# NJUVISION/PCGCv2

Measured on AMD Instinct MI355X. Metric: encode+decode Mpoints/sec at fixed bpp (r3 ckpt), vox10 frame, higher is better.
Workload: dtype f32

## Files before the change

### include/pcgc_hip.h

```cpp
#ifndef PCGC_HIP_H
#define PCGC_HIP_H

#include <stddef.h>
#include <stdint.h>

#ifdef __cplusplus
extern "C" {
#endif

const char* pcgc_last_error(void);
int pcgc_version(void);

int64_t pcgc_hash_capacity(int64_t n);
int pcgc_hash_clear(uint64_t* keys , int32_t* vals , int64_t cap, void* stream);
int pcgc_hash_insert(const int32_t* coords , int64_t n, int32_t stride, uint64_t* keys, int32_t* vals,
                     int64_t cap, void* stream);
int pcgc_hash_insert_policy(const int32_t* coords, int64_t n, int32_t stride, uint64_t* keys, int32_t* vals, int64_t cap,
                            int keep_last, void* stream);
int pcgc_hash_first_mask(const int32_t* coords, int64_t n, int32_t stride, const uint64_t* keys, const int32_t* vals,
                         int64_t cap, uint8_t* keep , int32_t* first_row , void* stream);

int pcgc_coords_check_order(const int32_t* coords , int64_t n, int32_t* out2 , void* stream);

int pcgc_coords_quantize(const int32_t* coords, int64_t n, int32_t stride_out, int32_t* out , void* stream);
int pcgc_coords_children(const int32_t* coords, int64_t n, int32_t stride_in, int32_t* out , void* stream);
int pcgc_coords_scale(const int32_t* coords, int64_t n, float factor, int32_t* out , void* stream);

size_t pcgc_scan_workspace_bytes(int64_t n);
int pcgc_mask_scan(const uint8_t* mask , int64_t n, int32_t* prefix , int32_t* total ,
                   void* workspace , size_t workspace_bytes, void* stream);
int pcgc_mask_scan_zeroed(const uint8_t* mask, int64_t n, int32_t* prefix, int32_t* total, void* workspace, size_t workspace_bytes,
                          void* stream);
int pcgc_compact_coords(const int32_t* coords, const uint8_t* mask, const int32_t* prefix, int64_t n,
                        int32_t* out , void* stream);
int pcgc_compact_feats(const float* in, int C, int in_ld, const uint8_t* mask, const int32_t* prefix, int64_t n,
                       float* out , void* stream);

int pcgc_kmap_k3(const int32_t* coords, int64_t n, int32_t stride, const uint64_t* keys, const int32_t* vals,
                 int64_t cap, int32_t* nbr , void* stream);

int pcgc_kmap_k3_children(const int32_t* parent_nbr, int64_t n_parent, int32_t* nbr , void* stream);
int pcgc_kmap_k3_prune(const int32_t* cand_nbr , int64_t n_cand, const uint8_t* mask, const int32_t* prefix,
                       const int32_t* orig , int64_t n_out, int32_t* nbr , void* stream);
int pcgc_kmap_k3_prune_parent(const int32_t* parent_nbr , int64_t n_parent, const uint8_t* mask,
                              const int32_t* prefix, const int32_t* orig, int64_t n_out, int32_t* nbr , void* stream);
int pcgc_kmap_k3_from_coarse(const int32_t* fine , int64_t n_fine, int32_t stride_fine,
                             const int32_t* parent_of , const int32_t* coarse_nbr ,
                             const int32_t* down , int64_t n_coarse, int32_t* nbr ,
                             void* stream);
int pcgc_down_maps(const int32_t* fine, const int32_t* first_row, const int32_t* prefix, int64_t n_fine, int32_t stride_fine,
                   int64_t n_coarse, int32_t* parent_of , int32_t* down , void* stream);
int pcgc_down_prepare(const int32_t* fine , int64_t n, int32_t stride_fine, int32_t* q ,
                      uint64_t* keys, int32_t* vals, int64_t cap, uint8_t* keep , int32_t* first_row ,
                      int32_t* prefix , int32_t* total , void* scan_ws, size_t scan_ws_bytes, void* stream);
int pcgc_down_finish(const int32_t* fine, const int32_t* q, const uint8_t* keep, const int32_t* first_row, const int32_t* prefix,
                     int64_t n, int32_t stride_fine, int64_t n_coarse, int32_t* coarse ,
                     int32_t* parent_of , int32_t* down , void* stream);
int pcgc_down_level(const int32_t* fine , int64_t n, int32_t stride_fine, int32_t* q, uint64_t* keys, int32_t* vals,
                    int64_t cap, uint8_t* keep, int32_t* first_row, int32_t* prefix, int32_t* total, void* scan_ws,
                    size_t scan_ws_bytes, int32_t* coarse , int32_t* parent_of ,
                    int32_t* down , int64_t* n_coarse_out , void* stream);
size_t pcgc_pyramid_scratch_bytes(int64_t n, int levels);
int pcgc_pyramid(const int32_t* fine , int64_t n, int32_t stride, int levels, void* scratch, size_t scratch_bytes,
                 int32_t* const* coarse, int32_t* const* parent_of, int32_t* const* down, int64_t* counts , void* stream);
int pcgc_compact_index(const uint8_t* mask, const int32_t* prefix, int64_t n, int32_t* orig , void* stream);

int pcgc_conv_gather(const int32_t* nbr, int K, int64_t n_out, const float* in, int64_t n_in , int Cin,
                     int in_ld, int in_coff, const float* W, const float* bias, const float* residual, int res_ld,
                     int res_coff, int relu, float* out, int Cout, int out_ld, int out_coff, void* stream);
int pcgc_last_conv_impl(void);
int pcgc_conv_gather_unit(const int32_t* nbr , int K, int64_t n_out, const float* W, const float* bias, int relu,
                          float* out, int Cout, int out_ld, void* stream);
int pcgc_conv_unit_from_coarse(const int32_t* fine , int64_t n_fine, int32_t stride_fine, const int32_t* parent_of,
                               const int32_t* coarse_nbr , const int32_t* down , int64_t n_coarse,
                               const float* W , const float* bias, int relu, float* out, int Cout, int out_ld, void* stream);
int pcgc_set_conv_impl(int impl);
int pcgc_set_up2_impl(int mfma);
int pcgc_irn_block(const int32_t* nbr , int64_t n, const float* x , int C, int x_ld,
                   const float* const* params, float* t_scratch, float* out, int out_ld, void* stream);
int pcgc_irn_pass(const int32_t* nbr, int64_t n, const float* x, int C, int x_ld, const float* const* params,
                  float* t_scratch, float* out, int out_ld, int pass, void* stream);
int pcgc_conv_up2(int64_t n_in, const float* in, int Cin, int in_ld, const float* W , const float* bias,
                  int relu, float* out , int Cout, void* stream);
int pcgc_conv_up2_gather(int64_t n_in, const float* in, int Cin, int in_ld, const int32_t* rows, const float* W ,
                         const float* bias, int relu, float* out , int Cout, void* stream);

int pcgc_conv_child(const int32_t* parent_nbr , int64_t n_parent, const float* in ,
                    int Cin, int in_ld, const float* table , int64_t table_bytes,
                    const float* bias, const float* residual, int res_ld, int relu, float* out, int Cout, int out_ld, void* stream);
int pcgc_irn_child_pass(const int32_t* parent_nbr, int64_t n_parent, int C, int pass, const float* in, int in_ld,
                        const float* table, int64_t table_bytes, const float* b0, const float* b1, const float* b2,
                        const float* x, int x_ld, float* out, int out_ld, void* stream);
int pcgc_irn_child_q4(const int32_t* parent_nbr, int64_t n_parent, int C, int pass, const float* in, int in_ld,
                      const float* table, int64_t table_bytes, const float* b0, const float* b1, const float* b2,
                      const float* x, int x_ld, float* out, int out_ld, void* stream);
int pcgc_cls_child_q4(const int32_t* parent_nbr, int64_t n_parent, const float* in, int Cin, int in_ld, const float* table,
                      int64_t table_bytes, const float* bias, float* out, void* stream);
int pcgc_irn_rows_pass(const int32_t* nbr, int64_t n, int C, int pass, const float* in, int in_ld, const float* table,
                       int64_t table_bytes, const float* b0, const float* b1, const float* b2, const float* x, int x_ld, float* out,
                       int out_ld, void* stream);
int pcgc_irn_rows_q4_pass(const int32_t* nbr, int64_t n, int C, int pass, const float* in, int in_ld, const float* table,
                          int64_t table_bytes, const float* b0, const float* b1, const float* b2, const float* x, int x_ld, float* out,
                          int out_ld, void* stream);
int pcgc_set_rows_q4_variant(int v);
int pcgc_conv_rows(const int32_t* nbr, int64_t n, const float* in, int Cin, int in_ld, const float* table, int64_t table_bytes,
                   const float* bias, const float* residual, int res_ld, int relu, float* out, int Cout, int out_ld, void* stream);
int pcgc_conv_down_rows(const int32_t* down, int64_t n_coarse, const float* in, int64_t n_in, int Cin, int in_ld, const float* table,
                        int64_t table_bytes, const float* bias, int relu, float* out, int Cout, int out_ld, void* stream);

int pcgc_conv_packed64(const int32_t* nbr, int64_t n, const float* in, int in_ld, const float* table, int64_t table_bytes,
                       const float* bias, int relu, float* out, int out_ld, void* stream);
int pcgc_set_packed_tuning(int rows, int waves);

int pcgc_set_convention(int what, int value);

size_t pcgc_topk_workspace_bytes(int64_t n);
int pcgc_topk_mask(const float* logits , int ld, int64_t n, int64_t k, uint8_t* mask ,
                   void* workspace, size_t workspace_bytes, void* stream);
int pcgc_topk_mask_segments(const float* logits, int ld, int nseg, const int64_t* seg_rows, const int64_t* seg_k, uint8_t* mask,
                            void* workspace, size_t workspace_bytes, void* stream);
size_t pcgc_topk_select_workspace_bytes(int64_t n);
int pcgc_topk_select(const float* logits , int ld, int nseg, const int64_t* seg_rows, const int64_t* seg_k,
                     const int32_t* coords, const int32_t* parent_coords, int32_t parent_stride,
                     uint8_t* bits, int32_t* wprefix, int32_t* orig, int32_t* out_coords, void* workspace, size_t workspace_bytes, void* stream);
int pcgc_kmap_k3_prune_sel(const int32_t* cand_nbr , int64_t n_cand, const uint8_t* bits, const int32_t* wprefix,
                           const int32_t* orig , int64_t n_out, int32_t* nbr , void* stream);
int pcgc_kmap_k3_prune_parent_sel(const int32_t* parent_nbr , int64_t n_parent, const uint8_t* bits, const int32_t* wprefix,
                                  const int32_t* orig, int64_t n_out, int32_t* nbr , void* stream);
int pcgc_gather_rows_f32_ld(const float* in, int C, int in_ld, const int32_t* orig, int64_t n_out, float* out , void* stream);
int pcgc_batch_counts(const int32_t* coords , int64_t n, int32_t* counts , void* stream);

size_t pcgc_sort_workspace_bytes(int64_t n);
int pcgc_sort_zyx(const int32_t* coords, int64_t n, int32_t* perm , void* workspace, size_t workspace_bytes,
                  void* stream);
int pcgc_sort_bzyx(const int32_t* coords, int64_t n, int32_t* perm , void* workspace, size_t workspace_bytes, void* stream);
int pcgc_gather_rows_i32x4(const int32_t* in, const int32_t* perm, int64_t n, int32_t* out, void* stream);
int pcgc_gather_rows_f32(const float* in, int C, const int32_t* perm, int64_t n, float* out, void* stream);

int pcgc_relu(const float* in, int64_t count, float* out, void* stream);
int pcgc_add(const float* a, const float* b, int64_t count, float* out, void* stream);

int pcgc_round_minmax(const float* feats, int64_t count, float* minmax , void* stream);
int pcgc_symbolize(const float* feats, int64_t count, float min_v, int16_t* sym , void* stream);
int pcgc_desymbolize(const int16_t* sym, int64_t count, float min_v, float* feats, void* stream);
int pcgc_quantize_symbols(const float* feats, int64_t count, float* minmax , int16_t* sym , void* stream);
int pcgc_quantize_symbols_segments(const float* feats, int C, int nseg, const int64_t* seg_rows, float* minmax, int16_t* sym, void* stream);
int pcgc_cdf_table(const float* params , int C, float min_v, float max_v, uint16_t* cdf_u16 ,
                   float* cdf_f32 , void* stream);


size_t pcgc_loss_workspace_bytes(int64_t elements);
int pcgc_hash_contains(const int32_t* coords , int64_t n, const uint64_t* keys, const int32_t* vals, int64_t cap,
                       const uint8_t* or_mask , uint8_t* mask , void* stream);
int pcgc_eb_likelihood(const float* feats, int ld, int64_t n, int C, const float* params , float bound, float* likelihood,
                       double* bits, void* workspace, size_t workspace_bytes, void* stream);
int pcgc_neg_log2_sum(const float* x, int ld, int64_t n, int C, double* bits , void* workspace, size_t workspace_bytes, void* stream);
int pcgc_bce_logits(const float* logits, int64_t ld, int64_t n, const uint8_t* truth , const uint8_t* pred ,
                    double* bce, int64_t* counts, void* workspace, size_t workspace_bytes, void* stream);

size_t pcgc_occ_workspace_bytes(int64_t n);
int pcgc_occ_symbols(const float* logits, int64_t ld, int64_t n, const uint8_t* truth , uint16_t* packed ,
                     int64_t* sums , void* workspace, size_t workspace_bytes, void* stream);
int pcgc_occ_tables(uint16_t* p1, int32_t* cost);

size_t pcgc_conv_wgrad_workspace_bytes(int K, int64_t n_rows, int Cin, int Cout);
int64_t pcgc_conv_wgrad_rows_per_group(int K, int64_t n_rows, int Cin, int Cout);
int pcgc_conv_wgrad(const int32_t* nbr, int K, int64_t n_out, const float* x, int64_t n_in, int Cin, int x_ld, const float* gy, int Cout,
                    int gy_ld, float* gW, float* gb, void* workspace, size_t workspace_bytes, void* stream);
int pcgc_conv_up2_wgrad(int64_t n_in, const float* x, int64_t x_rows, int Cin, int x_ld, const int32_t* rows, const float* gy, int Cout,
                        int gy_ld, float* gW, float* gb, void* workspace, size_t workspace_bytes, void* stream);
int pcgc_kmap_invert(const int32_t* nbr, int K, int64_t n_out, int64_t n_in, int32_t* inv , void* stream);
int pcgc_relu_bwd(const float* g, int g_ld, const float* y, int y_ld, int64_t n, int C, float* out, int out_ld, void* stream);
int pcgc_scatter_rows(const float* gy, int C, int gy_ld, const int32_t* orig, int64_t n_rows, float* gx, int64_t n_out, int gx_ld, void* stream);
int pcgc_bce_logits_bwd(const float* logits, int64_t ld, int64_t n, const uint8_t* truth, double scale, float* g , void* stream);
size_t pcgc_eb_bwd_workspace_bytes(int64_t n, int C);
int pcgc_eb_likelihood_bwd(const float* feats, int ld, int64_t n, int C, const float* params , float bound, double scale,
                           float* gy, float* gparams, void* workspace, size_t workspace_bytes, void* stream);

int64_t pcgc_rc_encode(const uint16_t* cdf , int C, int Lp, const int16_t* sym , int64_t n,
                       uint8_t* out , int64_t cap);
int pcgc_rc_decode(const uint16_t* cdf, int C, int Lp, const uint8_t* in, int64_t nbytes, int16_t* sym, int64_t n);
#define PCGC_RC_CKPT_WORDS 6
int64_t pcgc_rc_encode_indexed(const uint16_t* cdf, int C, int Lp, const int16_t* sym, int64_t n, uint8_t* out, int64_t cap, int n_ckpt,
                               uint32_t* ckpt );
int pcgc_rc_decode_indexed(const uint16_t* cdf, int C, int Lp, const uint8_t* in, int64_t nbytes, int16_t* sym, int64_t n, int n_ckpt,
                           const uint32_t* ckpt);
int64_t pcgc_rc_encode_ctx(const uint16_t* cdf , int R, int Lp, const uint16_t* ctx , const int16_t* sym ,
                           int64_t n, uint8_t* out , int64_t cap);
int pcgc_rc_decode_ctx(const uint16_t* cdf, int R, int Lp, const uint16_t* ctx , const uint8_t* in, int64_t nbytes,
                       int16_t* sym , int64_t n);
int pcgc_set_rc_threads(int threads);
int pcgc_set_rc_lanes(int mode);
int pcgc_set_rc_impl(int impl);

int64_t pcgc_oct_encode(const int32_t* xyz , int64_t n, uint8_t* out, int64_t cap);
int64_t pcgc_oct_decode_count(const uint8_t* in, int64_t nbytes);
int pcgc_oct_decode(const uint8_t* in, int64_t nbytes, int32_t* xyz , int64_t n);
int pcgc_set_oct_tiled(int on);
int pcgc_set_oct_model(int model);
int pcgc_oct_warm(void);

int pcgc_d1_nn(const int32_t* a , int64_t na, const uint64_t* b_keys, const int32_t* b_vals, int64_t b_cap,
               const int32_t* offsets , int n_offsets, double* sum , uint64_t* max_d2 ,
               int32_t* unresolved , void* stream);
int pcgc_d1_cell_masks(const int32_t* b , int64_t nb, const uint64_t* cell_keys, const int32_t* cell_vals, int64_t cell_cap,
                       uint64_t* masks , int64_t n_cells, void* stream);
int pcgc_d1_nn_cells(const int32_t* a , int64_t na, const uint64_t* cell_keys, const int32_t* cell_vals, int64_t cell_cap,
                     const uint64_t* masks, const int32_t* offsets , int n_offsets, int32_t reach2, double* sum, uint64_t* max_d2,
                     int32_t* unresolved, void* stream);

int pcgc_d2_runs(const int32_t* qs , int64_t nq, int32_t* runlen , void* stream);
int pcgc_d2_count(const int32_t* p , int64_t n, const int32_t* sel, const uint64_t* cell_keys, const int32_t* cell_vals,
                  int64_t cell_cap, const uint64_t* masks, const uint64_t* keys, const int32_t* vals, int64_t cap, const int32_t* runlen,
                  const int32_t* offsets , int n_offsets, int32_t reach2, int64_t* best , int32_t* cnt ,
                  int32_t* unresolved , int32_t* n_unresolved , void* stream);
int pcgc_d2_fill(const int32_t* p, int64_t n, const int32_t* sel, const uint64_t* cell_keys, const int32_t* cell_vals, int64_t cell_cap,
                 const uint64_t* masks, const uint64_t* keys, const int32_t* vals, int64_t cap, const int32_t* runlen, const int32_t* perm,
                 const int32_t* offsets, int n_offsets, int32_t reach2, const int64_t* best, const int64_t* seg , int32_t* rows, void* stream);
int pcgc_d2_exhaustive(const int32_t* p, int64_t n, const int32_t* sel, const int32_t* qs, int64_t nq, const int32_t* perm, int fill,
                       int64_t* best, int32_t* cnt, const int64_t* seg, int32_t* rows, int32_t* n_empty , void* stream);
size_t pcgc_d2_scan_workspace_bytes(int64_t n);
int pcgc_d2_scan(const int32_t* cnt , int64_t n, int64_t* seg , void* workspace, size_t workspace_bytes, void* stream);
int pcgc_d2_segment_lowest(const int64_t* seg, int64_t n, int32_t* rows, int32_t cap, int32_t* kept, void* stream);
int pcgc_d2_recv_count(const int64_t* seg, const int32_t* kept, int64_t na, const int32_t* rows, int64_t nb, int32_t* rcnt, void* stream);
int pcgc_d2_recv_fill(const int64_t* seg, const int32_t* kept, int64_t na, const int32_t* rows, int64_t nb, const int64_t* rseg, int32_t* cursor,
                      int32_t* recv, void* stream);
int pcgc_d2_normals(const int64_t* rseg, const int32_t* recv, int64_t nb, const double* na, const int64_t* seg_ba, const int32_t* kept_ba,
                    const int32_t* rows_ba, double* nb_out, void* stream);
int pcgc_d2_c2p(const int32_t* p, int64_t n, const int32_t* q, const double* nq, const int64_t* seg, const int32_t* kept, const int32_t* rows,
                double* c2p, void* stream);
size_t pcgc_d2_reduce_workspace_bytes(void);
int pcgc_d2_reduce(const int64_t* c2c, const double* c2p, int64_t n, int64_t* c2c_sum_max, double* c2p_sum, void* workspace, size_t workspace_bytes,
                   void* stream);

size_t pcgc_attr_transfer_workspace_bytes(int64_t ns, int64_t nt, int channels);
int pcgc_attr_transfer(const int64_t* seg_st, const int32_t* kept_st, const int32_t* rows_st, int64_t ns, const int64_t* seg_ts,
                       const int32_t* kept_ts, const int32_t* rows_ts, int64_t nt, const uint8_t* attr_s, int channels, uint8_t* attr_t,
                       void* workspace, size_t workspace_bytes, void* stream);
int pcgc_colour_dist(const uint8_t* cp, int64_t n, const uint8_t* cq, int64_t nq, const int64_t* seg, const int32_t* kept, const int32_t* rows,
                     int64_t* yuv2, int32_t* rgb2, void* stream);
size_t pcgc_colour_reduce_workspace_bytes(void);
int pcgc_colour_reduce(const int64_t* yuv2, const int32_t* rgb2, int64_t n, int64_t* out, void* workspace, size_t workspace_bytes, void* stream);

int64_t pcgc_normals_ball_masks(int32_t r2, uint64_t* table );
size_t pcgc_normals_workspace_bytes(int64_t n);
int pcgc_normals_estimate(const int32_t* coords , int64_t n, const int32_t* qs , const int32_t* perm,
                          const uint64_t* cell_keys, const int32_t* cell_vals, int64_t cell_cap, const uint64_t* masks, const uint64_t* keys,
                          const int32_t* vals, int64_t cap, const int32_t* runlen, const uint64_t* ball , int32_t r2, int orient,
                          const double* viewpoint , int64_t* moments , double* normals ,
                          double* lam , int32_t* count , uint8_t* valid , void* workspace,
                          size_t workspace_bytes, void* stream);
int pcgc_set_normals_mapping(int mode);

int64_t pcgc_ply_read_ascii_geo(const char* path, int32_t* xyz , int64_t cap);
int pcgc_ply_write_ascii_geo(const char* path, const int32_t* xyz , int64_t n);
int pcgc_ply_write_ascii_geo_rgb(const char* path, const int32_t* xyz , const uint8_t* rgb , int64_t n);

typedef int (*pcgc_table_fn)(const float* params, int C, float min_v, float max_v, uint16_t* table_u16, float* cdf_f32);
int pcgc_items_encode(int n_items, const char* const* stems, const int16_t* sym, const int32_t* xyz, const int64_t* rows, const float* ranges,
                      int C, const int32_t* counts, const float* eb_params, pcgc_table_fn table_fn, int index_segments, int write_coords,
                      int threads);
int pcgc_items_probe(int n_items, const char* const* stems, int64_t* rows, int32_t* channels, float* ranges, int32_t* counts,
                     int32_t* native_coords);
int pcgc_items_decode(int n_items, const char* const* stems, const int64_t* rows, int C, const float* ranges, const int32_t* native_coords,
                      const float* eb_params, pcgc_table_fn table_fn, int use_sidecar, int16_t* sym, int32_t* xyz, int coord_layout,
                      int coord_scale, int threads);

int pcgc_level_prepare_children(const int32_t* coords, int64_t n, int32_t stride, uint64_t* keys, int32_t* vals, int64_t cap, int32_t* nbr,
                                int32_t* children, int32_t* nbr_children, void* stream);

int pcgc_frame_decode(const char* stem, int C, const float* eb_params, pcgc_table_fn table_fn, int use_sidecar, int coord_scale,
                      int64_t cap_rows, int16_t* sym, int32_t* level, int64_t* info, float* range, int threads);
int pcgc_frame_decode_begin(const char* stem, int C, const float* eb_params, pcgc_table_fn table_fn, int use_sidecar, int coord_scale,
                            int64_t cap_rows, int16_t* sym, int32_t* level, int64_t* info, float* range, int threads);
int pcgc_frame_decode_end(void);
int pcgc_frame_worker_test(int delay_us);

int pcgc_table_cache(int mode);

uint32_t pcgc_crc32(uint32_t crc, const uint8_t* buf, int64_t len);

int pcgc_mesh_read(const char* path, double* verts , int64_t vcap, int32_t* faces , int64_t fcap,
                   int64_t* counts );
size_t pcgc_mesh_cdf_workspace_bytes(int64_t T);
int pcgc_mesh_area_cdf(const double* verts , int64_t V, const int32_t* faces , int64_t T,
                       double* cdf , int32_t* bad_faces , void* workspace, size_t workspace_bytes, void* stream);
int pcgc_mesh_sample(const double* verts, int64_t V, const int32_t* faces, const double* cdf, int64_t T, uint64_t seed, uint64_t first,
                     int64_t n, int32_t* tri , double* points , void* stream);
size_t pcgc_mesh_voxelize_workspace_bytes(int32_t resolution);
int pcgc_mesh_voxelize(const double* verts, int64_t V, const int32_t* faces, const double* cdf, int64_t T, uint64_t seed, int64_t n,
                       const double* R , int32_t resolution, int32_t* out , int64_t cap,
                       int32_t* count , void* workspace , size_t workspace_bytes, void* stream);

#define PCGC_COLLATE_MAX_ITEMS 16
typedef struct pcgc_collate_item {
    int64_t offset;
    int32_t first_row, rows, width, symmetry, extent, reserved;
} pcgc_collate_item;
int pcgc_collate_rows(const uint8_t* arena , const pcgc_collate_item* items , int n_items,
                      int32_t* coords_out , float* feats_out , void* stream);

#ifdef __cplusplus
}
#endif
#endif
```

### pcgcv2_amd/_build.py

```python
import os
import subprocess
import sys
from concurrent.futures import ThreadPoolExecutor

HERE = os.path.dirname(os.path.abspath(__file__))
CSRC = os.path.join(HERE, 'csrc')
VARIANT = os.environ.get('PCGC_BUILD_VARIANT', '')
OBJ = os.path.join(CSRC, '_obj' + ('_' + VARIANT if VARIANT else ''))
LIB = os.path.join(HERE, 'libpcgc_hip' + ('_' + VARIANT if VARIANT else '') + '.so')
SOURCES = ['coords.hip', 'select.hip', 'conv.hip', 'child_conv.hip', 'child_conv32.hip', 'child_cls_w.hip', 'child_irn.hip', 'child_irn_a16.hip', 'child_irn_b16.hip',
           'child_irn_a32.hip', 'child_irn_b32.hip', 'child_q4.hip', 'rows_irn.hip', 'rows_q4.hip', 'conv_packed.hip', 'entropy.hip', 'loss.hip', 'occupancy.hip', 'grad.hip', 'metric.hip', 'colour.hip', 'normals.hip', 'mesh.hip', 'collate.hip', 'hostcodec.cpp', 'ply.cpp', 'mesh_io.cpp']
HEADERS = [os.path.join(CSRC, 'pcgc_common.h'), os.path.join(CSRC, 'mfma_util.h'), os.path.join(CSRC, 'child_kernels.h'), os.path.join(CSRC, 'child_q4.h'), os.path.join(CSRC, 'q4x.h'), os.path.join(CSRC, 'q4x_sched.h'), os.path.join(CSRC, 'rows_q4_policy.h'), os.path.join(CSRC, 'eb_logits.h'), os.path.join(CSRC, 'occupancy_tables.h'), os.path.join(HERE, '..', 'include', 'pcgc_hip.h')]
FLAGS = ['--offload-arch=gfx950', '-O3', '-std=c++17', '-ffp-contract=off', '-fPIC', '-Wall', '-Wno-unused-result'] + \
        os.environ.get('PCGC_EXTRA_HIPCC_FLAGS', '').split()


def _hipcc():
    for c in (os.environ.get('HIPCC'), '/opt/rocm/bin/hipcc', 'hipcc'):
        if c and (os.path.isabs(c) and os.path.exists(c) or not os.path.isabs(c)):
            return c
    return 'hipcc'


def _stale(target, deps):
    if not os.path.exists(target):
        return True
    t = os.path.getmtime(target)
    return any(os.path.getmtime(d) > t for d in deps)


def build(force=False, verbose=False):
    os.makedirs(OBJ, exist_ok=True)
    if VARIANT:
        import shutil
        base = os.path.join(CSRC, '_obj')
        for src in SOURCES:
            o = src.rsplit('.', 1)[0] + '.o'
            if 'child_kernels.h' not in open(os.path.join(CSRC, src)).read() and os.path.exists(os.path.join(base, o)) \
                    and not os.path.exists(os.path.join(OBJ, o)):
                shutil.copy2(os.path.join(base, o), os.path.join(OBJ, o))
    hipcc = _hipcc()
    jobs = []
    only = [t for t in os.environ.get('PCGC_BUILD_ONLY', '').split(',') if t]
    for src in SOURCES:
        s = os.path.join(CSRC, src)
        o = os.path.join(OBJ, src.rsplit('.', 1)[0] + '.o')
        if only and os.path.exists(o):
            if src.rsplit('.', 1)[0] in only:
                jobs.append((o, [hipcc] + FLAGS + (['-x', 'hip'] if src.endswith('.hip') else []) + ['-c', s, '-o', o]))
            continue
        if force or _stale(o, [s] + HEADERS):
            lang = ['-x', 'hip'] if src.endswith('.hip') else []
            jobs.append((o, [hipcc] + FLAGS + lang + ['-c', s, '-o', o]))

    def run(job):
        o, cmd = job
        if verbose:
            print(' '.join(cmd), file=sys.stderr)
        r = subprocess.run(cmd, capture_output=True, text=True)
        if r.returncode != 0:
            raise RuntimeError('hipcc failed:\n' + ' '.join(cmd) + '\n' + r.stderr[-4000:])
        return o

    with ThreadPoolExecutor(max_workers=max(2, min(8, os.cpu_count() or 4))) as ex:
        list(ex.map(run, jobs))
    objs = [os.path.join(OBJ, s.rsplit('.', 1)[0] + '.o') for s in SOURCES]
    if force or jobs or _stale(LIB, objs):
        cmd = [hipcc, '--offload-arch=gfx950', '-shared', '-fPIC', '-o', LIB] + objs + ['-lz']
        r = subprocess.run(cmd, capture_output=True, text=True)
        if r.returncode != 0:
            raise RuntimeError('link failed:\n' + r.stderr[-4000:])
    if not VARIANT:
        build_reftable(force=force)
    return LIB


REFTABLE_LIB = os.path.join(HERE, 'libpcgc_reftable.so')


def build_reftable(force=False):
    src = os.path.join(CSRC, 'reftable.cpp')
    if not (force or _stale(REFTABLE_LIB, [src])):
        return REFTABLE_LIB
    import torch
    tdir = os.path.dirname(torch.__file__)
    cmd = ['g++', '-O2', '-std=c++17', '-fPIC', '-shared', f'-D_GLIBCXX_USE_CXX11_ABI={int(torch._C._GLIBCXX_USE_CXX11_ABI)}',
           '-I' + os.path.join(tdir, 'include'), '-I' + os.path.join(tdir, 'include', 'torch', 'csrc', 'api', 'include'), src,
           '-o', REFTABLE_LIB, '-L' + os.path.join(tdir, 'lib'), '-ltorch_cpu', '-lc10', '-Wl,-rpath,' + os.path.join(tdir, 'lib')]
    r = subprocess.run(cmd, capture_output=True, text=True)
    if r.returncode != 0:
        raise RuntimeError('g++ failed:\n' + ' '.join(cmd) + '\n' + r.stderr[-4000:])
    return REFTABLE_LIB


if __name__ == '__main__':
    print(build(force='--force' in sys.argv, verbose=True))
```

### pcgcv2_amd/_lib.py

```python
import ctypes as C
import os

_HERE = os.path.dirname(os.path.abspath(__file__))
LIB_PATH = os.environ.get('PCGC_LIB') or os.path.join(_HERE, 'libpcgc_hip.so')

vp, i64, i32, f32, sz = C.c_void_p, C.c_int64, C.c_int32, C.c_float, C.c_size_t
ci = C.c_int

SIGNATURES = {
    'pcgc_last_error': (C.c_char_p, []),
    'pcgc_version': (ci, []),
    'pcgc_hash_capacity': (i64, [i64]),
    'pcgc_hash_clear': (ci, [vp, vp, i64, vp]),
    'pcgc_hash_insert': (ci, [vp, i64, i32, vp, vp, i64, vp]),
    'pcgc_hash_insert_policy': (ci, [vp, i64, i32, vp, vp, i64, ci, vp]),
    'pcgc_set_convention': (ci, [ci, ci]),
    'pcgc_hash_first_mask': (ci, [vp, i64, i32, vp, vp, i64, vp, vp, vp]),
    'pcgc_coords_check_order': (ci, [vp, i64, vp, vp]),
    'pcgc_coords_quantize': (ci, [vp, i64, i32, vp, vp]),
    'pcgc_coords_children': (ci, [vp, i64, i32, vp, vp]),
    'pcgc_coords_scale': (ci, [vp, i64, f32, vp, vp]),
    'pcgc_scan_workspace_bytes': (sz, [i64]),
    'pcgc_mask_scan': (ci, [vp, i64, vp, vp, vp, sz, vp]),
    'pcgc_mask_scan_zeroed': (ci, [vp, i64, vp, vp, vp, sz, vp]),
    'pcgc_compact_coords': (ci, [vp, vp, vp, i64, vp, vp]),
    'pcgc_compact_feats': (ci, [vp, ci, ci, vp, vp, i64, vp, vp]),
    'pcgc_kmap_k3': (ci, [vp, i64, i32, vp, vp, i64, vp, vp]),
    'pcgc_kmap_k3_children': (ci, [vp, i64, vp, vp]),
    'pcgc_kmap_k3_prune': (ci, [vp, i64, vp, vp, vp, i64, vp, vp]),
    'pcgc_kmap_k3_prune_parent': (ci, [vp, i64, vp, vp, vp, i64, vp, vp]),
    'pcgc_kmap_k3_from_coarse': (ci, [vp, i64, i32, vp, vp, vp, i64, vp, vp]),
    'pcgc_down_maps': (ci, [vp, vp, vp, i64, i32, i64, vp, vp, vp]),
    'pcgc_down_prepare': (ci, [vp, i64, i32, vp, vp, vp, i64, vp, vp, vp, vp, vp, sz, vp]),
    'pcgc_down_finish': (ci, [vp, vp, vp, vp, vp, i64, i32, i64, vp, vp, vp, vp]),
    'pcgc_down_level': (ci, [vp, i64, i32, vp, vp, vp, i64, vp, vp, vp, vp, vp, sz, vp, vp, vp, vp, vp]),
    'pcgc_pyramid_scratch_bytes': (sz, [i64, ci]),
    'pcgc_pyramid': (ci, [vp, i64, i32, ci, vp, sz, vp, vp, vp, vp, vp]),
    'pcgc_compact_index': (ci, [vp, vp, i64, vp, vp]),
    'pcgc_conv_gather': (ci, [vp, ci, i64, vp, i64, ci, ci, ci, vp, vp, vp, ci, ci, ci, vp, ci, ci, ci, vp]),
    'pcgc_conv_gather_unit': (ci, [vp, ci, i64, vp, vp, ci, vp, ci, ci, vp]),
    'pcgc_conv_unit_from_coarse': (ci, [vp, i64, i32, vp, vp, vp, i64, vp, vp, ci, vp, ci, ci, vp]),
    'pcgc_set_conv_impl': (ci, [ci]),
    'pcgc_last_conv_impl': (ci, []),
    'pcgc_set_up2_impl': (ci, [ci]),
    'pcgc_irn_block': (ci, [vp, i64, vp, ci, ci, vp, vp, vp, ci, vp]),
    'pcgc_irn_pass': (ci, [vp, i64, vp, ci, ci, vp, vp, vp, ci, ci, vp]),
    'pcgc_conv_child': (ci, [vp, i64, vp, ci, ci, vp, i64, vp, vp, ci, ci, vp, ci, ci, vp]),
    'pcgc_irn_child_pass': (ci, [vp, i64, ci, ci, vp, ci, vp, i64, vp, vp, vp, vp, ci, vp, ci, vp]),
    'pcgc_irn_child_q4': (ci, [vp, i64, ci, ci, vp, ci, vp, i64, vp, vp, vp, vp, ci, vp, ci, vp]),
    'pcgc_cls_child_q4': (ci, [vp, i64, vp, ci, ci, vp, i64, vp, vp, vp]),
    'pcgc_conv_down_rows': (ci, [vp, i64, vp, i64, ci, ci, vp, i64, vp, ci, vp, ci, ci, vp]),
    'pcgc_conv_rows': (ci, [vp, i64, vp, ci, ci, vp, i64, vp, vp, ci, ci, vp, ci, ci, vp]),
    'pcgc_irn_rows_pass': (ci, [vp, i64, ci, ci, vp, ci, vp, i64, vp, vp, vp, vp, ci, vp, ci, vp]),
    'pcgc_irn_rows_q4_pass': (ci, [vp, i64, ci, ci, vp, ci, vp, i64, vp, vp, vp, vp, ci, vp, ci, vp]),
    'pcgc_set_rows_q4_variant': (ci, [ci]),
    'pcgc_conv_packed64': (ci, [vp, i64, vp, ci, vp, i64, vp, ci, vp, ci, vp]),
    'pcgc_set_packed_tuning': (ci, [ci, ci]),
    'pcgc_conv_up2': (ci, [i64, vp, ci, ci, vp, vp, ci, vp, ci, vp]),
    'pcgc_conv_up2_gather': (ci, [i64, vp, ci, ci, vp, vp, vp, ci, vp, ci, vp]),
    'pcgc_topk_workspace_bytes': (sz, [i64]),
    'pcgc_topk_mask': (ci, [vp, ci, i64, i64, vp, vp, sz, vp]),
    'pcgc_topk_mask_segments': (ci, [vp, ci, ci, vp, vp, vp, vp, sz, vp]),
    'pcgc_topk_select_workspace_bytes': (sz, [i64]),
    'pcgc_topk_select': (ci, [vp, ci, ci, vp, vp, vp, vp, i32, vp, vp, vp, vp, vp, sz, vp]),
    'pcgc_kmap_k3_prune_sel': (ci, [vp, i64, vp, vp, vp, i64, vp, vp]),
    'pcgc_kmap_k3_prune_parent_sel': (ci, [vp, i64, vp, vp, vp, i64, vp, vp]),
    'pcgc_gather_rows_f32_ld': (ci, [vp, ci, ci, vp, i64, vp, vp]),
    'pcgc_batch_counts': (ci, [vp, i64, vp, vp]),
    'pcgc_sort_bzyx': (ci, [vp, i64, vp, vp, sz, vp]),
    'pcgc_quantize_symbols_segments': (ci, [vp, ci, ci, vp, vp, vp, vp]),
    'pcgc_sort_workspace_bytes': (sz, [i64]),
    'pcgc_sort_zyx': (ci, [vp, i64, vp, vp, sz, vp]),
    'pcgc_gather_rows_i32x4': (ci, [vp, vp, i64, vp, vp]),
    'pcgc_gather_rows_f32': (ci, [vp, ci, vp, i64, vp, vp]),
    'pcgc_relu': (ci, [vp, i64, vp, vp]),
    'pcgc_add': (ci, [vp, vp, i64, vp, vp]),
    'pcgc_round_minmax': (ci, [vp, i64, vp, vp]),
    'pcgc_symbolize': (ci, [vp, i64, f32, vp, vp]),
    'pcgc_desymbolize': (ci, [vp, i64, f32, vp, vp]),
    'pcgc_quantize_symbols': (ci, [vp, i64, vp, vp, vp]),
    'pcgc_cdf_table': (ci, [vp, ci, f32, f32, vp, vp, vp]),
    'pcgc_loss_workspace_bytes': (sz, [i64]),
    'pcgc_hash_contains': (ci, [vp, i64, vp, vp, i64, vp, vp, vp]),
    'pcgc_eb_likelihood': (ci, [vp, ci, i64, ci, vp, f32, vp, vp, vp, sz, vp]),
    'pcgc_neg_log2_sum': (ci, [vp, ci, i64, ci, vp, vp, sz, vp]),
    'pcgc_bce_logits': (ci, [vp, i64, i64, vp, vp, vp, vp, vp, sz, vp]),
    'pcgc_occ_workspace_bytes': (sz, [i64]),
    'pcgc_occ_symbols': (ci, [vp, i64, i64, vp, vp, vp, vp, sz, vp]),
    'pcgc_occ_tables': (ci, [vp, vp]),
    'pcgc_conv_wgrad_workspace_bytes': (sz, [ci, i64, ci, ci]),
    'pcgc_conv_wgrad_rows_per_group': (i64, [ci, i64, ci, ci]),
    'pcgc_conv_wgrad': (ci, [vp, ci, i64, vp, i64, ci, ci, vp, ci, ci, vp, vp, vp, sz, vp]),
    'pcgc_conv_up2_wgrad': (ci, [i64, vp, i64, ci, ci, vp, vp, ci, ci, vp, vp, vp, sz, vp]),
    'pcgc_kmap_invert': (ci, [vp, ci, i64, i64, vp, vp]),
    'pcgc_relu_bwd': (ci, [vp, ci, vp, ci, i64, ci, vp, ci, vp]),
    'pcgc_scatter_rows': (ci, [vp, ci, ci, vp, i64, vp, i64, ci, vp]),
    'pcgc_bce_logits_bwd': (ci, [vp, i64, i64, vp, C.c_double, vp, vp]),
    'pcgc_eb_bwd_workspace_bytes': (sz, [i64, ci]),
    'pcgc_eb_likelihood_bwd': (ci, [vp, ci, i64, ci, vp, f32, C.c_double, vp, vp, vp, sz, vp]),
    'pcgc_d1_cell_masks': (ci, [vp, i64, vp, vp, i64, vp, i64, vp]),
    'pcgc_d1_nn_cells': (ci, [vp, i64, vp, vp, i64, vp, vp, ci, i32, vp, vp, vp, vp]),
    'pcgc_d1_nn': (ci, [vp, i64, vp, vp, i64, vp, ci, vp, vp, vp, vp]),
    'pcgc_d2_runs': (ci, [vp, i64, vp, vp]),
    'pcgc_d2_count': (ci, [vp, i64, vp, vp, vp, i64, vp, vp, vp, i64, vp, vp, ci, i32, vp, vp, vp, vp, vp]),
    'pcgc_d2_fill': (ci, [vp, i64, vp, vp, vp, i64, vp, vp, vp, i64, vp, vp, vp, ci, i32, vp, vp, vp, vp]),
    'pcgc_d2_exhaustive': (ci, [vp, i64, vp, vp, i64, vp, ci, vp, vp, vp, vp, vp, vp]),
    'pcgc_d2_scan_workspace_bytes': (sz, [i64]),
    'pcgc_d2_scan': (ci, [vp, i64, vp, vp, sz, vp]),
    'pcgc_d2_segment_lowest': (ci, [vp, i64, vp, i32, vp, vp]),
    'pcgc_d2_recv_count': (ci, [vp, vp, i64, vp, i64, vp, vp]),
    'pcgc_d2_recv_fill': (ci, [vp, vp, i64, vp, i64, vp, vp, vp, vp]),
    'pcgc_d2_normals': (ci, [vp, vp, i64, vp, vp, vp, vp, vp, vp]),
    'pcgc_d2_c2p': (ci, [vp, i64, vp, vp, vp, vp, vp, vp, vp]),
    'pcgc_d2_reduce_workspace_bytes': (sz, []),
    'pcgc_d2_reduce': (ci, [vp, vp, i64, vp, vp, vp, sz, vp]),
    'pcgc_attr_transfer_workspace_bytes': (sz, [i64, i64, ci]),
    'pcgc_attr_transfer': (ci, [vp, vp, vp, i64, vp, vp, vp, i64, vp, ci, vp, vp, sz, vp]),
    'pcgc_colour_dist': (ci, [vp, i64, vp, i64, vp, vp, vp, vp, vp, vp]),
    'pcgc_colour_reduce_workspace_bytes': (sz, []),
    'pcgc_colour_reduce': (ci, [vp, vp, i64, vp, vp, sz, vp]),
    'pcgc_normals_ball_masks': (i64, [i32, vp]),
    'pcgc_normals_workspace_bytes': (sz, [i64]),
    'pcgc_normals_estimate': (ci, [vp, i64, vp, vp, vp, vp, i64, vp, vp, vp, i64, vp, vp, i32, ci, vp, vp, vp, vp, vp, vp, vp, sz, vp]),
    'pcgc_set_normals_mapping': (ci, [ci]),
    'pcgc_rc_encode': (i64, [vp, ci, ci, vp, i64, vp, i64]),
    'pcgc_rc_decode': (ci, [vp, ci, ci, vp, i64, vp, i64]),
    'pcgc_set_rc_impl': (ci, [ci]),
    'pcgc_rc_encode_indexed': (i64, [vp, ci, ci, vp, i64, vp, i64, ci, vp]),
    'pcgc_rc_decode_indexed': (ci, [vp, ci, ci, vp, i64, vp, i64, ci, vp]),
    'pcgc_rc_encode_ctx': (i64, [vp, ci, ci, vp, vp, i64, vp, i64]),
    'pcgc_rc_decode_ctx': (ci, [vp, ci, ci, vp, vp, i64, vp, i64]),
    'pcgc_set_rc_threads': (ci, [ci]),
    'pcgc_set_rc_lanes': (ci, [ci]),
    'pcgc_set_oct_tiled': (ci, [ci]),
    'pcgc_set_oct_model': (ci, [ci]),
    'pcgc_oct_warm': (ci, []),
    'pcgc_oct_encode': (i64, [vp, i64, vp, i64]),
    'pcgc_oct_decode_count': (i64, [vp, i64]),
    'pcgc_oct_decode': (ci, [vp, i64, vp, i64]),
    'pcgc_items_encode': (ci, [ci, vp, vp, vp, vp, vp, ci, vp, vp, vp, ci, ci, ci]),
    'pcgc_items_probe': (ci, [ci, vp, vp, vp, vp, vp, vp]),
    'pcgc_items_decode': (ci, [ci, vp, vp, ci, vp, vp, vp, vp, ci, vp, vp, ci, ci, ci]),
    'pcgc_level_prepare_children': (ci, [vp, i64, i32, vp, vp, i64, vp, vp, vp, vp]),
    'pcgc_frame_decode': (ci, [C.c_char_p, ci, vp, vp, ci, ci, i64, vp, vp, vp, vp, ci]),
    'pcgc_frame_decode_begin': (ci, [C.c_char_p, ci, vp, vp, ci, ci, i64, vp, vp, vp, vp, ci]),
    'pcgc_frame_decode_end': (ci, []),
    'pcgc_frame_worker_test': (ci, [ci]),
    'pcgc_table_cache': (ci, [ci]),
    'pcgc_crc32': (C.c_uint32, [C.c_uint32, vp, i64]),
    'pcgc_ply_read_ascii_geo': (i64, [C.c_char_p, vp, i64]),
    'pcgc_ply_write_ascii_geo': (ci, [C.c_char_p, vp, i64]),
    'pcgc_ply_write_ascii_geo_rgb': (ci, [C.c_char_p, vp, vp, i64]),
    'pcgc_mesh_read': (ci, [C.c_char_p, vp, i64, vp, i64, vp]),
    'pcgc_mesh_cdf_workspace_bytes': (sz, [i64]),
    'pcgc_mesh_area_cdf': (ci, [vp, i64, vp, i64, vp, vp, vp, sz, vp]),
    'pcgc_mesh_sample': (ci, [vp, i64, vp, vp, i64, C.c_uint64, C.c_uint64, i64, vp, vp, vp]),
    'pcgc_mesh_voxelize_workspace_bytes': (sz, [i32]),
    'pcgc_mesh_voxelize': (ci, [vp, i64, vp, vp, i64, C.c_uint64, i64, vp, i32, vp, i64, vp, vp, sz, vp]),
    'pcgc_collate_rows': (ci, [vp, vp, ci, vp, vp, vp]),
}


class CollateItem(C.Structure):
    _fields_ = [('offset', i64), ('first_row', i32), ('rows', i32), ('width', i32), ('symmetry', i32), ('extent', i32), ('reserved', i32)]


class PcgcError(RuntimeError):
    pass


_lib = None


def lib():
    global _lib
    if _lib is None:
        if not os.path.exists(LIB_PATH):
            raise PcgcError(f'{LIB_PATH} not found: run `python -c "import __graft_entry__ as g; g.build()"` '
                            '(hipcc --offload-arch=gfx950). The HIP library is mandatory; there is no fallback path.')
        l = C.CDLL(LIB_PATH)
        for name, (res, args) in SIGNATURES.items():
            fn = getattr(l, name)
            fn.restype, fn.argtypes = res, args
        _lib = l
    return _lib


REFTABLE_PATH = os.path.join(_HERE, 'libpcgc_reftable.so')
_reftable = None


def reftable_lib():
    global _reftable
    if _reftable is None:
        if not os.path.exists(REFTABLE_PATH):
            raise PcgcError(f'{REFTABLE_PATH} not found: run `python -c "import __graft_entry__ as g; g.build()"`')
        import torch
        l = C.CDLL(REFTABLE_PATH)
        l.pcgc_reference_table.restype = ci
        l.pcgc_reference_table.argtypes = [vp, ci, f32, f32, vp, vp]
        l.pcgc_reference_table_clear.restype = ci
        l.pcgc_reference_table_clear.argtypes = []
        _reftable = l
    return _reftable


def check(rc, what=''):
    if rc != 0:
        raise PcgcError(f'{what or "pcgc call"} failed ({rc}): {lib().pcgc_last_error().decode()}')
```

### pcgcv2_amd/csrc/child_kernels.h

```cpp
#pragma once
#include "pcgc_common.h"
#include "mfma_util.h"
#include <type_traits>

#ifdef PCGC_CHILD_TIMING
static __device__ unsigned long long g_child_dbg[8];
#define CHILD_T(var) const unsigned long long var = __builtin_amdgcn_s_memtime()
#define CHILD_TADD(slot, a, b) do { child_dbg[slot] += (b) - (a); } while (0)
#define CHILD_DBG_DECL unsigned long long child_dbg[8] = {0, 0, 0, 0, 0, 0, 0, 0};
#define CHILD_DBG_PARAM , unsigned long long (&child_dbg)[8]
#define CHILD_DBG_ARG , child_dbg
#define CHILD_TFLUSH do { if ((threadIdx.x & 63) == 0) { for (int q_ = 0; q_ < 8; ++q_) if (child_dbg[q_]) atomicAdd(&g_child_dbg[q_], child_dbg[q_]); } } while (0)
#define CHILD_TIMING_READER(NAME)                                                                                      \
    extern "C" int NAME(unsigned long long* out8, int reset) {                                                         \
        (void)hipDeviceSynchronize();                                                                                  \
        if (out8) (void)hipMemcpyFromSymbol(out8, HIP_SYMBOL(g_child_dbg), 8 * sizeof(unsigned long long));           \
        if (reset) { unsigned long long z[8] = {0}; (void)hipMemcpyToSymbol(HIP_SYMBOL(g_child_dbg), z, sizeof(z)); }  \
        return 0;                                                                                                      \
    }
#else
#define CHILD_T(var)
#define CHILD_TADD(slot, a, b)
#define CHILD_DBG_DECL
#define CHILD_DBG_PARAM
#define CHILD_DBG_ARG
#define CHILD_TFLUSH
#define CHILD_TIMING_READER(NAME)
#endif

struct ChildEpi {
    const float* bias;
    const float* res;
    int res_ld;
    int relu;
    float* out;
    int out_ld;
    int nt;
};
struct IrnEpi {
    const float* b0;
    const float* b1;
    const float* b2;
    const float* x;
    int x_ld;
    float* out;
    int out_ld;
};
namespace {


constexpr int halo_p1(int c) { return c == 0 ? 0 : (c == 3 ? 2 : 1); }
constexpr int halo_bit(int c) { return (c == 0 || c == 2) ? 1 : 0; }
constexpr int cell_kp(int c) { return halo_p1(c >> 4) * 9 + halo_p1((c >> 2) & 3) * 3 + halo_p1(c & 3); }
constexpr int cell_child(int c) { return halo_bit(c & 3) + 2 * halo_bit((c >> 2) & 3) + 4 * halo_bit(c >> 4); }
constexpr bool axis_reach(int c, int jb) { return c - jb >= 0 && c - jb <= 2; }
constexpr unsigned cell_reach(int c) {
    unsigned m = 0;
    for (int j = 0; j < 8; ++j)
        if (axis_reach(c & 3, j & 1) && axis_reach((c >> 2) & 3, (j >> 1) & 1) && axis_reach(c >> 4, j >> 2)) m |= 1u << j;
    return m;
}
constexpr int cell_k(int c, int j) {
    return ((c >> 4) - (j >> 2)) * 9 + (((c >> 2) & 3) - ((j >> 1) & 1)) * 3 + ((c & 3) - (j & 1));
}
constexpr int cz_of(int c) { return c >> 4; }
constexpr int cy_of(int c) { return (c >> 2) & 3; }
constexpr int cx_of(int c) { return c & 3; }
constexpr bool in02(int v) { return v >= 0 && v <= 2; }

struct HaloGeometry {
    static constexpr int NCELLS = 64, ROW_MUL = 8, NMAP = 27;
    static constexpr int kp(int c) { return cell_kp(c); }
    static constexpr int child(int c) { return cell_child(c); }
    static constexpr int byte_off(int) { return 0; }
};

template <int NB_, int NT, int HZ = -1>
struct PlainConv : HaloGeometry {
    static constexpr int NB = NB_, ROWCHUNKS = 4, T = 8 * NT, KS = 4;
    static constexpr int Z_HALF = HZ;
    static constexpr bool HALF = false;
    static constexpr int kfirst(int) { return 0; }
    static constexpr bool active(int c, int t) { return (HZ < 0 || (((t / NT) >> 2) & 1) == HZ) && ((cell_reach(c) >> (t / NT)) & 1); }
    static constexpr int frag(int c, int t) { return cell_k(c, t / NT) * NT + t % NT; }
    static constexpr bool uses_block(int, int) { return true; }
    static constexpr int frag_off(int c, int t, int cb) { return (frag(c, t) * NB + cb) * 64 * KS * 4; }
};
template <int NB_>
struct ClsHead : HaloGeometry {
    static constexpr int NB = NB_, ROWCHUNKS = 4, T = 1, KS = 4;
    static constexpr bool HALF = true;
    static constexpr int ROWB = NB * 64 + 16;
    static constexpr int TABLE_BYTES = (125 * ROWB + 1023) / 1024 * 1024;
    static constexpr int kfirst(int) { return 0; }
    static constexpr bool active(int, int) { return true; }
    static constexpr bool uses_block(int, int) { return true; }
    static constexpr int frag_off(int c, int, int cb) { return (cz_of(c) * 25 + cy_of(c) * 5 + cx_of(c)) * ROWB + cb * 64; }
    __device__ static inline int lane_table_off(int mi, int mq) {
        const int j = mi & 7;
        return (31 - (25 * (j >> 2) + 5 * ((j >> 1) & 1) + (j & 1))) * ROWB + mq * 16;
    }
};
template <int C, int HZ = -1>
struct PassA : HaloGeometry {
    static_assert(C == 16 || C == 32, "children-level passes: C = 16, 32 (C = 64 runs on the rows kernels through the level's own map)");
    static constexpr int Q = C / 4, NB = C / 16, ROWCHUNKS = 4, CPT = 16 / Q , TH = 8 / CPT, T = 2 * TH, KS = 4;
    static_assert(HZ < 0 || CPT <= 2, "half units: tiles of one or two children (a z-half tile holds both halves' columns)");
    static constexpr int Z_HALF = HZ;
    static constexpr bool HALF = false;
    static constexpr int kfirst(int) { return 0; }
    static constexpr int tz(int t) { return CPT == 4 ? (t % TH) : (t % TH) >> 1; }
    static constexpr int ty(int t) { return (t % TH) & 1; }
    static constexpr bool active(int c, int t) {
        const int kz = cz_of(c) - tz(t);
        if (HZ >= 0 && tz(t) != HZ) return false;
        if (CPT == 4) {
            if (t < TH) return in02(kz);
            return kz == 1 && (cy_of(c) == 1 || cy_of(c) == 2) && (cx_of(c) == 1 || cx_of(c) == 2);
        }
        const int ky = cy_of(c) - ty(t);
        if (t < TH) return in02(kz) && in02(ky);
        return kz == 1 && ky == 1 && (cx_of(c) == 1 || cx_of(c) == 2);
    }
    static constexpr int N0 = CPT == 4 ? 48 : (CPT == 2 ? 36 : 27);
    static constexpr int frag(int c, int t) {
        const int kz = cz_of(c) - tz(t);
        if (CPT == 4) return t < TH ? kz * 16 + (c & 15) : N0 + (cy_of(c) - 1) * 2 + (cx_of(c) - 1);
        const int ky = cy_of(c) - ty(t);
        return t < TH ? (kz * 3 + ky) * 4 + cx_of(c) : N0 + (cx_of(c) - 1);
    }
    static constexpr bool uses_block(int, int) { return true; }
    static constexpr int frag_off(int c, int t, int cb) { return (frag(c, t) * NB + cb) * 64 * KS * 4; }
};
template <int C, int HZ = -1, bool T2_ = false>
struct PassB : HaloGeometry {
    static constexpr bool T2 = T2_;
    static_assert(!T2_ || C == 16, "the split layout exists for C = 16");
    static constexpr int Q = C / 4, NB = 1, ROWCHUNKS = Q / 2 , KS = Q / 4;
    static constexpr int CPT0 = 16 / (2 * Q) , T0 = 8 / CPT0, CPT1 = 16 / Q, T1 = 8 / CPT1, T = T0 + T1;
    static constexpr int Z_HALF = HZ;
    static_assert(HZ < 0 || CPT1 <= 2, "half units: no tile may hold children of both z halves");
    static constexpr bool HALF = false;
    static constexpr int kfirst(int t) { return t < T0 ? 0 : KS; }
    static constexpr int tile_z(int t) { return t < T0 ? ((t * CPT0) >> 2) & 1 : (((t - T0) * CPT1) >> 2) & 1; }
    static constexpr bool active(int c, int t) {
        if (HZ >= 0 && tile_z(t) != HZ) return false;
        if (t < T0) {
            if (CPT0 == 1) return (cell_reach(c) >> t) & 1;
            return in02(cz_of(c) - (t >> 1)) && in02(cy_of(c) - (t & 1));
        }
        const int u = t - T0;
        if (CPT1 == 2) return in02(cz_of(c) - (u >> 1)) && in02(cy_of(c) - (u & 1));
        return in02(cz_of(c) - u);
    }
    static constexpr int N0 = CPT0 == 1 ? 27 : 36;
    static constexpr int N1 = CPT1 == 2 ? 36 : 48;
    static constexpr int FRAG_W12 = N0 + N1;
    static constexpr int frag(int c, int t) {
        if (t < T0) {
            if (CPT0 == 1) return cell_k(c, t);
            return ((cz_of(c) - (t >> 1)) * 3 + (cy_of(c) - (t & 1))) * 4 + cx_of(c);
        }
        const int u = t - T0;
        if (CPT1 == 2) return N0 + ((cz_of(c) - (u >> 1)) * 3 + (cy_of(c) - (u & 1))) * 4 + cx_of(c);
        return N0 + (cz_of(c) - u) * 16 + (c & 15);
    }
    static constexpr bool uses_block(int, int) { return true; }
    static constexpr int frag_off(int c, int t, int cb) { return (frag(c, t) * NB + cb) * 64 * KS * 4; }
};

template <class V, class = void> struct child_t2_layout : std::false_type {};
template <class V> struct child_t2_layout<V, std::enable_if_t<V::T2>> : std::true_type {};

template <int I, int N, typename F>
__device__ __forceinline__ void static_for(F&& f) {
    if constexpr (I < N) {
        f(std::integral_constant<int, I>{});
        static_for<I + 1, N>(f);
    }
}

template <int KS> struct BFrag;
template <> struct BFrag<4> {
    f32x4 v;
    template <int OFF> __device__ __forceinline__ void load(unsigned base) { asm volatile("ds_read_b128 %0, %1 offset:%2" : "=v"(v) : "v"(base), "n"(OFF) : "memory"); }
    __device__ __forceinline__ void tie() { asm volatile("" : "+v"(v)); }
    __device__ __forceinline__ float get(int i) const { return v[i]; }
};
typedef float f32x2 __attribute__((ext_vector_type(2)));
template <> struct BFrag<2> {
    f32x2 v;
    template <int OFF> __device__ __forceinline__ void load(unsigned base) { asm volatile("ds_read_b64 %0, %1 offset:%2" : "=v"(v) : "v"(base), "n"(OFF) : "memory"); }
    __device__ __forceinline__ void tie() { asm volatile("" : "+v"(v)); }
    __device__ __forceinline__ float get(int i) const { return v[i]; }
};
template <> struct BFrag<1> {
    float v;
    template <int OFF> __device__ __forceinline__ void load(unsigned base) { asm volatile("ds_read_b32 %0, %1 offset:%2" : "=v"(v) : "v"(base), "n"(OFF) : "memory"); }
    __device__ __forceinline__ void tie() { asm volatile("" : "+v"(v)); }
    __device__ __forceinline__ float get(int) const { return v; }
};
template <int OFF>
__device__ __forceinline__ float lds_ld32_off(unsigned base) {
    float v;
    asm volatile("ds_read_b32 %0, %1 offset:%2" : "=v"(v) : "v"(base), "n"(OFF) : "memory");
    return v;
}
template <int OFF>
__device__ __forceinline__ f32x4 lds_ld128_off(unsigned base) {
    f32x4 v;
    asm volatile("ds_read_b128 %0, %1 offset:%2" : "=v"(v) : "v"(base), "n"(OFF) : "memory");
    return v;
}

template <class V> constexpr int frag_floats() { return (V::HALF ? 32 : 64) * V::KS; }

template <int NW, bool PERSIST = true>
__device__ __forceinline__ int64_t child_tile(int i, int wave, int64_t ntiles) {
    if constexpr (!PERSIST) {
        const int64_t tile = (int64_t)xcd_tile(blockIdx.x, gridDim.x) * NW + wave;
        return (i == 0 && tile < ntiles) ? tile : -1;
    }
    const int64_t S = (ntiles + 7) >> 3;
    const int64_t l = (blockIdx.x >> 3) + (int64_t)(gridDim.x >> 3) * (wave + NW * i);
    const int64_t tile = (blockIdx.x & 7) * S + l;
    return (l < S && tile < ntiles) ? tile : -1;
}

template <int NW>
__device__ __forceinline__ void child_stage_table(const float* __restrict__ table, int table_bytes, unsigned char* lds_raw) {
    float4* tab = (float4*)lds_raw;
    for (int i = threadIdx.x; i < table_bytes / 16; i += NW * 64) tab[i] = ((const float4*)table)[i];
    __syncthreads();
}

struct ChildCells { int n; int c[64]; };
template <class V> constexpr ChildCells child_cells() {
    ChildCells L{};
    for (int c = 0; c < V::NCELLS; ++c) {
        bool used = false;
        for (int t = 0; t < V::T; ++t) used = used || V::active(c, t);
        if (used) L.c[L.n++] = c;
    }
    return L;
}

template <class V, int D, int MT>
__device__ __forceinline__ void child_tile_mainloop_mt(const int32_t* __restrict__ pnbr, int64_t n_p, int64_t p0,
                                                       const __amdgpu_buffer_rsrc_t& rs_in, int in_ld, const unsigned char* lds_raw,
                                                       float4* ring, f32x4 (&acc)[MT][V::T] CHILD_DBG_PARAM) {
    constexpr int NB = V::NB, T = V::T, KS = V::KS;
    static_assert(MT == 1 || MT == 2, "one or two M tiles per wave");
    static_assert((D & (D - 1)) == 0, "ring depth must be a power of two");
    static_assert((D - 1) * NB * MT < 64, "vmcnt is 6 bits");
    CHILD_T(t_tile0);
    const int lane = threadIdx.x & 63;
    const int mi = lane & 15, mq = lane >> 4;
    const int dma_r = lane >> 2;
    bool row_ok[MT];
#pragma unroll
    for (int m = 0; m < MT; ++m) row_ok[m] = p0 + 16 * m + dma_r < n_p;
    constexpr unsigned ABSENT = 0xF0000000u;
    unsigned rowb[MT][V::NMAP];
#pragma unroll
    for (int m = 0; m < MT; ++m)
#pragma unroll
        for (int kp = 0; kp < V::NMAP; ++kp) rowb[m][kp] = (unsigned)pnbr[(int64_t)kp * n_p + (row_ok[m] ? p0 + 16 * m + dma_r : 0)];
    const int f_a = (0x78 >> (2 * (mi >> 2))) & 3;
    const int dma_chunk = (lane & 3) ^ ((0x78 >> (2 * ((dma_r >> 2) & 3))) & 3);
    const bool chunk_ok = dma_chunk < V::ROWCHUNKS;
    const unsigned row_bytes = (unsigned)in_ld * 4u;
    asm volatile("s_waitcnt vmcnt(0)" ::: "memory");
#pragma unroll
    for (int m = 0; m < MT; ++m)
#pragma unroll
        for (int kp = 0; kp < V::NMAP; ++kp)
            rowb[m][kp] = (row_ok[m] && (int)rowb[m][kp] >= 0) ? rowb[m][kp] * ((unsigned)V::ROW_MUL * row_bytes) : ABSENT;
    constexpr bool T2 = child_t2_layout<V>::value;
    const unsigned lane_off = chunk_ok ? (unsigned)dma_chunk * (T2 ? 64u : 16u) : ABSENT;
    CHILD_T(t_loop0);

    constexpr ChildCells CL = child_cells<V>();
    constexpr int NC = CL.n;
    auto issue = [&](auto ii) {
        constexpr int i = decltype(ii)::value, c = CL.c[i];
        float4* dst = ring + (i & (D - 1)) * (MT * NB * 64);
#pragma unroll
        for (int m = 0; m < MT; ++m) {
            unsigned voff = rowb[m][V::kp(c)] + (T2 ? (unsigned)((V::child(c) >> 2) * 128 + (V::child(c) & 3) * 16) : (unsigned)V::child(c) * row_bytes) + lane_off +
                            (unsigned)V::byte_off(c);
            if constexpr (V::ROWCHUNKS < 4) voff = chunk_ok ? voff : 0xFFFFFFF0u;
#pragma unroll
            for (int cb = 0; cb < NB; ++cb)
                __builtin_amdgcn_raw_ptr_buffer_load_lds(rs_in, (lds_void_ptr)(dst + (m * NB + cb) * 64), 16, (int)(voff + cb * 64), 0, 0, 0);
        }
        asm volatile("" ::: "memory");
    };

#pragma unroll
    for (int m = 0; m < MT; ++m)
#pragma unroll
        for (int t = 0; t < T; ++t) acc[m][t] = (f32x4){0.f, 0.f, 0.f, 0.f};
    unsigned tab_lane;
    if constexpr (V::HALF) tab_lane = (unsigned)(uintptr_t)(lds_void_ptr)(lds_raw + V::lane_table_off(mi, mq));
    else tab_lane = (unsigned)(uintptr_t)(lds_void_ptr)((const float*)lds_raw + lane * KS);
    unsigned a_addr[4];
#pragma unroll
    for (int jj = 0; jj < 4; ++jj) a_addr[jj] = (unsigned)(uintptr_t)(lds_void_ptr)((const float*)ring + (mi * 4 + (jj ^ f_a)) * 4 + mq);
    constexpr unsigned ksteps_used = [] { unsigned m = 0; for (int t = 0; t < T; ++t) for (int j = 0; j < KS; ++j) m |= 1u << (V::kfirst(t) + j); return m; }();

    static_assert(NB * T <= 32, "all B fragments of a cell are held in registers at once");
    static_for<0, (D < NC ? D : NC)>(issue);
    static_for<0, NC>([&](auto ii) {
        constexpr int i = decltype(ii)::value, c = CL.c[i];
        constexpr int younger = (NC - 1 - i) < (D - 1) ? (NC - 1 - i) : (D - 1);
        wait_vmcnt<younger * NB * MT>();
        float a[MT][NB][4];
        BFrag<KS> b[NB][T];
        static_for<0, NB>([&](auto icb) {
            constexpr int cb = decltype(icb)::value;
            static_for<0, MT>([&](auto im) {
                constexpr int m = decltype(im)::value;
                static_for<0, 4>([&](auto ij) {
                    constexpr int jj = decltype(ij)::value;
                    if constexpr ((ksteps_used >> jj) & 1)
                        a[m][cb][jj] = lds_ld32_off<(((i & (D - 1)) * MT + m) * NB + cb) * 1024>(a_addr[jj]);
                });
            });
            static_for<0, T>([&](auto it) {
                constexpr int t = decltype(it)::value;
                if constexpr (V::active(c, t) && V::uses_block(t, cb)) {
                    constexpr int off = V::frag_off(c, t, cb);
                    if constexpr (off < 65536) b[cb][t].template load<off>(tab_lane);
                    else b[cb][t].template load<off - 65536>(tab_lane + 65536);
                }
            });
        });
        asm volatile("s_waitcnt lgkmcnt(0)" ::: "memory");
        static_for<0, NB>([&](auto icb) {
            constexpr int cb = decltype(icb)::value;
            static_for<0, MT>([&](auto im) {
                static_for<0, 4>([&](auto ij) {
                    constexpr int jj = decltype(ij)::value;
                    if constexpr ((ksteps_used >> jj) & 1) lds_tie(a[decltype(im)::value][cb][jj]);
                });
            });
            static_for<0, T>([&](auto it) {
                constexpr int t = decltype(it)::value;
                if constexpr (V::active(c, t) && V::uses_block(t, cb)) b[cb][t].tie();
            });
        });
        if constexpr (i + D < NC) issue(std::integral_constant<int, i + D>{});
        static_for<0, NB>([&](auto icb) {
            constexpr int cb = decltype(icb)::value;
            static_for<0, 4>([&](auto ij) {
                constexpr int jj = decltype(ij)::value;
                static_for<0, T>([&](auto it) {
                    constexpr int t = decltype(it)::value;
                    if constexpr (V::active(c, t) && V::uses_block(t, cb) && jj >= V::kfirst(t) && jj < V::kfirst(t) + KS) {
                        static_for<0, MT>([&](auto im) {
                            constexpr int m = decltype(im)::value;
                            acc[m][t] = __builtin_amdgcn_mfma_f32_16x16x4f32(a[m][cb][jj], b[cb][t].get(jj - V::kfirst(t)), acc[m][t], 0, 0, 0);
                        });
                    }
                });
            });
        });
    });
#ifdef PCGC_CHILD_TIMING
    asm volatile("s_nop 0" : "+v"(acc[0][0]));
    CHILD_T(t_loop1);
    CHILD_TADD(0, t_tile0, t_loop0);
    CHILD_TADD(1, t_loop0, t_loop1);
    CHILD_TADD(3, 0ull, 1ull);
#endif
}

template <class V, int D>
__device__ __forceinline__ void child_tile_mainloop(const int32_t* __restrict__ pnbr, int64_t n_p, int64_t p0,
                                                    const __amdgpu_buffer_rsrc_t& rs_in, int in_ld, const unsigned char* lds_raw,
                                                    float4* ring, f32x4 (&acc)[V::T] CHILD_DBG_PARAM) {
    child_tile_mainloop_mt<V, D, 1>(pnbr, n_p, p0, rs_in, in_ld, lds_raw, ring, reinterpret_cast<f32x4 (&)[1][V::T]>(acc) CHILD_DBG_ARG);
}

__device__ __forceinline__ void wave_lds_sync() {
    __builtin_amdgcn_fence(__ATOMIC_RELEASE, "wavefront");
    __builtin_amdgcn_wave_barrier();
    __builtin_amdgcn_fence(__ATOMIC_ACQUIRE, "wavefront");
}

template <int W, int ROWS>
struct ChildResidual { float4 x[(ROWS * (W / 4) + 63) / 64]; };
template <int W, int ROWS>
__device__ __forceinline__ void child_flush_prefetch(ChildResidual<W, ROWS>& rr, int64_t row0, int64_t rows_total, const float* __restrict__ res,
                                                     int res_ld, int lane, int half = -1) {
    constexpr int C4 = W / 4, N = (ROWS * C4 + 63) / 64;
    if (!res) return;
#pragma unroll
    for (int it = 0; it < N; ++it) {
        const int i = lane + 64 * it, lr = i / C4, c4 = i % C4;
        const int64_t row = row0 + lr;
        const bool ok = i < ROWS * C4 && row < rows_total && !(half >= 0 && ((lr >> 2) & 1) != half);
        rr.x[it] = ok ? *(const float4*)(res + row * res_ld + 4 * c4) : make_float4(0.f, 0.f, 0.f, 0.f);
    }
}
template <int W, int ROWS>
__device__ __forceinline__ void child_flush(const float* scratch, const ChildResidual<W, ROWS>& rr, bool has_res, int64_t row0, int64_t rows_total,
                                            float* __restrict__ out, int out_ld, int relu, int lane, int half = -1) {
    constexpr int C4 = W / 4, N = (ROWS * C4 + 63) / 64;
    ChildResidual<W, ROWS> xr = rr;
    if (has_res) {
#pragma unroll
        for (int it = 0; it < N; ++it) asm volatile("" : "+v"(xr.x[it].x), "+v"(xr.x[it].y), "+v"(xr.x[it].z), "+v"(xr.x[it].w));
    }
#pragma unroll
    for (int it = 0; it < N; ++it) {
        const int i = lane + 64 * it, lr = i / C4, c4 = i % C4;
        const int64_t row = row0 + lr;
        if (i >= ROWS * C4 || row >= rows_total || (half >= 0 && ((lr >> 2) & 1) != half)) continue;
        float4 v = ((const float4*)scratch)[i];
        if (has_res) {
            const float4 x = xr.x[it];
            v.x = v.x + x.x; v.y = v.y + x.y; v.z = v.z + x.z; v.w = v.w + x.w;
        }
        if (relu) { v.x = fmaxf(v.x, 0.0f); v.y = fmaxf(v.y, 0.0f); v.z = fmaxf(v.z, 0.0f); v.w = fmaxf(v.w, 0.0f); }
        *(float4*)(out + row * out_ld + 4 * c4) = v;
    }
}
template <int W, int ROWS>
__device__ __forceinline__ void child_flush(const float* scratch, int64_t row0, int64_t rows_total, float* __restrict__ out, int out_ld,
                                            int relu, int lane, int half = -1) {
    constexpr int C4 = W / 4, N = (ROWS * C4 + 63) / 64;
#pragma unroll
    for (int it = 0; it < N; ++it) {
        const int i = lane + 64 * it, lr = i / C4, c4 = i % C4;
        const int64_t row = row0 + lr;
        if (i >= ROWS * C4 || row >= rows_total || (half >= 0 && ((lr >> 2) & 1) != half)) continue;
        float4 v = ((const float4*)scratch)[i];
        if (relu) { v.x = fmaxf(v.x, 0.0f); v.y = fmaxf(v.y, 0.0f); v.z = fmaxf(v.z, 0.0f); v.w = fmaxf(v.w, 0.0f); }
        *(float4*)(out + row * out_ld + 4 * c4) = v;
    }
}
template <int W>
__device__ __forceinline__ void child_flush(const float* scratch, int rows, int64_t row0, int64_t rows_total, float* __restrict__ out,
                                            int out_ld, const float* __restrict__ res, int res_ld, int relu, int lane, int half = -1) {
    constexpr int C4 = W / 4;
    for (int i = lane; i < rows * C4; i += 64) {
        const int lr = i / C4, c4 = i % C4;
        const int64_t row = row0 + lr;
        if (row >= rows_total || (half >= 0 && ((lr >> 2) & 1) != half)) continue;
        float4 v = ((const float4*)scratch)[i];
        if (res) {
            const float4 x = *(const float4*)(res + row * res_ld + 4 * c4);
            v.x = v.x + x.x; v.y = v.y + x.y; v.z = v.z + x.z; v.w = v.w + x.w;
        }
        if (relu) { v.x = fmaxf(v.x, 0.0f); v.y = fmaxf(v.y, 0.0f); v.z = fmaxf(v.z, 0.0f); v.w = fmaxf(v.w, 0.0f); }
        *(float4*)(out + row * out_ld + 4 * c4) = v;
    }
}

#define CHILD_IN_ROWS(V, n_p) (V::ROW_MUL * (n_p))
#define CHILD_KERNEL_PROLOGUE(V, NW, D, RING_FLOAT4)                                                                          \
    CHILD_DBG_DECL                                                                                                            \
    extern __shared__ __attribute__((aligned(16))) unsigned char lds_raw[];                                                   \
    const int lane = threadIdx.x & 63, mi = lane & 15, mq = lane >> 4;                                                        \
    const int wave = __builtin_amdgcn_readfirstlane(threadIdx.x >> 6);                                                        \
    float4* ring = (float4*)(lds_raw + table_bytes) + wave * (RING_FLOAT4);                                                   \
    child_stage_table<NW>(table, table_bytes, lds_raw);                                                                        \
    const __amdgpu_buffer_rsrc_t rs_in = __builtin_amdgcn_make_buffer_rsrc((void*)in, 0, (int)(CHILD_IN_ROWS(V, n_p) * in_ld * 4), 0x00020000); \
    const int64_t ntiles = (n_p + 15) >> 4;

template <class T_> struct child_type_tag { using type = T_; };
template <int NB, int NT, int NW, int D, bool SPLIT = false, int MT = 1, bool RES = false>
__global__ void __launch_bounds__(NW * 64)
k_child_conv(const int32_t* __restrict__ pnbr, int64_t n_p, const float* __restrict__ in, int in_ld,
             const float* __restrict__ table, int table_bytes, ChildEpi ep) {
    using V = PlainConv<NB, NT>;
    CHILD_KERNEL_PROLOGUE(V, NW, D, D * NB * 64 * MT)
    float bvs[NT];
#pragma unroll
    for (int n = 0; n < NT; ++n) bvs[n] = ep.bias ? ep.bias[16 * n + mi] : 0.0f;
    auto unit = [&](auto tag, const int64_t pu) {
        using VV = typename decltype(tag)::type;
        constexpr int HZ = VV::Z_HALF;
        f32x4 acc[MT][VV::T];
        child_tile_mainloop_mt<VV, D, MT>(pnbr, n_p, pu, rs_in, in_ld, lds_raw, ring, acc CHILD_DBG_ARG);
        constexpr int W = 16 * NT, CH = (64 * W * 4 <= D * NB * 1024 * MT) ? 64 : 32, PPC = CH / 8, MQC = PPC / 4;
        float* scratch = (float*)ring;
#pragma unroll
        for (int m = 0; m < MT; ++m) {
            const int64_t p0 = pu + 16 * m;
            if (m > 0 && p0 >= n_p) break;
#pragma unroll
            for (int h = 0; h < 128 / CH; ++h) {
                ChildResidual<W, RES ? CH : 1> rr;
                if constexpr (RES) child_flush_prefetch<W, CH>(rr, 8 * p0 + h * CH, 8 * n_p, ep.res, ep.res_ld, lane, HZ);
                if (mq / MQC == h) {
#pragma unroll
                    for (int t = 0; t < VV::T; ++t) {
                        const int j = t / NT, n = t % NT;
                        if (HZ >= 0 && ((j >> 2) & 1) != HZ) continue;
#pragma unroll
                        for (int r = 0; r < 4; ++r) {
                            float v = acc[m][t][r];
                            if (ep.bias) v = v + bvs[n];
                            scratch[(8 * (4 * (mq % MQC) + r) + j) * W + 16 * n + mi] = v;
                        }
                    }
                }
                wave_lds_sync();
                if constexpr (RES) child_flush<W, CH>(scratch, rr, true, 8 * p0 + h * CH, 8 * n_p, ep.out, ep.out_ld, ep.relu, lane, HZ);
                else child_flush<W, CH>(scratch, 8 * p0 + h * CH, 8 * n_p, ep.out, ep.out_ld, ep.relu, lane, HZ);
                wave_lds_sync();
            }
        }
    };
    const int64_t nunits = (SPLIT ? 2 : 1) * ((n_p + 16 * MT - 1) / (16 * MT));
    for (int i = 0;; ++i) {
        const int64_t u = child_tile<NW>(i, wave, nunits);
        if (u < 0) break;
        CHILD_T(t_it0);
        if constexpr (SPLIT) {
            if (u & 1) unit(child_type_tag<PlainConv<NB, NT, 1>>{}, (u >> 1) * (16 * MT));
            else unit(child_type_tag<PlainConv<NB, NT, 0>>{}, (u >> 1) * (16 * MT));
        } else {
            unit(child_type_tag<V>{}, u * (16 * MT));
        }
#ifdef PCGC_CHILD_TIMING
        { CHILD_T(t_dr0); asm volatile("s_waitcnt vmcnt(0)" ::: "memory"); CHILD_T(t_it1); CHILD_TADD(5, t_dr0, t_it1); CHILD_TADD(4, t_it0, t_it1); }
#endif
    }
    CHILD_TFLUSH;
}

template <int NB, int NW, int D, int MT = 1>
__global__ void __launch_bounds__(NW * 64)
k_child_cls(const int32_t* __restrict__ pnbr, int64_t n_p, const float* __restrict__ in, int in_ld,
            const float* __restrict__ table, int table_bytes, ChildEpi ep) {
    using V = ClsHead<NB>;
    CHILD_KERNEL_PROLOGUE(V, NW, D, D * NB * 64 * MT)
    const float bv = ep.bias ? ep.bias[0] : 0.0f;
    const int64_t nunits = (n_p + 16 * MT - 1) / (16 * MT);
    for (int i = 0;; ++i) {
        const int64_t tile = child_tile<NW>(i, wave, nunits);
        if (tile < 0) break;
        const int64_t pu = tile * (16 * MT);
        CHILD_T(t_it0);
        f32x4 acc[MT][1];
        child_tile_mainloop_mt<V, D, MT>(pnbr, n_p, pu, rs_in, in_ld, lds_raw, ring, acc CHILD_DBG_ARG);
        if (mi < 8) {
#pragma unroll
            for (int m = 0; m < MT; ++m) {
#pragma unroll
                for (int r = 0; r < 4; ++r) {
                    const int64_t p = pu + 16 * m + 4 * mq + r;
                    if (p >= n_p) continue;
                    float v = acc[m][0][r];
                    if (ep.bias) v = v + bv;
                    ep.out[(8 * p + mi) * ep.out_ld] = v;
                }
            }
        }
#ifdef PCGC_CHILD_TIMING
        { CHILD_T(t_dr0); asm volatile("s_waitcnt vmcnt(0)" ::: "memory"); CHILD_T(t_it1); CHILD_TADD(5, t_dr0, t_it1); CHILD_TADD(4, t_it0, t_it1); }
#endif
    }
    CHILD_TFLUSH;
}



template <int C, int NW, int D, bool SPLIT = false, int MT = 1>
__global__ void __launch_bounds__(NW * 64)
k_child_irn_a(const int32_t* __restrict__ pnbr, int64_t n_p, const float* __restrict__ in, int in_ld,
              const float* __restrict__ table, int table_bytes, IrnEpi ep) {
    using V = PassA<C>;
    constexpr int Q = V::Q, CPT = V::CPT, TH = V::TH;
    static_assert(!SPLIT || CPT <= 2, "half units: tiles of one or two children");
    CHILD_KERNEL_PROLOGUE(V, NW, D, D * V::NB * 64 * MT)
    const int co = mi % Q, sub = mi / Q;
    const float b00 = ep.b0[co], b10 = ep.b1[co];
    auto unit = [&](auto tag, const int64_t pu) {
        using VV = typename decltype(tag)::type;
        constexpr int HZ = VV::Z_HALF;
        f32x4 acc[MT][VV::T];
        child_tile_mainloop_mt<VV, D, MT>(pnbr, n_p, pu, rs_in, in_ld, lds_raw, ring, acc CHILD_DBG_ARG);
        constexpr int W = 2 * Q, CH = (64 * W * 4 <= D * V::NB * 1024 * MT) ? 64 : 32, MQC = CH / 32;
        float* scratch = (float*)ring;
#pragma unroll
        for (int m = 0; m < MT; ++m) {
            const int64_t p0 = pu + 16 * m;
            if (m > 0 && p0 >= n_p) break;
#pragma unroll
            for (int h = 0; h < 128 / CH; ++h) {
                if (mq / MQC == h) {
#pragma unroll
                    for (int t = 0; t < TH; ++t) {
                        if (HZ >= 0 && (((t * CPT) >> 2) & 1) != HZ) continue;
                        const int j = t * CPT + sub;
#pragma unroll
                        for (int r = 0; r < 4; ++r) {
                            float* y = scratch + (8 * (4 * (mq % MQC) + r) + j) * W;
                            y[co] = fmaxf(acc[m][t][r] + b00, 0.0f);
                            y[Q + co] = fmaxf(acc[m][TH + t][r] + b10, 0.0f);
                        }
                    }
                }
                wave_lds_sync();
                child_flush<W, CH>(scratch, 8 * p0 + h * CH, 8 * n_p, ep.out, W, 0, lane, HZ);
                wave_lds_sync();
            }
        }
    };
    const int64_t nunits = (SPLIT ? 2 : 1) * ((n_p + 16 * MT - 1) / (16 * MT));
    for (int i = 0;; ++i) {
        const int64_t u = child_tile<NW>(i, wave, nunits);
        if (u < 0) break;
        CHILD_T(t_it0);
        if constexpr (SPLIT) {
            if (u & 1) unit(child_type_tag<PassA<C, 1>>{}, (u >> 1) * (16 * MT));
            else unit(child_type_tag<PassA<C, 0>>{}, (u >> 1) * (16 * MT));
        } else {
            unit(child_type_tag<V>{}, u * (16 * MT));
        }
#ifdef PCGC_CHILD_TIMING
        { CHILD_T(t_dr0); asm volatile("s_waitcnt vmcnt(0)" ::: "memory"); CHILD_T(t_it1); CHILD_TADD(5, t_dr0, t_it1); CHILD_TADD(4, t_it0, t_it1); }
#endif
    }
    CHILD_TFLUSH;
}

template <int C, int NW, int D, bool SPLIT = false, int MT = 1, bool T2 = false>
__global__ void __launch_bounds__(NW * 64)
k_child_irn_b(const int32_t* __restrict__ pnbr, int64_t n_p, const float* __restrict__ in , int in_ld,
              const float* __restrict__ table, int table_bytes, IrnEpi ep) {
    using V = PassB<C, -1, T2>;
    constexpr int Q = V::Q, H = 2 * Q, KQ = Q / 4, T0 = V::T0, T1 = V::T1, CPT0 = V::CPT0, CPT1 = V::CPT1;
    constexpr int CH = ((128 * Q + 64 * C) * 4 <= D * 1024 * MT) ? 64 : 32, MQC = CH / 32;
    constexpr int NEEDF4 = (128 * Q + CH * C) / 4;
    constexpr int RINGF4 = (D * 64 * MT > NEEDF4) ? D * 64 * MT : NEEDF4;
    CHILD_KERNEL_PROLOGUE(V, NW, D, RINGF4)
    float* us = (float*)ring;
    float* stage = us + 128 * Q;
    float w12[KQ];
#pragma unroll
    for (int jj = 0; jj < KQ; ++jj) w12[jj] = ((const float*)lds_raw)[V::FRAG_W12 * frag_floats<V>() + lane * KQ + jj];
    const int c1 = mi % Q, sub1 = mi / Q, c0 = mi % H, sub0 = mi / H;
    const float b11 = ep.b1[c1], b01 = ep.b0[c0], b12 = mi < H ? ep.b2[mi] : 0.0f;
    auto unit = [&](auto tag, const int64_t pu) {
        using VV = typename decltype(tag)::type;
        constexpr int HZ = VV::Z_HALF;
        f32x4 acc[MT][VV::T];
        child_tile_mainloop_mt<VV, D, MT>(pnbr, n_p, pu, rs_in, in_ld, lds_raw, ring, acc CHILD_DBG_ARG);
#pragma unroll
        for (int m = 0; m < MT; ++m) {
        const int64_t p0 = pu + 16 * m;
        if (m > 0 && p0 >= n_p) break;
        ChildResidual<C, CH> rr;
        child_flush_prefetch<C, CH>(rr, 8 * p0, 8 * n_p, ep.x, ep.x_ld, lane, HZ);
        {
#pragma unroll
            for (int u = 0; u < T1; ++u) {
                if (HZ >= 0 && VV::tile_z(T0 + u) != HZ) continue;
#pragma unroll
                for (int r = 0; r < 4; ++r) us[(8 * (4 * mq + r) + u * CPT1 + sub1) * Q + c1] = fmaxf(acc[m][T0 + u][r] + b11, 0.0f);
            }
        }
        wave_lds_sync();
        {
#pragma unroll
            for (int h = 0; h < 128 / CH; ++h) {
                if (h > 0) child_flush_prefetch<C, CH>(rr, 8 * p0 + h * CH, 8 * n_p, ep.x, ep.x_ld, lane, HZ);
                if (mq / MQC == h) {
#pragma unroll
                    for (int t = 0; t < T0; ++t) {
                        if (HZ >= 0 && VV::tile_z(t) != HZ) continue;
                        const int j = t * CPT0 + sub0;
#pragma unroll
                        for (int r = 0; r < 4; ++r) stage[(8 * (4 * (mq % MQC) + r) + j) * C + c0] = acc[m][t][r] + b01;
                    }
                }
                float au[CH / 16][KQ];
#pragma unroll
                for (int gg = 0; gg < CH / 16; ++gg)
#pragma unroll
                    for (int jj = 0; jj < KQ; ++jj) au[gg][jj] = us[(16 * (h * (CH / 16) + gg) + mi) * Q + 4 * jj + mq];
                f32x4 d[CH / 16];
#pragma unroll
                for (int gg = 0; gg < CH / 16; ++gg) {
                    d[gg] = (f32x4){0.f, 0.f, 0.f, 0.f};
#pragma unroll
                    for (int jj = 0; jj < KQ; ++jj) d[gg] = __builtin_amdgcn_mfma_f32_16x16x4f32(au[gg][jj], w12[jj], d[gg], 0, 0, 0);
                }
                if (mi < H) {
#pragma unroll
                    for (int gg = 0; gg < CH / 16; ++gg)
#pragma unroll
                        for (int r = 0; r < 4; ++r) stage[(16 * gg + 4 * mq + r) * C + H + mi] = d[gg][r] + b12;
                }
                wave_lds_sync();
                child_flush<C, CH>(stage, rr, ep.x != nullptr, 8 * p0 + h * CH, 8 * n_p, ep.out, ep.out_ld, 0, lane, HZ);
                wave_lds_sync();
            }
        }
        }
    };
    const int64_t nunits = (SPLIT ? 2 : 1) * ((n_p + 16 * MT - 1) / (16 * MT));
    for (int i = 0;; ++i) {
        const int64_t u = child_tile<NW>(i, wave, nunits);
        if (u < 0) break;
        CHILD_T(t_it0);
        if constexpr (SPLIT) {
            if (u & 1) unit(child_type_tag<PassB<C, 1, T2>>{}, (u >> 1) * (16 * MT));
            else unit(child_type_tag<PassB<C, 0, T2>>{}, (u >> 1) * (16 * MT));
        } else {
            unit(child_type_tag<V>{}, u * (16 * MT));
        }
#ifdef PCGC_CHILD_TIMING
        { CHILD_T(t_dr0); asm volatile("s_waitcnt vmcnt(0)" ::: "memory"); CHILD_T(t_it1); CHILD_TADD(5, t_dr0, t_it1); CHILD_TADD(4, t_it0, t_it1); }
#endif
    }
    CHILD_TFLUSH;
}

struct ChildLdsGrant { size_t bytes[16] = {0}; };
template <typename K>
int child_lds_limit(K kern, size_t lds, ChildLdsGrant& granted) {
    if (lds > 160 * 1024) { pcgc_set_error("child kernel: %zu bytes of LDS needed", lds); return -2; }
    int dev = 0;
    (void)hipGetDevice(&dev);
    size_t& g = granted.bytes[dev & 15];
    if (lds > 48 * 1024 && lds > g) {
        hipError_t e = hipFuncSetAttribute((const void*)kern, hipFuncAttributeMaxDynamicSharedMemorySize, (int)lds);
        if (e != hipSuccess) { pcgc_set_error("child kernel: cannot raise the LDS limit to %zu: %s", lds, hipGetErrorString(e)); return -1; }
        g = lds;
    }
    return 0;
}
static unsigned child_grid_units(int64_t n_units, int nw, size_t lds, int max_waves_per_cu = 16) {
    static int cus = 0;
    if (!cus) { hipDeviceProp_t p; int dev = 0; (void)hipGetDevice(&dev); cus = (hipGetDeviceProperties(&p, dev) == hipSuccess && p.multiProcessorCount > 0) ? p.multiProcessorCount : 256; }
    int per_cu = (int)((160 * 1024) / (lds ? lds : 1));
    if (per_cu > max_waves_per_cu / nw) per_cu = max_waves_per_cu / nw;
    if (per_cu < 1) per_cu = 1;
    int64_t want = (n_units + nw - 1) / nw;
    int64_t g = (int64_t)cus * per_cu;
    if (g > want) g = want;
    g = (g + 7) / 8 * 8;
    return (unsigned)g;
}
static unsigned child_grid(int64_t n_p, int nw, size_t lds, int units_per_tile = 1) {
    return child_grid_units(((n_p + 15) / 16) * units_per_tile, nw, lds);
}
#define CHILD_LAUNCH_EX(KERN, NW, RINGBYTES, EP, MT_, UPT)                                                                     \
    do {                                                                                                                       \
        const size_t lds = (size_t)table_bytes + (size_t)(NW) * (RINGBYTES);                                                   \
        auto kern = KERN;                                                                                                      \
        static ChildLdsGrant granted;                                                                                          \
        if (int rc = child_lds_limit(kern, lds, granted)) return rc;                                                           \
        const int64_t units = ((n_p + 16 * (MT_) - 1) / (16 * (MT_))) * (UPT);                                                 \
        hipLaunchKernelGGL(kern, dim3(child_grid_units(units, NW, lds)), dim3((NW) * 64), lds, s, pnbr, n_p, in, in_ld, table, table_bytes, EP); \
        return 0;                                                                                                              \
    } while (0)
#define CHILD_LAUNCH(KERN, NW, RINGBYTES, EP) CHILD_LAUNCH_EX(KERN, NW, RINGBYTES, EP, 1, 1)
#define CHILD_LAUNCH_SPLIT(KERN, NW, RINGBYTES, EP) CHILD_LAUNCH_EX(KERN, NW, RINGBYTES, EP, 1, 2)

template <int NB, int NT, int NW, int D, int MT = 1>
int launch_child_conv(const int32_t* pnbr, int64_t n_p, const float* in, int in_ld, const float* table, int table_bytes,
                      const ChildEpi& ep, hipStream_t s) {
    CHILD_LAUNCH_EX((k_child_conv<NB, NT, NW, D, false, MT, false>), NW, D * NB * 1024 * MT, ep, MT, 1);
}
template <int NB, int NT, int NW, int D>
int launch_child_conv_split(const int32_t* pnbr, int64_t n_p, const float* in, int in_ld, const float* table, int table_bytes,
                            const ChildEpi& ep, hipStream_t s) {
    CHILD_LAUNCH_EX((k_child_conv<NB, NT, NW, D, true, 1, false>), NW, D * NB * 1024, ep, 1, 2);
}
template <int NB, int NW, int D, int MT = 1, int WPC = 16>
int launch_child_cls(const int32_t* pnbr, int64_t n_p, const float* in, int in_ld, const float* table, int table_bytes,
                     const ChildEpi& ep, hipStream_t s) {
    const size_t lds = (size_t)table_bytes + (size_t)NW * (D * NB * 1024 * MT);
    auto kern = k_child_cls<NB, NW, D, MT>;
    static ChildLdsGrant granted;
    if (int rc = child_lds_limit(kern, lds, granted)) return rc;
    const int64_t units = (n_p + 16 * MT - 1) / (16 * MT);
    hipLaunchKernelGGL(kern, dim3(child_grid_units(units, NW, lds, WPC)), dim3(NW * 64), lds, s, pnbr, n_p, in, in_ld, table, table_bytes, ep);
    return 0;
}
template <int C, int NW, int D, int MT = 1>
int launch_child_irn_a(const int32_t* pnbr, int64_t n_p, const float* in, int in_ld, const float* table, int table_bytes,
                       const IrnEpi& ep, hipStream_t s) {
    CHILD_LAUNCH_EX((k_child_irn_a<C, NW, D, false, MT>), NW, D * (C / 16) * 1024 * MT, ep, MT, 1);
}
template <int C, int NW, int D>
int launch_child_irn_a_split(const int32_t* pnbr, int64_t n_p, const float* in, int in_ld, const float* table, int table_bytes,
                             const IrnEpi& ep, hipStream_t s) {
    CHILD_LAUNCH_SPLIT((k_child_irn_a<C, NW, D, true>), NW, D * (C / 16) * 1024, ep);
}
template <int C, int NW, int D, int MT = 1, bool T2 = false>
int launch_child_irn_b(const int32_t* pnbr, int64_t n_p, const float* in, int in_ld, const float* table, int table_bytes,
                       const IrnEpi& ep, hipStream_t s) {
    constexpr int Q = C / 4, CH = ((128 * Q + 64 * C) * 4 <= D * 1024 * MT) ? 64 : 32;
    constexpr int need = (128 * Q + CH * C) * 4;
    constexpr int ringb = (D * 1024 * MT > need) ? D * 1024 * MT : need;
    CHILD_LAUNCH_EX((k_child_irn_b<C, NW, D, false, MT, T2>), NW, ringb, ep, MT, 1);
}
template <int C, int NW, int D>
int launch_child_irn_b_split(const int32_t* pnbr, int64_t n_p, const float* in, int in_ld, const float* table, int table_bytes,
                             const IrnEpi& ep, hipStream_t s) {
    constexpr int Q = C / 4, CH = ((128 * Q + 64 * C) * 4 <= D * 1024) ? 64 : 32;
    constexpr int need = (128 * Q + CH * C) * 4;
    constexpr int ringb = (D * 1024 > need) ? D * 1024 : need;
    CHILD_LAUNCH_SPLIT((k_child_irn_b<C, NW, D, true>), NW, ringb, ep);
}

}

#define CHILD_COMMON_CHECKS(ROWS_LD)                                                                                           \
    PCGC_REQUIRE(parent_nbr && in && table, "null argument");                                                                  \
    PCGC_REQUIRE(((ROWS_LD) & 3) == 0 && (((uintptr_t)in | (uintptr_t)table) & 15) == 0, "unaligned input");                 \
    PCGC_REQUIRE(8 * n_parent * (int64_t)(ROWS_LD) * 4 < (int64_t)0xF0000000, "tensor too large for 32-bit buffer offsets"); \
    PCGC_REQUIRE(table_bytes % 16 == 0, "table size");                                                                         \
    if (n_parent == 0) return 0;
```

### pcgcv2_amd/csrc/child_q4.h

```cpp
#pragma once
#include "child_kernels.h"

namespace {

struct Q4Group {
    int cell, child, kind;
    int k;
    bool first, last;
    bool fin;
};
struct Q4Sched {
    int n;
    Q4Group g[232];
    int vm_wait[232];
    int pend[232];
};
constexpr int Q4_PASS_A = 0, Q4_CLS = 1;
template <int KIND, int MT, int D = 2>
constexpr Q4Sched q4_sched() {
    Q4Sched S{};
    for (int c = 0; c < 64; ++c) {
        const int n0 = S.n;
        if (KIND == Q4_CLS) {
            for (int h = 0; h < 2; ++h)
                if (in02(cz_of(c) - h)) { S.g[S.n] = Q4Group{c, h, 0, S.n, false, false, false}; S.n++; }
        } else {
            for (int j = 0; j < 8; ++j) {
                if (!((cell_reach(c) >> j) & 1)) continue;
                const int k = cell_k(c, j);
                S.g[S.n++] = Q4Group{c, j, 0, k, false, false, k == 26};
                if (k == 13) S.g[S.n++] = Q4Group{c, j, 1, 27, false, false, false};
            }
        }
        S.g[n0].first = true;
        S.g[S.n - 1].last = true;
    }
    int ops = 0, pending = 0;
    int gather_end[64 + 16] = {};
    for (int c = 0; c < D; ++c) { ops += 4 * MT; gather_end[c] = ops; }
    for (int n = 0; n < S.n; ++n) {
        const Q4Group& G = S.g[n];
        if (G.last && G.cell + 1 < 64) S.vm_wait[n] = ops - gather_end[G.cell + 1];
        if (G.first && G.cell + D < 64) { ops += 4 * MT; gather_end[G.cell + D] = ops; }
        S.pend[n] = pending;
        ops += pending;
        pending = (KIND == Q4_PASS_A && ((G.kind == 1) || G.fin) && (G.child & 3) == 3) ? 4 * MT : 0;
    }
    return S;
}

typedef unsigned u32x4 __attribute__((ext_vector_type(4)));
__device__ __forceinline__ void q4_store(const f32x4& v, const __amdgpu_buffer_rsrc_t& rs, unsigned voff) {
    u32x4 u = {__float_as_uint(v[0]), __float_as_uint(v[1]), __float_as_uint(v[2]), __float_as_uint(v[3])};
#ifndef Q4_STORE_AUX
#define Q4_STORE_AUX 0
#endif
    __builtin_amdgcn_raw_buffer_store_b128(u, rs, (int)voff, 0, Q4_STORE_AUX);
}

template <int KIND, int NW, int MT, int D = 2>
__global__ void __launch_bounds__(NW * 64)
k_child_q4(const int32_t* __restrict__ pnbr, int64_t n_p, const float* __restrict__ in, int in_ld,
           const float* __restrict__ table, int table_bytes, IrnEpi ep) {
    constexpr int TP = 64 * MT, SLOT_F4 = MT * 256;
    constexpr Q4Sched S = q4_sched<KIND, MT, D>();
    constexpr int NACC = KIND == Q4_CLS ? 2 : 8, OUT_ROW_BYTES = KIND == Q4_CLS ? 4 : 32;
    extern __shared__ __attribute__((aligned(16))) unsigned char lds_raw[];
    const int lane = threadIdx.x & 63;
    const int wave = __builtin_amdgcn_readfirstlane(threadIdx.x >> 6);
    float4* ring = (float4*)(lds_raw + table_bytes) + wave * (D * SLOT_F4);
    child_stage_table<NW>(table, table_bytes, lds_raw);
    const __amdgpu_buffer_rsrc_t rs_in = __builtin_amdgcn_make_buffer_rsrc((void*)in, 0, (int)(8 * n_p * in_ld * 4), 0x00020000);
    const __amdgpu_buffer_rsrc_t rs_out = __builtin_amdgcn_make_buffer_rsrc((void*)ep.out, 0, (int)(8 * n_p * OUT_ROW_BYTES), 0x00020000);
    const int co = lane & 3;
    float b00[4], b10[4];
#pragma unroll
    for (int r = 0; r < 4; ++r) { b00[r] = KIND == Q4_CLS ? (ep.b0 ? ep.b0[0] : 0.0f) : ep.b0[r]; b10[r] = KIND == Q4_CLS ? 0.0f : ep.b1[r]; }
    const unsigned tab_lane = (unsigned)(uintptr_t)(lds_void_ptr)((const float*)lds_raw + co * 16);
    const unsigned a_row = (unsigned)(uintptr_t)(lds_void_ptr)((const float*)ring + lane * 16 + (((lane >> 2) & 3) << 2));
    const unsigned row_bytes = (unsigned)in_ld * 4u;
    const unsigned lane_off = (unsigned)(((lane & 3) ^ ((lane >> 4) & 3)) * 16);
    constexpr unsigned ABSENT = 0xF0000000u;
    const int64_t ntiles = (n_p + TP - 1) / TP;

    for (int it = 0;; ++it) {
#ifdef Q4_EXP_TILE_ORDER
        int64_t tile;
        {
            const int64_t S = (ntiles + 7) >> 3;
            const int64_t l = ((int64_t)(blockIdx.x >> 3) + (int64_t)(gridDim.x >> 3) * it) * NW + wave;
            tile = (blockIdx.x & 7) * S + l;
            if (!(l < S && tile < ntiles)) tile = -1;
        }
#else
        const int64_t tile = child_tile<NW>(it, wave, ntiles);
#endif
        if (tile < 0) break;
        const int64_t p_base = tile * TP;
        unsigned rowb[MT][27];
        bool ok[MT];
#pragma unroll
        for (int m = 0; m < MT; ++m) {
            const int64_t rho = p_base + 64 * m + 16 * (lane & 3) + (lane >> 2);
            ok[m] = rho < n_p;
#pragma unroll
            for (int kp = 0; kp < 27; ++kp) rowb[m][kp] = (unsigned)pnbr[(int64_t)kp * n_p + (ok[m] ? rho : 0)];
        }
        asm volatile("s_waitcnt vmcnt(0)" ::: "memory");
#pragma unroll
        for (int m = 0; m < MT; ++m)
#pragma unroll
            for (int kp = 0; kp < 27; ++kp)
#ifdef Q4_KO_GATHER
                rowb[m][kp] = ((int)rowb[m][kp] == 0x7FFFFFF1) ? rowb[m][kp] * (8u * row_bytes) : ABSENT;
#else
                rowb[m][kp] = (ok[m] && (int)rowb[m][kp] >= 0) ? rowb[m][kp] * (8u * row_bytes) : ABSENT;
#endif
        auto ovq = [&](int m) { return (unsigned)((p_base + 64 * m + (lane & ~3)) * 256 + (lane & 3) * 16); };
#ifdef Q4_KO_STORE
        f32x4 sink = (f32x4){0.f, 0.f, 0.f, 0.f};
#endif

        f32x4 acc0[MT][NACC], c1[MT][KIND == Q4_CLS ? 1 : 4];
#pragma unroll
        for (int m = 0; m < MT; ++m)
#pragma unroll
            for (int j = 0; j < NACC; ++j) acc0[m][j] = (f32x4){0.f, 0.f, 0.f, 0.f};
        f32x4 a[MT][4], b[2][4];

        auto gather = [&](auto ic) {
            constexpr int c = decltype(ic)::value, kp = cell_kp(c), ch = cell_child(c), slot = c % D;
            const unsigned cell_off = (unsigned)ch * row_bytes + lane_off;
#pragma unroll
            for (int m = 0; m < MT; ++m) {
                const int rb = (int)rowb[m][kp];
                const unsigned v0 = (unsigned)__builtin_amdgcn_update_dpp(0, rb, 0x00, 0xF, 0xF, true) + cell_off;
                const unsigned v1 = (unsigned)__builtin_amdgcn_update_dpp(0, rb, 0x55, 0xF, 0xF, true) + cell_off;
                const unsigned v2 = (unsigned)__builtin_amdgcn_update_dpp(0, rb, 0xAA, 0xF, 0xF, true) + cell_off;
                const unsigned v3 = (unsigned)__builtin_amdgcn_update_dpp(0, rb, 0xFF, 0xF, 0xF, true) + cell_off;
                float4* dst = ring + slot * SLOT_F4 + m * 256;
                __builtin_amdgcn_raw_ptr_buffer_load_lds(rs_in, (lds_void_ptr)(dst), 16, (int)v0, 0, 0, 0);
                __builtin_amdgcn_raw_ptr_buffer_load_lds(rs_in, (lds_void_ptr)(dst + 64), 16, (int)v1, 0, 0, 0);
                __builtin_amdgcn_raw_ptr_buffer_load_lds(rs_in, (lds_void_ptr)(dst + 128), 16, (int)v2, 0, 0, 0);
                __builtin_amdgcn_raw_ptr_buffer_load_lds(rs_in, (lds_void_ptr)(dst + 192), 16, (int)v3, 0, 0, 0);
            }
            asm volatile("" ::: "memory");
        };
        auto load_a = [&](auto ic, auto ie) {
            constexpr int c = decltype(ic)::value, e = decltype(ie)::value, slot = c % D;
            static_for<0, MT>([&](auto im) {
                constexpr int m = decltype(im)::value;
                a[m][e] = lds_ld128_off<(slot * MT + m) * 4096>(a_row ^ (unsigned)(e << 4));
            });
        };
        auto load_b = [&](auto in_, auto ibuf) {
            constexpr int n = decltype(in_)::value, buf = decltype(ibuf)::value;
            static_for<0, 4>([&](auto ie) {
                constexpr int e = decltype(ie)::value;
                b[buf][e] = lds_ld128_off<S.g[n].k * 256 + e * 16>(tab_lane);
            });
        };
        auto epi = [&](auto in_) {
            constexpr int n = decltype(in_)::value;
            constexpr Q4Group G = S.g[n];
            constexpr int sidx = G.child & 3, h = G.child >> 2;
            if constexpr (G.kind == 1) {
                static_for<0, MT>([&](auto im) {
                    constexpr int m = decltype(im)::value;
#pragma unroll
                    for (int r = 0; r < 4; ++r) c1[m][sidx][r] = fmaxf(c1[m][sidx][r] + b10[r], 0.0f);
                });
            }
            if constexpr ((G.kind == 1 || G.fin) && sidx == 3) {
                float onehot[4];
#pragma unroll
                for (int k = 0; k < 4; ++k) onehot[k] = (co == k) ? 1.0f : 0.0f;
                static_for<0, MT>([&](auto im) {
                    constexpr int m = decltype(im)::value;
                    f32x4 V[4], W[4];
#pragma unroll
                    for (int k = 0; k < 4; ++k) {
                        if constexpr (G.kind == 1) V[k] = c1[m][k];
                        else {
#pragma unroll
                            for (int r = 0; r < 4; ++r) V[k][r] = fmaxf(acc0[m][4 * h + k][r] + b00[r], 0.0f);
                        }
                    }
#pragma unroll
                    for (int r = 0; r < 4; ++r) W[r] = (f32x4){0.f, 0.f, 0.f, 0.f};
#pragma unroll
                    for (int k = 0; k < 4; ++k)
#pragma unroll
                        for (int r = 0; r < 4; ++r) W[r] = __builtin_amdgcn_mfma_f32_4x4x1f32(V[k][r], onehot[k], W[r], 0, 0, 0);
#pragma unroll
                    for (int t = 0; t < 4; ++t) {
                        const f32x4 v = {W[0][t], W[1][t], W[2][t], W[3][t]};
#ifdef Q4_KO_STORE
                        sink = sink + v;
#else
                        q4_store(v, rs_out, ovq(m) + (unsigned)(t * 256 + h * 128 + (G.kind == 1 ? 64 : 0)));
#endif
                    }
                });
            }
        };

        using I0 = std::integral_constant<int, 0>;
        static_for<0, D>(gather);
        wait_vmcnt<4 * MT * (D - 1)>();
        load_b(I0{}, I0{});
        static_for<0, 4>([&](auto ie) { load_a(I0{}, ie); });

        static_for<0, S.n>([&](auto in_) {
            constexpr int n = decltype(in_)::value, cur = n & 1;
            constexpr Q4Group G = S.g[n];
            constexpr bool has_next = n + 1 < S.n, next_cell = G.cell + 1 < 64;
            if constexpr (G.first) wait_lgkmcnt<3 * MT>(); else wait_lgkmcnt<0>();
            static_for<0, 4>([&](auto ie) { lds_tie(b[cur][decltype(ie)::value]); });
            if constexpr (G.first) static_for<0, MT>([&](auto im) { lds_tie(a[decltype(im)::value][0]); });
            if constexpr (has_next) load_b(std::integral_constant<int, has_next ? n + 1 : n>{}, std::integral_constant<int, cur ^ 1>{});
            if constexpr (G.last && next_cell) wait_vmcnt<S.vm_wait[n]>();
            if constexpr (G.kind == 1) static_for<0, MT>([&](auto im) { c1[decltype(im)::value][G.child & 3] = (f32x4){0.f, 0.f, 0.f, 0.f}; });
            static_for<0, 4>([&](auto ie) {
                constexpr int e = decltype(ie)::value;
                if constexpr (G.first && e > 0) {
                    __builtin_amdgcn_sched_barrier(0);
                    wait_lgkmcnt<(3 - e) * MT + (has_next ? 4 : 0) + ((G.last && next_cell) ? e * MT : 0)>();
                    static_for<0, MT>([&](auto im) { lds_tie(a[decltype(im)::value][e]); });
                }
                static_for<0, 4>([&](auto iu) {
                    constexpr int u = decltype(iu)::value;
                    static_for<0, MT>([&](auto im) {
                        constexpr int m = decltype(im)::value;
#ifdef Q4_KO_MFMA
                        if constexpr (u == 0) { if constexpr (G.kind == 1) c1[m][G.child & 3][0] += a[m][e][0] * b[cur][e][0]; else acc0[m][G.child][0] += a[m][e][0] * b[cur][e][0]; }
#else
                        if constexpr (G.kind == 1) c1[m][G.child & 3] = __builtin_amdgcn_mfma_f32_4x4x1f32(b[cur][e][u], a[m][e][u], c1[m][G.child & 3], 0, 0, 0);
                        else acc0[m][G.child] = __builtin_amdgcn_mfma_f32_4x4x1f32(b[cur][e][u], a[m][e][u], acc0[m][G.child], 0, 0, 0);
#endif
                    });
                });
                if constexpr (G.last && next_cell) {
                    __builtin_amdgcn_sched_barrier(0);
                    load_a(std::integral_constant<int, next_cell ? G.cell + 1 : G.cell>{}, ie);
                }
            });
            __builtin_amdgcn_sched_barrier(0);
            if constexpr (G.first && G.cell + D < 64) gather(std::integral_constant<int, (G.cell + D < 64) ? G.cell + D : 0>{});
            if constexpr (KIND == Q4_PASS_A && n > 0) epi(std::integral_constant<int, (n > 0 ? n - 1 : 0)>{});
        });
        if constexpr (KIND == Q4_PASS_A) {
            epi(std::integral_constant<int, S.n - 1>{});
        } else {
            static_for<0, MT>([&](auto im) {
                constexpr int m = decltype(im)::value;
                const unsigned ov = (unsigned)((p_base + 64 * m + lane) * 32);
#pragma unroll
                for (int h = 0; h < 2; ++h) {
                    f32x4 v = acc0[m][h];
                    if (ep.b0) {
#pragma unroll
                        for (int r = 0; r < 4; ++r) v[r] = v[r] + b00[r];
                    }
#ifdef Q4_KO_STORE
                    sink = sink + v;
#else
                    q4_store(v, rs_out, ov + (unsigned)(h * 16));
#endif
                }
            });
        }
#ifdef Q4_KO_STORE
        q4_store(sink, rs_out, ovq(0));
#endif
    }
}

template <int KIND, int NW, int MT, int D = 2>
int launch_child_q4(const int32_t* pnbr, int64_t n_p, const float* in, int in_ld, const float* table, int table_bytes,
                    const IrnEpi& ep, hipStream_t s) {
    const size_t lds = (size_t)table_bytes + (size_t)NW * (D * MT * 4096);
    auto kern = k_child_q4<KIND, NW, MT, D>;
    static ChildLdsGrant granted;
    if (int rc = child_lds_limit(kern, lds, granted)) return rc;
    const int64_t units = (n_p + 64 * MT - 1) / (64 * MT);
    hipLaunchKernelGGL(kern, dim3(child_grid_units(units, NW, lds)), dim3(NW * 64), lds, s, pnbr, n_p, in, in_ld, table, table_bytes, ep);
    return 0;
}

}
```

### pcgcv2_amd/csrc/rows_irn.hip

```cpp
#include "child_kernels.h"

namespace {

struct RowsGeometry {
    static constexpr int NCELLS = 27, ROW_MUL = 1, NMAP = 27;
    static constexpr int kp(int c) { return c; }
    static constexpr int child(int) { return 0; }
    static constexpr int byte_off(int) { return 0; }
};
struct RowsPassA64H {
    static constexpr int NCELLS = 54, ROW_MUL = 1, NMAP = 27;
    static constexpr int kp(int c) { return c >> 1; }
    static constexpr int child(int) { return 0; }
    static constexpr int byte_off(int c) { return (c & 1) * 128; }
    static constexpr int NB = 2, ROWCHUNKS = 4, T = 2, KS = 4, Z_HALF = -1;
    static constexpr bool HALF = false;
    static constexpr int kfirst(int) { return 0; }
    static constexpr bool active(int c, int t) { return t == 0 || (c >> 1) == 13; }
    static constexpr int frag(int c, int t) { return t == 0 ? (c >> 1) : 27; }
    static constexpr bool uses_block(int, int) { return true; }
    static constexpr int frag_off(int c, int t, int cb) { return (frag(c, t) * 4 + 2 * (c & 1) + cb) * 1024; }
};
struct RowsPassB64 : RowsGeometry {
    static constexpr int NB = 2, ROWCHUNKS = 4, T = 3, KS = 4, Z_HALF = -1, FRAG_W12 = 81;
    static constexpr bool HALF = false;
    static constexpr int kfirst(int) { return 0; }
    static constexpr bool active(int, int) { return true; }
    static constexpr int frag(int c, int t) { return t < 2 ? 2 * c + t : 54 + c; }
    static constexpr bool uses_block(int t, int cb) { return t < 2 ? cb == 0 : cb == 1; }
    static constexpr int frag_off(int c, int t, int) { return frag(c, t) * 1024; }
};

template <int NW, int D, class V = RowsPassA64H>
__global__ void __launch_bounds__(NW * 64)
k_rows_irn_a64(const int32_t* __restrict__ pnbr, int64_t n_p , const float* __restrict__ in, int in_ld,
               const float* __restrict__ table, int table_bytes, IrnEpi ep) {
    CHILD_KERNEL_PROLOGUE(V, NW, D, D * V::NB * 64)
    const float b00 = ep.b0[mi], b10 = ep.b1[mi];
    float* scratch = (float*)ring;
    for (int i = 0;; ++i) {
        const int64_t tile = child_tile<NW>(i, wave, ntiles);
        if (tile < 0) break;
        const int64_t row0 = tile * 16;
        CHILD_T(t_it0);
        f32x4 acc[V::T];
        child_tile_mainloop<V, D>(pnbr, n_p, row0, rs_in, in_ld, lds_raw, ring, acc CHILD_DBG_ARG);
#pragma unroll
        for (int r = 0; r < 4; ++r) {
            scratch[(4 * mq + r) * 32 + mi] = fmaxf(acc[0][r] + b00, 0.0f);
            scratch[(4 * mq + r) * 32 + 16 + mi] = fmaxf(acc[1][r] + b10, 0.0f);
        }
        wave_lds_sync();
        child_flush<32, 16>(scratch, row0, n_p, ep.out, 32, 0, lane);
        wave_lds_sync();
#ifdef PCGC_CHILD_TIMING
        { CHILD_T(t_dr0); asm volatile("s_waitcnt vmcnt(0)" ::: "memory"); CHILD_T(t_it1); CHILD_TADD(5, t_dr0, t_it1); CHILD_TADD(4, t_it0, t_it1); }
#endif
    }
    CHILD_TFLUSH;
}

template <int NW, int D>
__global__ void __launch_bounds__(NW * 64)
k_rows_irn_b64(const int32_t* __restrict__ pnbr, int64_t n_p, const float* __restrict__ in , int in_ld,
               const float* __restrict__ table, int table_bytes, IrnEpi ep) {
    using V = RowsPassB64;
    constexpr int NEEDF4 = (16 * 16 + 16 * 64) / 4;
    constexpr int RINGF4 = (D * V::NB * 64 > NEEDF4) ? D * V::NB * 64 : NEEDF4;
    CHILD_KERNEL_PROLOGUE(V, NW, D, RINGF4)
    float* us = (float*)ring;
    float* stage = us + 16 * 16;
    f32x4 w12[2];
#pragma unroll
    for (int n2 = 0; n2 < 2; ++n2) w12[n2] = *((const f32x4*)(lds_raw + (V::FRAG_W12 + n2) * 1024) + lane);
    const float b01a = ep.b0[mi], b01b = ep.b0[16 + mi], b11 = ep.b1[mi], b12a = ep.b2[mi], b12b = ep.b2[16 + mi];
    for (int i = 0;; ++i) {
        const int64_t tile = child_tile<NW>(i, wave, ntiles);
        if (tile < 0) break;
        const int64_t row0 = tile * 16;
        CHILD_T(t_it0);
        f32x4 acc[V::T];
        child_tile_mainloop<V, D>(pnbr, n_p, row0, rs_in, in_ld, lds_raw, ring, acc CHILD_DBG_ARG);
        ChildResidual<64, 16> rr;
        child_flush_prefetch<64, 16>(rr, row0, n_p, ep.x, ep.x_ld, lane);
#pragma unroll
        for (int r = 0; r < 4; ++r) {
            us[(4 * mq + r) * 16 + mi] = fmaxf(acc[2][r] + b11, 0.0f);
            stage[(4 * mq + r) * 64 + mi] = acc[0][r] + b01a;
            stage[(4 * mq + r) * 64 + 16 + mi] = acc[1][r] + b01b;
        }
        wave_lds_sync();
#pragma unroll
        for (int n2 = 0; n2 < 2; ++n2) {
            f32x4 d = (f32x4){0.f, 0.f, 0.f, 0.f};
#pragma unroll
            for (int jj = 0; jj < 4; ++jj) d = __builtin_amdgcn_mfma_f32_16x16x4f32(us[mi * 16 + 4 * jj + mq], w12[n2][jj], d, 0, 0, 0);
#pragma unroll
            for (int r = 0; r < 4; ++r) stage[(4 * mq + r) * 64 + 32 + 16 * n2 + mi] = d[r] + (n2 ? b12b : b12a);
        }
        wave_lds_sync();
        child_flush<64, 16>(stage, rr, ep.x != nullptr, row0, n_p, ep.out, ep.out_ld, 0, lane);
        wave_lds_sync();
#ifdef PCGC_CHILD_TIMING
        { CHILD_T(t_dr0); asm volatile("s_waitcnt vmcnt(0)" ::: "memory"); CHILD_T(t_it1); CHILD_TADD(5, t_dr0, t_it1); CHILD_TADD(4, t_it0, t_it1); }
#endif
    }
    CHILD_TFLUSH;
}

struct RowsPassA32 : RowsGeometry {
    static constexpr int NB = 2, ROWCHUNKS = 4, T = 1, KS = 4, Z_HALF = -1;
    static constexpr bool HALF = false;
    static constexpr int kfirst(int) { return 0; }
    static constexpr bool active(int, int) { return true; }
    static constexpr int frag(int c, int) { return c; }
    static constexpr bool uses_block(int, int) { return true; }
    static constexpr int frag_off(int c, int t, int cb) { return (frag(c, t) * NB + cb) * 1024; }
};
struct RowsPassB32 : RowsGeometry {
    static constexpr int NB = 1, ROWCHUNKS = 4, T = 2, KS = 2, Z_HALF = -1, FRAG_W12 = 54;
    static constexpr bool HALF = false;
    static constexpr int kfirst(int t) { return t == 0 ? 0 : 2; }
    static constexpr bool active(int, int) { return true; }
    static constexpr int frag(int c, int t) { return t == 0 ? c : 27 + c; }
    static constexpr bool uses_block(int, int) { return true; }
    static constexpr int frag_off(int c, int t, int) { return frag(c, t) * 512; }
};
template <int NW, int D>
__global__ void __launch_bounds__(NW * 64)
k_rows_irn_a32(const int32_t* __restrict__ pnbr, int64_t n_p, const float* __restrict__ in, int in_ld,
               const float* __restrict__ table, int table_bytes, IrnEpi ep) {
    using V = RowsPassA32;
    CHILD_KERNEL_PROLOGUE(V, NW, D, D * V::NB * 64)
    const float bcol = mi < 8 ? ep.b0[mi] : ep.b1[mi - 8];
    float* scratch = (float*)ring;
    for (int i = 0;; ++i) {
        const int64_t tile = child_tile<NW>(i, wave, ntiles);
        if (tile < 0) break;
        const int64_t row0 = tile * 16;
        CHILD_T(t_it0);
        f32x4 acc[V::T];
        child_tile_mainloop<V, D>(pnbr, n_p, row0, rs_in, in_ld, lds_raw, ring, acc CHILD_DBG_ARG);
#pragma unroll
        for (int r = 0; r < 4; ++r) scratch[(4 * mq + r) * 16 + mi] = fmaxf(acc[0][r] + bcol, 0.0f);
        wave_lds_sync();
        child_flush<16, 16>(scratch, row0, n_p, ep.out, 16, 0, lane);
        wave_lds_sync();
#ifdef PCGC_CHILD_TIMING
        { CHILD_T(t_dr0); asm volatile("s_waitcnt vmcnt(0)" ::: "memory"); CHILD_T(t_it1); CHILD_TADD(5, t_dr0, t_it1); CHILD_TADD(4, t_it0, t_it1); }
#endif
    }
    CHILD_TFLUSH;
}
template <int NW, int D>
__global__ void __launch_bounds__(NW * 64)
k_rows_irn_b32(const int32_t* __restrict__ pnbr, int64_t n_p, const float* __restrict__ in , int in_ld,
               const float* __restrict__ table, int table_bytes, IrnEpi ep) {
    using V = RowsPassB32;
    constexpr int NEEDF4 = (16 * 8 + 16 * 32) / 4;
    constexpr int RINGF4 = (D * V::NB * 64 > NEEDF4) ? D * V::NB * 64 : NEEDF4;
    CHILD_KERNEL_PROLOGUE(V, NW, D, RINGF4)
    float* us = (float*)ring;
    float* stage = us + 16 * 8;
    float w12[2];
#pragma unroll
    for (int jj = 0; jj < 2; ++jj) w12[jj] = ((const float*)(lds_raw + V::FRAG_W12 * 512))[lane * 2 + jj];
    const float b01 = ep.b0[mi], b11 = mi < 8 ? ep.b1[mi] : 0.0f, b12 = ep.b2[mi];
    for (int i = 0;; ++i) {
        const int64_t tile = child_tile<NW>(i, wave, ntiles);
        if (tile < 0) break;
        const int64_t row0 = tile * 16;
        CHILD_T(t_it0);
        f32x4 acc[V::T];
        child_tile_mainloop<V, D>(pnbr, n_p, row0, rs_in, in_ld, lds_raw, ring, acc CHILD_DBG_ARG);
        ChildResidual<32, 16> rr;
        child_flush_prefetch<32, 16>(rr, row0, n_p, ep.x, ep.x_ld, lane);
#pragma unroll
        for (int r = 0; r < 4; ++r) {
            if (mi < 8) us[(4 * mq + r) * 8 + mi] = fmaxf(acc[1][r] + b11, 0.0f);
            stage[(4 * mq + r) * 32 + mi] = acc[0][r] + b01;
        }
        wave_lds_sync();
        f32x4 d = (f32x4){0.f, 0.f, 0.f, 0.f};
#pragma unroll
        for (int jj = 0; jj < 2; ++jj) d = __builtin_amdgcn_mfma_f32_16x16x4f32(us[mi * 8 + 4 * jj + mq], w12[jj], d, 0, 0, 0);
#pragma unroll
        for (int r = 0; r < 4; ++r) stage[(4 * mq + r) * 32 + 16 + mi] = d[r] + b12;
        wave_lds_sync();
        child_flush<32, 16>(stage, rr, ep.x != nullptr, row0, n_p, ep.out, ep.out_ld, 0, lane);
        wave_lds_sync();
#ifdef PCGC_CHILD_TIMING
        { CHILD_T(t_dr0); asm volatile("s_waitcnt vmcnt(0)" ::: "memory"); CHILD_T(t_it1); CHILD_TADD(5, t_dr0, t_it1); CHILD_TADD(4, t_it0, t_it1); }
#endif
    }
    CHILD_TFLUSH;
}

template <int NB_, int NT>
struct RowsConv : RowsGeometry {
    static constexpr int NB = NB_, ROWCHUNKS = 4, T = NT, KS = 4, Z_HALF = -1;
    static constexpr bool HALF = false;
    static constexpr int kfirst(int) { return 0; }
    static constexpr bool active(int, int) { return true; }
    static constexpr int frag(int c, int t) { return c * NT + t; }
    static constexpr bool uses_block(int, int) { return true; }
    static constexpr int frag_off(int c, int t, int cb) { return (frag(c, t) * NB + cb) * 1024; }
};
template <int NB, int NT, int NW, int D>
__global__ void __launch_bounds__(NW * 64)
k_rows_conv(const int32_t* __restrict__ pnbr, int64_t n_p, const float* __restrict__ in, int in_ld,
            const float* __restrict__ table, int table_bytes, ChildEpi ep) {
    using V = RowsConv<NB, NT>;
    constexpr int W = 16 * NT;
    constexpr int NEEDF4 = 16 * W / 4;
    constexpr int RINGF4 = (D * NB * 64 > NEEDF4) ? D * NB * 64 : NEEDF4;
    CHILD_KERNEL_PROLOGUE(V, NW, D, RINGF4)
    float* scratch = (float*)ring;
    float bv[NT];
#pragma unroll
    for (int t = 0; t < NT; ++t) bv[t] = ep.bias ? ep.bias[16 * t + mi] : 0.0f;
    for (int i = 0;; ++i) {
        const int64_t tile = child_tile<NW>(i, wave, ntiles);
        if (tile < 0) break;
        const int64_t row0 = tile * 16;
        CHILD_T(t_it0);
        f32x4 acc[V::T];
        child_tile_mainloop<V, D>(pnbr, n_p, row0, rs_in, in_ld, lds_raw, ring, acc CHILD_DBG_ARG);
        ChildResidual<W, 16> rr;
        child_flush_prefetch<W, 16>(rr, row0, n_p, ep.res, ep.res_ld, lane);
#pragma unroll
        for (int t = 0; t < NT; ++t) {
#pragma unroll
            for (int r = 0; r < 4; ++r) {
                float v = acc[t][r];
                if (ep.bias) v = v + bv[t];
                scratch[(4 * mq + r) * W + 16 * t + mi] = v;
            }
        }
        wave_lds_sync();
        child_flush<W, 16>(scratch, rr, ep.res != nullptr, row0, n_p, ep.out, ep.out_ld, ep.relu, lane);
        wave_lds_sync();
#ifdef PCGC_CHILD_TIMING
        { CHILD_T(t_dr0); asm volatile("s_waitcnt vmcnt(0)" ::: "memory"); CHILD_T(t_it1); CHILD_TADD(5, t_dr0, t_it1); CHILD_TADD(4, t_it0, t_it1); }
#endif
    }
    CHILD_TFLUSH;
}

struct DownGeometry {
    static constexpr int NCELLS = 8, ROW_MUL = 1, NMAP = 8;
    static constexpr int kp(int c) { return c; }
    static constexpr int child(int) { return 0; }
    static constexpr int byte_off(int) { return 0; }
};
template <int NB_, int NT>
struct RowsDown : DownGeometry {
    static constexpr int NB = NB_, ROWCHUNKS = 4, T = NT, KS = 4, Z_HALF = -1;
    static constexpr bool HALF = false;
    static constexpr int kfirst(int) { return 0; }
    static constexpr bool active(int, int) { return true; }
    static constexpr int frag(int c, int t) { return c * NT + t; }
    static constexpr bool uses_block(int, int) { return true; }
    static constexpr int frag_off(int c, int t, int cb) { return (frag(c, t) * NB + cb) * 1024; }
};
template <int NB, int NT, int NW, int D>
__global__ void __launch_bounds__(NW * 64)
k_rows_down(const int32_t* __restrict__ pnbr , int64_t n_p , const float* __restrict__ in, int in_ld,
            const float* __restrict__ table, int table_bytes, ChildEpi ep, int64_t n_in ) {
    using V = RowsDown<NB, NT>;
    constexpr int W = 16 * NT;
    constexpr int NEEDF4 = 16 * W / 4;
    constexpr int RINGF4 = (D * NB * 64 > NEEDF4) ? D * NB * 64 : NEEDF4;
    CHILD_KERNEL_PROLOGUE(V, NW, D, RINGF4)
    (void)rs_in;
    const __amdgpu_buffer_rsrc_t rs_fine = __builtin_amdgcn_make_buffer_rsrc((void*)in, 0, (int)(n_in * in_ld * 4), 0x00020000);
    float* scratch = (float*)ring;
    float bv[NT];
#pragma unroll
    for (int t = 0; t < NT; ++t) bv[t] = ep.bias ? ep.bias[16 * t + mi] : 0.0f;
    for (int i = 0;; ++i) {
        const int64_t tile = child_tile<NW>(i, wave, ntiles);
        if (tile < 0) break;
        const int64_t row0 = tile * 16;
        CHILD_T(t_it0);
        f32x4 acc[V::T];
        child_tile_mainloop<V, D>(pnbr, n_p, row0, rs_fine, in_ld, lds_raw, ring, acc CHILD_DBG_ARG);
        ChildResidual<W, 16> rr;
        child_flush_prefetch<W, 16>(rr, row0, n_p, ep.res, ep.res_ld, lane);
#pragma unroll
        for (int t = 0; t < NT; ++t) {
#pragma unroll
            for (int r = 0; r < 4; ++r) {
                float v = acc[t][r];
                if (ep.bias) v = v + bv[t];
                scratch[(4 * mq + r) * W + 16 * t + mi] = v;
            }
        }
        wave_lds_sync();
        child_flush<W, 16>(scratch, rr, ep.res != nullptr, row0, n_p, ep.out, ep.out_ld, ep.relu, lane);
        wave_lds_sync();
#ifdef PCGC_CHILD_TIMING
        { CHILD_T(t_dr0); asm volatile("s_waitcnt vmcnt(0)" ::: "memory"); CHILD_T(t_it1); CHILD_TADD(5, t_dr0, t_it1); CHILD_TADD(4, t_it0, t_it1); }
#endif
    }
    CHILD_TFLUSH;
}

template <typename K, typename EPI>
int launch_rows(K kern, int nw, size_t lds, const int32_t* nbr, int64_t n, const float* in, int in_ld, const float* table, int table_bytes,
                const EPI& ep, hipStream_t s, ChildLdsGrant& granted) {
    if (int rc = child_lds_limit(kern, lds, granted)) return rc;
    hipLaunchKernelGGL(kern, dim3(child_grid(n, nw, lds)), dim3(nw * 64), lds, s, nbr, n, in, in_ld, table, table_bytes, ep);
    return 0;
}

}

constexpr int64_t ROWS32_DEEP_MAX = 32768;

extern "C" int pcgc_irn_rows_pass(const int32_t* nbr, int64_t n, int C, int pass, const float* in, int in_ld, const float* table,
                                  int64_t table_bytes, const float* b0, const float* b1, const float* b2, const float* x, int x_ld, float* out,
                                  int out_ld, void* stream) {
    PCGC_REQUIRE(nbr && in && table, "null argument");
    PCGC_REQUIRE((in_ld & 3) == 0 && (((uintptr_t)in | (uintptr_t)table) & 15) == 0, "unaligned input");
    PCGC_REQUIRE(n * (int64_t)in_ld * 4 < (int64_t)0xF0000000, "tensor too large for 32-bit buffer offsets");
    PCGC_REQUIRE(C == 64 || C == 32, "channels must be 32 or 64");
    PCGC_REQUIRE(pass == 1 || pass == 2, "pass must be 1 (A) or 2 (B)");
    PCGC_REQUIRE(out && b0 && b1 && (pass == 1 || (b2 && x)), "null argument");
    PCGC_REQUIRE((out_ld & 3) == 0 && (((uintptr_t)out) & 15) == 0 && (pass == 1 || ((x_ld & 3) == 0 && (((uintptr_t)x) & 15) == 0)),
                 "rows must be 16-byte aligned");
    PCGC_REQUIRE(pass == 2 || out_ld == C / 2, "pass A writes a dense [rows, C/2] tensor");
    PCGC_REQUIRE(pass == 1 ? in_ld >= C : in_ld >= C / 2, "input rows narrower than the pass reads");
    PCGC_REQUIRE(table_bytes == (C == 64 ? (pass == 1 ? 28 * 4 * 1024 : 83 * 1024) : (pass == 1 ? 27 * 2 * 1024 : 55 * 512)), "table size");
    if (n == 0) return 0;
    hipStream_t s = S(stream);
    IrnEpi ep{b0, b1, b2, x, x_ld, out, out_ld};
    int rc;
    static ChildLdsGrant granted[8];
#define ROWS_GO(SLOT, KERN, NW_, RINGBYTES) launch_rows(KERN, NW_, (size_t)table_bytes + (size_t)(NW_) * (RINGBYTES), nbr, n, in, in_ld, table, (int)table_bytes, ep, s, granted[SLOT])
    if (C == 32 && n <= ROWS32_DEEP_MAX) {
        rc = pass == 1 ? ROWS_GO(4, (k_rows_irn_a32<8, 4>), 8, 4 * 2048) : ROWS_GO(5, (k_rows_irn_b32<8, 8>), 8, 8 * 1024);
    } else if (C == 32) {
        rc = pass == 1 ? ROWS_GO(0, (k_rows_irn_a32<16, 2>), 16, 2 * 2048) : ROWS_GO(1, (k_rows_irn_b32<16, 4>), 16, 4 * 1024);
    } else if (pass == 1) {
        rc = ROWS_GO(2, (k_rows_irn_a64<12, 2, RowsPassA64H>), 12, 2 * 2048);
    } else {
        rc = ROWS_GO(3, (k_rows_irn_b64<12, 2>), 12, 5120);
    }
#undef ROWS_GO
    if (rc) return rc;
    PCGC_CHECK_LAUNCH("irn_rows_pass");
    return 0;
}

extern "C" int pcgc_conv_rows(const int32_t* nbr, int64_t n, const float* in, int Cin, int in_ld, const float* table, int64_t table_bytes,
                              const float* bias, const float* residual, int res_ld, int relu, float* out, int Cout, int out_ld, void* stream) {
    PCGC_REQUIRE(nbr && in && table && out, "null argument");
    PCGC_REQUIRE((in_ld & 3) == 0 && (((uintptr_t)in | (uintptr_t)table) & 15) == 0, "unaligned input");
    PCGC_REQUIRE((out_ld & 3) == 0 && (((uintptr_t)out) & 15) == 0, "output rows must be 16-byte aligned");
    PCGC_REQUIRE(residual == nullptr || ((res_ld & 3) == 0 && (((uintptr_t)residual) & 15) == 0), "residual rows must be 16-byte aligned");
    PCGC_REQUIRE(n * (int64_t)in_ld * 4 < (int64_t)0xF0000000, "tensor too large for 32-bit buffer offsets");
    PCGC_REQUIRE(Cin == 32 && Cout == 32, "conv_rows: 32 -> 32");
    PCGC_REQUIRE(in_ld >= Cin && out_ld >= Cout, "rows narrower than the layer");
    PCGC_REQUIRE(table_bytes == (int64_t)27 * Cin * Cout * 4, "table size");
    if (n == 0) return 0;
    hipStream_t s = S(stream);
    ChildEpi ep{bias, residual, res_ld, relu, out, out_ld, Cout / 16};
    static ChildLdsGrant granted[4];
    int rc;
#define ROWS_GO(SLOT, KERN, NW_, RINGBYTES) launch_rows(KERN, NW_, (size_t)table_bytes + (size_t)(NW_) * (RINGBYTES), nbr, n, in, in_ld, table, (int)table_bytes, ep, s, granted[SLOT])
    rc = ROWS_GO(3, (k_rows_conv<2, 2, 12, 2>), 12, 2 * 2048);
#undef ROWS_GO
    if (rc) return rc;
    PCGC_CHECK_LAUNCH("conv_rows");
    return 0;
}

extern "C" int pcgc_conv_down_rows(const int32_t* down, int64_t n_coarse, const float* in, int64_t n_in, int Cin, int in_ld, const float* table,
                                   int64_t table_bytes, const float* bias, int relu, float* out, int Cout, int out_ld, void* stream) {
    PCGC_REQUIRE(down && in && table && out, "null argument");
    PCGC_REQUIRE((in_ld & 3) == 0 && (((uintptr_t)in | (uintptr_t)table) & 15) == 0, "unaligned input");
    PCGC_REQUIRE((out_ld & 3) == 0 && (((uintptr_t)out) & 15) == 0, "output rows must be 16-byte aligned");
    PCGC_REQUIRE(n_in * (int64_t)in_ld * 4 < (int64_t)0xF0000000, "tensor too large for 32-bit buffer offsets");
    PCGC_REQUIRE((Cin == 16 && Cout == 32) || (Cin == 32 && Cout == 64) || (Cin == 64 && Cout == 32), "conv_down_rows: 16 -> 32, 32 -> 64 or 64 -> 32");
    PCGC_REQUIRE(in_ld >= Cin && out_ld >= Cout, "rows narrower than the layer");
    PCGC_REQUIRE(table_bytes == (int64_t)8 * Cin * Cout * 4, "table size");
    if (n_coarse == 0) return 0;
    hipStream_t s = S(stream);
    ChildEpi ep{bias, nullptr, 0, relu, out, out_ld, Cout / 16};
    static ChildLdsGrant granted[3];
    int rc;
#define DOWN_GO(SLOT, NB_, NT_, NW_, D_)                                                                                                       \
    do {                                                                                                                                       \
        constexpr int need = 16 * 16 * (NT_) * 4, ringb = ((D_) * (NB_) * 1024 > need) ? (D_) * (NB_) * 1024 : need;                           \
        const size_t lds = (size_t)table_bytes + (size_t)(NW_) * ringb;                                                                        \
        auto kern = k_rows_down<NB_, NT_, NW_, D_>;                                                                                            \
        rc = child_lds_limit(kern, lds, granted[SLOT]);                                                                                        \
        if (!rc) hipLaunchKernelGGL(kern, dim3(child_grid(n_coarse, NW_, lds)), dim3((NW_) * 64), lds, s, down, n_coarse, in, in_ld, table,   \
                                    (int)table_bytes, ep, n_in);                                                                               \
    } while (0)
    if (Cin == 16) DOWN_GO(0, 1, 2, 16, 2);
    else if (Cin == 32) DOWN_GO(1, 2, 4, 12, 2);
    else DOWN_GO(2, 4, 2, 8, 2);
#undef DOWN_GO
    if (rc) return rc;
    PCGC_CHECK_LAUNCH("conv_down_rows");
    return 0;
}
CHILD_TIMING_READER(pcgc_child_timing_rows)
```

### pcgcv2_amd/csrc/rows_q4.hip

```cpp
#include "q4x.h"

namespace {

#include "rows_q4_policy.h"

#define ROWS_Q4_PROLOGUE                                                                                                       \
    extern __shared__ __attribute__((aligned(16))) unsigned char lds_raw[];                                                    \
    const int lane = threadIdx.x & 63;                                                                                         \
    const int wave = __builtin_amdgcn_readfirstlane(threadIdx.x >> 6);                                                         \
    float4* ring = (float4*)(lds_raw + table_bytes) + wave * (D * MT * 256);                                                   \
    unsigned char* stage = (unsigned char*)ring;                                                                               \
    child_stage_table<NW>(table, table_bytes, lds_raw);                                                                        \
    const __amdgpu_buffer_rsrc_t rs_in = __builtin_amdgcn_make_buffer_rsrc((void*)in, 0, (int)(n * in_ld * 4), 0x00020000);   \
    const int64_t ntiles = (n + 64 * MT - 1) / (64 * MT);

template <int NW, int MT, int D, bool PAIRED>
__global__ void __launch_bounds__(NW * 64)
k_rows_q4_a32(const int32_t* __restrict__ nbr, int64_t n, const float* __restrict__ in, int in_ld, const float* __restrict__ table,
              int table_bytes, IrnEpi ep) {
    ROWS_Q4_PROLOGUE
    float bias[4][4];
#pragma unroll
    for (int c = 0; c < 4; ++c)
#pragma unroll
        for (int r = 0; r < 4; ++r) bias[c][r] = c < 2 ? ep.b0[4 * c + r] : ep.b1[4 * (c - 2) + r];
    for (int it = 0;; ++it) {
        const int64_t tile = child_tile<NW>(it, wave, ntiles);
        if (tile < 0) break;
        const int64_t row0 = tile * (64 * MT);
        f32x4 acc[MT][4];
        Q4XTile<RowsQ4A32<PAIRED>, MT, D>::run(nbr, n, row0, rs_in, (unsigned)in_ld * 4u, lds_raw, ring, acc);
#pragma unroll
        for (int m = 0; m < MT; ++m)
#pragma unroll
            for (int c = 0; c < 4; ++c) {
                f32x4 v;
#pragma unroll
                for (int r = 0; r < 4; ++r) v[r] = fmaxf(acc[m][c][r] + bias[c][r], 0.0f);
                *(f32x4*)(stage + m * 4096 + q4x_stage_addr<4>(lane, c)) = v;
            }
        wave_lds_sync();
#pragma unroll
        for (int m = 0; m < MT; ++m)
#pragma unroll
            for (int i = 0; i < 4; ++i) {
                const int q = lane + 64 * i, r = q >> 2, c = q & 3;
                const int64_t row = row0 + 64 * m + r;
                if (row < n) *(f32x4*)(ep.out + row * 16 + 4 * c) = *(const f32x4*)(stage + m * 4096 + q4x_stage_addr<4>(r, c));
            }
        wave_lds_sync();
    }
}

template <int NW, int MT, int D>
__global__ void __launch_bounds__(NW * 64)
k_rows_q4_b32(const int32_t* __restrict__ nbr, int64_t n, const float* __restrict__ in , int in_ld,
              const float* __restrict__ table, int table_bytes, IrnEpi ep) {
    static_assert(D >= 2, "the output staging needs two ring slots");
    ROWS_Q4_PROLOGUE
    float b01[4][4], b11[2][4], b12[4][4];
#pragma unroll
    for (int g = 0; g < 4; ++g)
#pragma unroll
        for (int r = 0; r < 4; ++r) { b01[g][r] = ep.b0[4 * g + r]; b12[g][r] = ep.b2[4 * g + r]; }
#pragma unroll
    for (int g = 0; g < 2; ++g)
#pragma unroll
        for (int r = 0; r < 4; ++r) b11[g][r] = ep.b1[4 * g + r];
    const unsigned tab_lane = (unsigned)(uintptr_t)(lds_void_ptr)((const float*)lds_raw + (lane & 3) * 16);
    for (int it = 0;; ++it) {
        const int64_t tile = child_tile<NW>(it, wave, ntiles);
        if (tile < 0) break;
        const int64_t row0 = tile * (64 * MT);
        f32x4 acc[MT][6];
        Q4XTile<RowsQ4B32, MT, D>::run(nbr, n, row0, rs_in, (unsigned)in_ld * 4u, lds_raw, ring, acc);
        f32x4 xr[MT][8];
#pragma unroll
        for (int m = 0; m < MT; ++m)
#pragma unroll
            for (int i = 0; i < 8; ++i) {
                const int q = lane + 64 * i;
                const int64_t row = row0 + 64 * m + (q >> 3);
                xr[m][i] = row < n ? *(const f32x4*)(ep.x + row * ep.x_ld + 4 * (q & 7)) : (f32x4){0.f, 0.f, 0.f, 0.f};
            }
        f32x4 w12[2][4];
        static_for<0, 2>([&](auto ip) {
            static_for<0, 4>([&](auto ie) {
                constexpr int p = decltype(ip)::value, e = decltype(ie)::value;
                w12[p][e] = lds_ld128_off<(RowsQ4B32::FRAG_W12 + p) * 256 + e * 16>(tab_lane);
            });
        });
        wait_lgkmcnt<0>();
        static_for<0, 2>([&](auto ip) { static_for<0, 4>([&](auto ie) { lds_tie(w12[decltype(ip)::value][decltype(ie)::value]); }); });
        f32x4 o2[MT][4];
#pragma unroll
        for (int m = 0; m < MT; ++m) {
            f32x4 u[2];
#pragma unroll
            for (int g = 0; g < 2; ++g)
#pragma unroll
                for (int r = 0; r < 4; ++r) u[g][r] = fmaxf(acc[m][4 + g][r] + b11[g][r], 0.0f);
#pragma unroll
            for (int g = 0; g < 4; ++g) o2[m][g] = (f32x4){0.f, 0.f, 0.f, 0.f};
#pragma unroll
            for (int p = 0; p < 2; ++p)
#pragma unroll
                for (int e = 0; e < 4; ++e)
#pragma unroll
                    for (int uu = 0; uu < 4; ++uu)
                        o2[m][2 * p + (e >> 1)] = __builtin_amdgcn_mfma_f32_4x4x1f32(w12[p][e][uu], u[e & 1][uu], o2[m][2 * p + (e >> 1)], 0, 0, 0);
        }
#pragma unroll
        for (int m = 0; m < MT; ++m)
#pragma unroll
            for (int c = 0; c < 8; ++c) {
                f32x4 v;
#pragma unroll
                for (int r = 0; r < 4; ++r) v[r] = c < 4 ? acc[m][c][r] + b01[c][r] : o2[m][c - 4][r] + b12[c - 4][r];
                *(f32x4*)(stage + m * 8192 + q4x_stage_addr<8>(lane, c)) = v;
            }
        wave_lds_sync();
#pragma unroll
        for (int m = 0; m < MT; ++m)
#pragma unroll
            for (int i = 0; i < 8; ++i) {
                const int q = lane + 64 * i, r = q >> 3, c = q & 7;
                const int64_t row = row0 + 64 * m + r;
                f32x4 v = *(const f32x4*)(stage + m * 8192 + q4x_stage_addr<8>(r, c));
                v = v + xr[m][i];
                if (row < n) *(f32x4*)(ep.out + row * ep.out_ld + 4 * c) = v;
            }
        wave_lds_sync();
    }
}

template <typename K>
int launch_rows_q4(K kern, int nw, int mt, int d, const int32_t* nbr, int64_t n, const float* in, int in_ld, const float* table, int table_bytes,
                   const IrnEpi& ep, hipStream_t s, ChildLdsGrant& granted) {
    const size_t lds = (size_t)table_bytes + (size_t)nw * d * mt * 4096;
    if (int rc = child_lds_limit(kern, lds, granted)) return rc;
    const int64_t units = (n + 64 * mt - 1) / (64 * mt);
    hipLaunchKernelGGL(kern, dim3(child_grid_units(units, nw, lds)), dim3(nw * 64), lds, s, nbr, n, in, in_ld, table, table_bytes, ep);
    return 0;
}

int g_rows_q4_variant = 0;

}

extern "C" int pcgc_set_rows_q4_variant(int v) {
    if (v < 0 || v > 3) return -1;
    g_rows_q4_variant = v;
    return 0;
}

extern "C" int pcgc_irn_rows_q4_pass(const int32_t* nbr, int64_t n, int C, int pass, const float* in, int in_ld, const float* table,
                                     int64_t table_bytes, const float* b0, const float* b1, const float* b2, const float* x, int x_ld,
                                     float* out, int out_ld, void* stream) {
    PCGC_REQUIRE(nbr && in && table, "null argument");
    PCGC_REQUIRE((in_ld & 3) == 0 && (((uintptr_t)in | (uintptr_t)table) & 15) == 0, "unaligned input");
    PCGC_REQUIRE(n * (int64_t)in_ld * 4 < (int64_t)0xF0000000, "tensor too large for 32-bit buffer offsets");
    PCGC_REQUIRE(C == 32, "the quad-block rows kernels serve C = 32");
    PCGC_REQUIRE(pass == 1 || pass == 2, "pass must be 1 (A) or 2 (B)");
    PCGC_REQUIRE(out && b0 && b1 && (pass == 1 || (b2 && x)), "null argument");
    PCGC_REQUIRE((out_ld & 3) == 0 && (((uintptr_t)out) & 15) == 0 && (pass == 1 || ((x_ld & 3) == 0 && (((uintptr_t)x) & 15) == 0)),
                 "rows must be 16-byte aligned");
    PCGC_REQUIRE(pass == 2 || out_ld == 16, "pass A writes a dense [rows, 16] tensor");
    PCGC_REQUIRE(pass == 1 ? in_ld >= 32 : in_ld == 16, "input rows: x at least 32 wide, t dense [rows, 16]");
    PCGC_REQUIRE(pass == 1 || (out_ld >= 32 && x_ld >= 32), "pass B rows narrower than the layer");
    PCGC_REQUIRE(table_bytes == (pass == 1 ? RowsQ4A32Base::NFRAG : RowsQ4B32::NFRAG) * 256, "table size");
    if (n == 0) return 0;
    hipStream_t s = S(stream);
    IrnEpi ep{b0, b1, b2, x, x_ld, out, out_ld};
    const int v = g_rows_q4_variant ? g_rows_q4_variant : 3;
    static ChildLdsGrant granted[6];
    int rc;
#define Q4_GO(SLOT, KERN, NW_, MT_, D_) launch_rows_q4(KERN, NW_, MT_, D_, nbr, n, in, in_ld, table, (int)table_bytes, ep, s, granted[SLOT])
    if (pass == 1)
        rc = v == 1 ? Q4_GO(0, (k_rows_q4_a32<8, 2, 2, false>), 8, 2, 2) : v == 2 ? Q4_GO(1, (k_rows_q4_a32<8, 1, 4, true>), 8, 1, 4)
           : Q4_GO(2, (k_rows_q4_a32<16, 1, 2, false>), 16, 1, 2);
    else
        rc = v == 1 ? Q4_GO(3, (k_rows_q4_b32<8, 2, 2>), 8, 2, 2) : v == 2 ? Q4_GO(4, (k_rows_q4_b32<8, 1, 4>), 8, 1, 4) : Q4_GO(5, (k_rows_q4_b32<12, 1, 2>), 12, 1, 2);
#undef Q4_GO
    if (rc) return rc;
    PCGC_CHECK_LAUNCH("irn_rows_q4_pass");
    return 0;
}
```

### pcgcv2_amd/ops.py

```python
import os as _os

import numpy as np
import torch

from ._lib import lib, check, PcgcError


def _stream(t=None):
    if t is None:
        return torch.cuda.current_stream().cuda_stream
    return torch.cuda.current_stream(t.device).cuda_stream


def _p(t):
    return None if t is None else t.data_ptr()


def _dev(t, dtype, what):
    if not t.is_cuda:
        raise PcgcError(f'{what}: expected a ROCm device tensor, got {t.device} (no CPU fallback exists)')
    if t.dtype != dtype:
        raise PcgcError(f'{what}: expected {dtype}, got {t.dtype}')
    if not t.is_contiguous():
        raise PcgcError(f'{what}: tensor must be contiguous')
# ... 395 lines not shown
    return out


def coords_children(coords, stride_in):
    out = torch.empty((8 * coords.shape[0], 4), dtype=torch.int32, device=coords.device)
    check(lib().pcgc_coords_children(_p(_i32(coords)), coords.shape[0], int(stride_in), _p(out), _stream(coords)), 'coords_children')
    return out


def coords_scale(coords, factor):
    out = torch.empty_like(coords)
    check(lib().pcgc_coords_scale(_p(_i32(coords)), coords.shape[0], float(np.float32(factor)), _p(out), _stream(coords)),
          'coords_scale')
    return out


def kmap_k3(coords, stride, table):
    n = coords.shape[0]
    nbr = torch.empty((27, n), dtype=torch.int32, device=coords.device)
    check(lib().pcgc_kmap_k3(_p(_i32(coords)), n, int(stride), _p(table.keys), _p(table.vals), table.cap, _p(nbr), _stream(coords)),
          'kmap_k3')
    return nbr


def set_conv_impl(impl):
    check(lib().pcgc_set_conv_impl(int(impl)), 'set_conv_impl')


def conv_gather(nbr, x, W, bias, out=None, residual=None, relu=False, n_out=None):
    _f32(x, 'x'); _f32(W, 'W')
    if W.dim() == 2:
        K, (Cin, Cout) = 1, W.shape
    else:
        K, Cin, Cout = W.shape
    if x.shape[1] != Cin:
        raise PcgcError(f'conv_gather: input has {x.shape[1]} channels, kernel expects {Cin}')
    if nbr is None:
        n_out = x.shape[0]
    else:
        n_out = nbr.shape[1]
        if nbr.shape[0] != K:
            raise PcgcError('conv_gather: kernel map / kernel volume mismatch')
    if out is None:
        out = torch.empty((n_out, Cout), dtype=torch.float32, device=x.device)
    res_p, res_ld = (None, 0) if residual is None else (_p(_f32(residual)), _ld(residual))
    prof = K == 27 and PROFILE.want(('conv', Cin, Cout, n_out))
    if prof:
        mfma = Cin in (16, 32, 64) and Cout in (16, 32, 64) and n_out >= 8192
        e0, e1 = PROFILE.bracket(('conv', Cin, Cout, n_out), f'k3 gather conv Cin={Cin} Cout={Cout} (k_conv_gather_mfma*/dma, per-row gather)', n_out,
                                 lambda P, a=Cin, b=Cout, n=n_out: P * a * 4 + P * 8 + n * b * 4,
                                 lambda P, a=Cin, b=Cout: 2 * P * a * b,
                                 compulsory=x.shape[0] * Cin * 4 + 27 * n_out * 4 + n_out * Cout * 4,
                                 mfma_issued=(2 * 27 * ((n_out + 15) // 16 * 16) * Cin * Cout) if mfma else None)
        e0.record()
    check(lib().pcgc_conv_gather(_p(nbr), K, n_out, _p(x), x.shape[0], Cin, _ld(x), 0, _p(W), _p(bias), res_p, res_ld, 0, int(relu),
                                 _p(out), Cout, _ld(out), 0, _stream(nbr)), 'conv_gather')
    if prof:
        e1.record()
    elif PROFILE.counting and K == 27:
        PROFILE.count(nbr)
    return out




def conv_gather_unit(nbr, W, bias, relu=False):
    _f32(W, 'W')
    K, Cin, Cout = W.shape
    if Cin != 1 or nbr.shape[0] != K:
        raise PcgcError('conv_gather_unit: kernel [K, 1, Cout] and a [K, n] map expected')
    n_out = nbr.shape[1]
    out = torch.empty((n_out, Cout), dtype=torch.float32, device=W.device)
    key = ('conv', 1, Cout, n_out)
    prof = K == 27 and PROFILE.want(key)
    if prof:
        e0, e1 = PROFILE.bracket(key, f'k3 conv 1->{Cout} on the unit input (k_conv_unit: kernel map only, no feature gather)', n_out,
                                 lambda P, b=Cout, n=n_out: P * 4 + P * 8 + n * b * 4, lambda P, b=Cout: 2 * P * b,
                                 compulsory=27 * n_out * 4 + n_out * Cout * 4)
        e0.record()
    check(lib().pcgc_conv_gather_unit(_p(nbr), K, n_out, _p(W), _p(bias), int(relu), _p(out), Cout, Cout, _stream(nbr)), 'conv_gather_unit')
    if prof:
        e1.record()
    elif PROFILE.counting and K == 27:
        PROFILE.count(nbr)
    return out


def conv_unit_from_coarse(fine, stride_fine, parent_of, coarse_nbr, down, W, bias, relu=False):
    _f32(W, 'W')
    K, Cin, Cout = W.shape
    if Cin != 1 or K != 27:
        raise PcgcError('conv_unit_from_coarse: kernel [27, 1, Cout] expected')
    n = fine.shape[0]
    out = torch.empty((n, Cout), dtype=torch.float32, device=W.device)
    key = ('conv', 1, Cout, n)
    prof = PROFILE.want(key)
    if prof:
        e0, e1 = PROFILE.bracket(key, f'k3 conv 1->{Cout} on the unit input (k_conv_unit_coarse: presence from the parent level\'s map, no map of its own)', n,
                                 lambda P, b=Cout, n=n: P * 4 + P * 8 + n * b * 4, lambda P, b=Cout: 2 * P * b,
                                 compulsory=n * 16 + n * 4 + n * Cout * 4)
        e0.record()
    check(lib().pcgc_conv_unit_from_coarse(_p(_i32(fine)), n, int(stride_fine), _p(parent_of), _p(coarse_nbr), _p(down), coarse_nbr.shape[1],
                                           _p(W), _p(bias), int(relu), _p(out), Cout, Cout, _stream(fine)), 'conv_unit_from_coarse')
    if prof:
        e1.record()
    return out


def set_up2_impl(mfma):
    check(lib().pcgc_set_up2_impl(int(mfma)), 'set_up2_impl')




def _irn_pass_formulas(n, C, map_bytes, names):
    Q = C // 4
    return ((1, names[0], lambda P: (P * C * 4 + P * 8 + n * Q * 4) + n * (C + Q) * 4, lambda P: 2 * P * C * Q + 2 * n * C * Q,
             n * C * 4 + map_bytes + n * 2 * Q * 4),
            (2, names[1], lambda P: (P * Q * 4 + P * 8 + n * 2 * Q * 4) + (P * Q * 4 + P * 8 + n * Q * 4) + n * 3 * Q * 4,
             lambda P: 2 * P * Q * 2 * Q + 2 * P * Q * Q + 2 * n * Q * 2 * Q,
             n * 2 * Q * 4 + map_bytes + n * C * 4 + n * C * 4))


def irn_block(nbr, x, params):
    import ctypes
    _f32(x, 'x')
    n, C = x.shape
    t = torch.empty((n, C // 2), dtype=torch.float32, device=x.device)
    out = torch.empty((n, C), dtype=torch.float32, device=x.device)
    arr = (ctypes.c_void_p * 10)(*[p.data_ptr() for p in params])
    if PROFILE.counting:
        PROFILE.count(nbr)
    name_a, name_b = (f'k_irn_a<{C}, 16>', f'k_irn_b<{C}, 16>') if C == 64 else (f'k_irn_a_split<{C}>', f'k_irn_b_split<{C}>')
    if not (PROFILE.want((name_a, n)) or PROFILE.want((name_b, n))):
        check(lib().pcgc_irn_block(_p(nbr), n, _p(x), C, _ld(x), arr, _p(t), _p(out), C, _stream(nbr)), 'irn_block')
        return out
    Q = C // 4
    passes = _irn_pass_formulas(n, C, 27 * n * 4, (name_a, name_b))
    for ps, name, bf, ff, comp in passes:
        prof = PROFILE.want((name, n))
        if prof:
            e0, e1 = PROFILE.bracket((name, n), name + ' (per-row gather, VALU)', n, bf, ff, compulsory=comp)
            e0.record()
        check(lib().pcgc_irn_pass(_p(nbr), n, _p(x), C, _ld(x), arr, _p(t), _p(out), C, ps, _stream(nbr)), 'irn_pass')
        if prof:
            e1.record()
    return out




def irn_block_rows64(nbr, x, params, tables):
    _f32(x, 'x')
    n = x.shape[0]
    ta, tb = tables
    t = torch.empty((n, 32), dtype=torch.float32, device=x.device)
    out = torch.empty((n, 64), dtype=torch.float32, device=x.device)
    P = [p.data_ptr() for p in params]
    s = _stream(x)
    if PROFILE.counting:
        PROFILE.count(nbr)
    tiles = (n + 15) // 16
    forms = _irn_pass_formulas(n, 64, 27 * n * 4, ('k_rows_irn_a64', 'k_rows_irn_b64'))
    per_tile = (27 * 16 + 16, 27 * 12 + 8)
    calls = (lambda: lib().pcgc_irn_rows_pass(_p(nbr), n, 64, 1, _p(x), _ld(x), _p(ta), ta.numel() * 4, P[1], P[5], None, None, 0, _p(t), 32, s),
             lambda: lib().pcgc_irn_rows_pass(_p(nbr), n, 64, 2, _p(t), 32, _p(tb), tb.numel() * 4, P[3], P[7], P[9], _p(x), _ld(x), _p(out), 64, s))
    for (ps, name, bf, ff, comp), call, mf in zip(forms, calls, per_tile):
        prof = PROFILE.want((name, n))
        if prof:
            e0, e1 = PROFILE.bracket((name, n), name + ' (fused InceptionResNet pass on a plain level, LDS-resident table + per-wave row ring, fp32 MFMA)', n, bf, ff,
                                     compulsory=comp, mfma_issued=tiles * mf * 2048)
            e0.record()
        check(call(), 'irn_rows_pass')
        if prof:
            e1.record()
    return out


def _rows_irn32_index():
    C, Q = 32, 8
    shapes = [(27, C, Q), (27, Q, 2 * Q), (C, Q), (27, Q, Q), (Q, 2 * Q)]
    off, Ws = 0, []
    for shp in shapes:
        n = int(np.prod(shp))
        Ws.append(np.arange(off, off + n, dtype=np.int64).reshape(shp))
        off += n
    W00, W01, W10, W11, W12 = Ws
    fa = [_fragment([W00[k][:, co] for co in range(Q)] + [(W10[:, co] if k == 13 else None) for co in range(Q)], 2) for k in range(27)]
    pad = lambda w: np.concatenate([np.full(Q, -1, np.int64), w])
    fb = [_fragment([W01[k][:, co] for co in range(16)], 1, KS=2, k0=0) for k in range(27)]
    fb += [_fragment([pad(W11[k][:, co]) for co in range(Q)] + [None] * Q, 1, KS=2, k0=2) for k in range(27)]
    fb.append(_fragment([W12[:, co] for co in range(16)], 1, KS=2, k0=0))
    return np.concatenate([f.reshape(-1) for f in fa]), np.concatenate([f.reshape(-1) for f in fb])


def rows_irn32_tables(params):
    W00, b00, W01, b01, W10, b10, W11, b11, W12, b12 = params
    ia, ib = _table_index(('rows_irn32', W00.device), _rows_irn32_index)
    flat = torch.cat([w.detach().reshape(-1) for w in (W00, W01, W10, W11, W12)])
    return _gather_table(ia, flat), _gather_table(ib, flat)




def irn_block_rows32(nbr, x, params, tables):
    _f32(x, 'x')
    n = x.shape[0]
    ta, tb = tables
    t = torch.empty((n, 16), dtype=torch.float32, device=x.device)
    out = torch.empty((n, 32), dtype=torch.float32, device=x.device)
    P = [p.data_ptr() for p in params]
    s = _stream(x)
    if PROFILE.counting:
        PROFILE.count(nbr)
    tiles = (n + 15) // 16
    forms = _irn_pass_formulas(n, 32, 27 * n * 4, ('k_rows_irn_a32', 'k_rows_irn_b32'))
    per_tile = (27 * 8, 27 * 4 + 2)
    calls = (lambda: lib().pcgc_irn_rows_pass(_p(nbr), n, 32, 1, _p(x), _ld(x), _p(ta), ta.numel() * 4, P[1], P[5], None, None, 0, _p(t), 16, s),
             lambda: lib().pcgc_irn_rows_pass(_p(nbr), n, 32, 2, _p(t), 16, _p(tb), tb.numel() * 4, P[3], P[7], P[9], _p(x), _ld(x), _p(out), 32, s))
    for (ps, name, bf, ff, comp), call, mf in zip(forms, calls, per_tile):
        prof = PROFILE.want((name, n))
        if prof:
            e0, e1 = PROFILE.bracket((name, n), name + ' (fused InceptionResNet pass on a plain level, LDS-resident table + per-wave row ring, packed-N fp32 MFMA)', n, bf, ff,
                                     compulsory=comp, mfma_issued=tiles * mf * 2048)
            e0.record()
        check(call(), 'irn_rows_pass')
        if prof:
            e1.record()
    return out


def rows32_pass(nbr, x, params, tables, ps, t=None):
    n = x.shape[0]
    ta, tb = tables
    P = [p.data_ptr() for p in params]
    s = _stream(x)
    if ps == 1:
        t = torch.empty((n, 16), dtype=torch.float32, device=x.device)
        check(lib().pcgc_irn_rows_pass(_p(nbr), n, 32, 1, _p(x), _ld(x), _p(ta), ta.numel() * 4, P[1], P[5], None, None, 0, _p(t), 16, s), 'irn_rows_pass')
        return t
    out = torch.empty((n, 32), dtype=torch.float32, device=x.device)
    check(lib().pcgc_irn_rows_pass(_p(nbr), n, 32, 2, _p(t), 16, _p(tb), tb.numel() * 4, P[3], P[7], P[9], _p(x), _ld(x), _p(out), 32, s), 'irn_rows_pass')
    return out


def rows_q4_tables(params):
    W00, b00, W01, b01, W10, b10, W11, b11, W12, b12 = params
    C = W00.shape[1]
    if C != 32:
        raise PcgcError('rows_q4_tables: C = 32')
    a0 = W00.detach().reshape(27, 2, 16, 2, 4).permute(0, 1, 3, 4, 2).reshape(-1)
    a1 = W10.detach().reshape(2, 16, 2, 4).permute(0, 2, 3, 1).reshape(-1)
    x01 = W01.detach().reshape(27, 8, 2, 2, 4).permute(0, 2, 4, 3, 1).reshape(27, 2, 64)
    y11 = W11.detach().reshape(27, 8, 2, 4).permute(0, 3, 2, 1).reshape(27, 1, 64)
    w12 = W12.detach().reshape(8, 2, 2, 4).permute(1, 3, 2, 0).reshape(-1)
    return torch.cat([a0, a1]).contiguous(), torch.cat([torch.cat([x01, y11], 1).reshape(-1), w12]).contiguous()




def rows_q4_pass(nbr, x, params, tables, ps, t=None):
    n = x.shape[0]
    ta, tb = tables
    P = [p.data_ptr() for p in params]
    s = _stream(x)
    if ps == 1:
        t = torch.empty((n, 16), dtype=torch.float32, device=x.device)
        check(lib().pcgc_irn_rows_q4_pass(_p(nbr), n, 32, 1, _p(x), _ld(x), _p(ta), ta.numel() * 4, P[1], P[5], None, None, 0, _p(t), 16, s), 'irn_rows_q4_pass')
        return t
    out = torch.empty((n, 32), dtype=torch.float32, device=x.device)
    check(lib().pcgc_irn_rows_q4_pass(_p(nbr), n, 32, 2, _p(t), 16, _p(tb), tb.numel() * 4, P[3], P[7], P[9], _p(x), _ld(x), _p(out), 32, s), 'irn_rows_q4_pass')
    return out


def irn_block_rows32_q4(nbr, x, params, tables):
    _f32(x, 'x')
    n = x.shape[0]
    ta, tb = tables
    t = torch.empty((n, 16), dtype=torch.float32, device=x.device)
    out = torch.empty((n, 32), dtype=torch.float32, device=x.device)
    P = [p.data_ptr() for p in params]
    s = _stream(x)
    if PROFILE.counting:
        PROFILE.count(nbr)
    tiles = (n + 63) // 64
    forms = _irn_pass_formulas(n, 32, 27 * n * 4, ('k_rows_q4_a32', 'k_rows_q4_b32'))
    per_tile = (112 * 16, 81 * 16 + 32)
    calls = (lambda: lib().pcgc_irn_rows_q4_pass(_p(nbr), n, 32, 1, _p(x), _ld(x), _p(ta), ta.numel() * 4, P[1], P[5], None, None, 0, _p(t), 16, s),
             lambda: lib().pcgc_irn_rows_q4_pass(_p(nbr), n, 32, 2, _p(t), 16, _p(tb), tb.numel() * 4, P[3], P[7], P[9], _p(x), _ld(x), _p(out), 32, s))
    for (ps, name, bf, ff, comp), call, mf in zip(forms, calls, per_tile):
        prof = PROFILE.want((name, n))
        if prof:
            e0, e1 = PROFILE.bracket((name, n), name + ' (fused InceptionResNet pass on a plain level, quad-block 4x4x1 fp32 MFMA, lane = row)', n, bf, ff,
                                     compulsory=comp, mfma_issued=tiles * mf * 512)
            e0.record()
        check(call(), 'irn_rows_q4_pass')
        if prof:
            e1.record()
    return out


def set_rows_q4_variant(v):
    check(lib().pcgc_set_rows_q4_variant(int(v)), 'set_rows_q4_variant')




def _halo_cells():
    P1 = (0, 1, 1, 2)
    B = (1, 0, 1, 0)
    cells = []
    for cz in range(4):
        for cy in range(4):
            for cx in range(4):
                kp = P1[cz] * 9 + P1[cy] * 3 + P1[cx]
                jc = B[cx] + 2 * B[cy] + 4 * B[cz]
                reach = []
                for j in range(8):
                    kx, ky, kz = cx - (j & 1), cy - ((j >> 1) & 1), cz - (j >> 2)
                    if 0 <= kx <= 2 and 0 <= ky <= 2 and 0 <= kz <= 2:
                        reach.append((j, kz * 9 + ky * 3 + kx))
                cells.append((kp, jc, reach))
    assert sum(len(r) for _, _, r in cells) == 216
    return cells


def child_conv_table(W):
    K, Cin, Cout = W.shape
    NB, NT = Cin // 16, Cout // 16
    return W.detach().reshape(K, NB, 4, 4, NT, 16).permute(0, 4, 1, 3, 5, 2).contiguous().reshape(-1)


def _fragment(col_weights, NB, KS=4, k0=0, half=False):
    ncol = 8 if half else 16
    out = np.full((NB, 4, ncol, KS), -1, np.int64)
    for mi, w in enumerate(col_weights):
        if w is None:
            continue
        for cb in range(NB):
            for jj in range(KS):
                for mq in range(4):
                    ch = 16 * cb + 4 * (k0 + jj) + mq
                    if ch < len(w):
                        out[cb, mq, mi, jj] = w[ch]
    return out.reshape(NB, -1)


_TABLE_INDEX = {}


def _table_index(key, make):
    hit = _TABLE_INDEX.get(key)
    if hit is None:
        made = make()
        dev = key[-1]
        up = lambda a: None if a is None else torch.from_numpy(a).to(dev)
        hit = tuple(up(a) for a in made) if isinstance(made, tuple) else up(made)
        if torch.device(dev).type == 'cuda':
            torch.cuda.current_stream(dev).synchronize()
        _TABLE_INDEX[key] = hit
    return hit


def _gather_table(index, flat):
    return torch.where(index >= 0, flat[index.clamp(min=0)], torch.zeros((), dtype=flat.dtype, device=flat.device)).contiguous()


def _cls_index(C):
    nb = C // 16
    rowf = nb * 16 + 4
    idx = np.full(((125 * rowf * 4 + 1023) // 1024 * 256,), -1, np.int64)
    for kz in range(3):
        for ky in range(3):
            for kx in range(3):
                r = 25 * (kz + 1) + 5 * (ky + 1) + (kx + 1)
                k = 9 * kz + 3 * ky + kx
                for cb in range(nb):
                    for mq in range(4):
                        for jj in range(4):
                            idx[r * rowf + cb * 16 + mq * 4 + jj] = k * C + 16 * cb + 4 * jj + mq
    return idx


def child_cls_table(W):
    C = W.shape[1]
    return _gather_table(_table_index(('cls', C, W.device), lambda: _cls_index(C)), W.detach().reshape(-1))


def _q4_cls_index(C):
    W = np.arange(27 * C, dtype=np.int64).reshape(27, C)
    frags = []
    for c, (kp, jc, reach) in enumerate(_halo_cells()):
        cz = c >> 4
        kof = dict(reach)
        for h in range(2):
            if not 0 <= cz - h <= 2:
                continue
            f = np.full((4, C), -1, np.int64)
            for sidx in range(4):
                if 4 * h + sidx in kof:
                    f[sidx] = W[kof[4 * h + sidx]]
            frags.append(f.reshape(-1))
    assert len(frags) == 96
    return np.concatenate(frags)


def child_q4_cls_table(W):
    C = W.shape[1]
    return _gather_table(_table_index(('q4cls', C, W.device), lambda: _q4_cls_index(C)), W.detach().reshape(-1))


def cls_child_q4(parent_nbr, x, table, bias):
    _f32(x, 'x')
    n_p = parent_nbr.shape[1]
    if x.shape[0] != 8 * n_p:
        raise PcgcError('cls_child_q4: feature rows must be 8 x the parent level')
    Cin = x.shape[1]
    n = 8 * n_p
    out = torch.empty((n, 1), dtype=torch.float32, device=x.device)
    key = ('child_conv', Cin, 1, n)
    prof = PROFILE.want(key)
    if prof:
        e0, e1 = PROFILE.bracket(key, f'k_child_q4<1, 8, 2> (k3 {Cin}->1 on a children level, parent-map halo gather + quad-block 4x4x1 fp32 MFMA)', n,
                                 lambda P, a=Cin: P * a * 4 + P * 8 + n * 4, lambda P, a=Cin: 2 * P * a,
                                 compulsory=n * Cin * 4 + 27 * n_p * 4 + n * 4, mfma_issued=((n_p + 63) // 64) * 96 * 16 * 512)
        e0.record()
    check(lib().pcgc_cls_child_q4(_p(parent_nbr), n_p, _p(x), Cin, _ld(x), _p(table), table.numel() * 4, _p(bias), _p(out), _stream(x)), 'cls_child_q4')
    if prof:
        e1.record()
    elif PROFILE.counting:
        PROFILE.count_children(parent_nbr)
    return out


def _irn_index(C):
    Q, NB = C // 4, C // 16
    shapes = [(27, C, Q), (27, Q, 2 * Q), (C, Q), (27, Q, Q), (Q, 2 * Q)]
    off, Ws = 0, []
    for shp in shapes:
        n = int(np.prod(shp))
        Ws.append(np.arange(off, off + n, dtype=np.int64).reshape(shp))
        off += n
    W00, W01, W10, W11, W12 = Ws
    cpt = 16 // Q

    def packed(Wk3, width, kz, ky, cy, cx):
        cols = []
        nchild = 16 // width
        for sub in range(nchild):
            if ky is None:
                jy, jx = sub >> 1, sub & 1
                kyy = cy - jy
            else:
                jx, kyy = sub, ky
            kxx = cx - jx
            ok = 0 <= kyy <= 2 and 0 <= kxx <= 2
            for co in range(width):
                cols.append(Wk3[kz * 9 + kyy * 3 + kxx][:, co] if ok else None)
        return cols

    fa = []
    if cpt == 1:
        for k in range(27):
            fa.append(_fragment([W00[k][:, co] for co in range(16)], NB))
        fa.append(_fragment([W10[:, co] for co in range(16)], NB))
        fb = []
        for k in range(27):
            for n2 in range(2):
                fb.append(_fragment([W01[k][:, 16 * n2 + co] for co in range(16)], 1))
        for k in range(27):
            fb.append(_fragment([W11[k][:, co] for co in range(16)], 1))
        for n2 in range(2):
            fb.append(_fragment([W12[:, 16 * n2 + co] for co in range(16)], 1))
        return np.concatenate([f.reshape(-1) for f in fa]), np.concatenate([f.reshape(-1) for f in fb])
    if cpt == 4:
        for kz in range(3):
            for cy in range(4):
                for cx in range(4):
                    fa.append(_fragment(packed(W00, Q, kz, None, cy, cx), NB))
        for vy in range(2):
            for vx in range(2):
                fa.append(_fragment([W10[:, co] if sub == vy * 2 + vx else None for sub in range(4) for co in range(Q)], NB))
    else:
        for kz in range(3):
            for ky in range(3):
                for cx in range(4):
                    fa.append(_fragment(packed(W00, Q, kz, ky, None, cx), NB))
        for vx in range(2):
            fa.append(_fragment([W10[:, co] if sub == vx else None for sub in range(2) for co in range(Q)], NB))
    table_a = np.concatenate([f.reshape(-1) for f in fa])
    KS = Q // 4
    H = 2 * Q
    fb = []
    pad = lambda w, lo: np.concatenate([np.full(lo, -1, np.int64), w])
    if H == 16:
        for k in range(27):
            fb.append(_fragment([W01[k][:, co] for co in range(16)], 1, KS=KS, k0=0))
    else:
        for kz in range(3):
            for ky in range(3):
                for cx in range(4):
                    fb.append(_fragment(packed(W01, H, kz, ky, None, cx), 1, KS=KS, k0=0))
    W11p = np.stack([np.stack([pad(W11[k][:, co], Q) for co in range(Q)], 1) for k in range(27)])
    if cpt == 2:
        for kz in range(3):
            for ky in range(3):
                for cx in range(4):
                    fb.append(_fragment(packed(W11p, Q, kz, ky, None, cx), 1, KS=KS, k0=KS))
    else:
        for kz in range(3):
            for cy in range(4):
                for cx in range(4):
                    fb.append(_fragment(packed(W11p, Q, kz, None, cy, cx), 1, KS=KS, k0=KS))
    fb.append(_fragment([W12[:, co] if co < H else None for co in range(16)], 1, KS=KS, k0=0))
    table_b = np.concatenate([f.reshape(-1) for f in fb])
    return table_a, table_b


def child_irn_tables(params):
    W00, b00, W01, b01, W10, b10, W11, b11, W12, b12 = params
    C = W00.shape[1]
    ia, ib = _table_index(('irn', C, W00.device), lambda: _irn_index(C))
    flat = torch.cat([w.detach().reshape(-1) for w in (W00, W01, W10, W11, W12)])
    return _gather_table(ia, flat), (None if ib is None else _gather_table(ib, flat))




def child_q4_tables(params):
    W00, W10 = params[0], params[4]
    C = W00.shape[1]
    return torch.cat([W00.detach().reshape(27, C, C // 4).permute(0, 2, 1).reshape(-1),
                      W10.detach().reshape(C, C // 4).t().reshape(-1)]).contiguous()




def irn_block_child(parent_nbr, x, params, tables, q4_table=None):
    _f32(x, 'x')
    n_p = parent_nbr.shape[1]
    n, C = x.shape
    if n != 8 * n_p:
        raise PcgcError('irn_block_child: feature rows must be 8 x the parent level')
    ta, tb = tables
    t = torch.empty((n, C // 2), dtype=torch.float32, device=x.device)
    out = torch.empty((n, C), dtype=torch.float32, device=x.device)
    P = [p.data_ptr() for p in params]
    s = _stream(x)
    if PROFILE.counting:
        PROFILE.count_children(parent_nbr)
    tiles = (n_p + 15) // 16
    per_tile = {16: (416, 248), 32: (1216, 736)}[C]
    names = (f'k_child_irn_a<{C}>', f'k_child_irn_b<{C}>')
    q4 = PATH.CHILD_Q4 and C == 16 and q4_table is not None
    if q4:
        per_tile = ((216 + 8) * 16 // 4 // 4 + 128 // 8 // 4, per_tile[1])
        names = ('k_child_q4<0, 8, 2>', 'k_child_irn_b<16>')
    forms = _irn_pass_formulas(n, C, 27 * n_p * 4, names)
    if q4:
        calls = (lambda: lib().pcgc_irn_child_q4(_p(parent_nbr), n_p, C, 1, _p(x), _ld(x), _p(q4_table), q4_table.numel() * 4, P[1], P[5], None,
                                                 None, 0, _p(t), C // 2, s),
                 lambda: lib().pcgc_irn_child_q4(_p(parent_nbr), n_p, C, 2, _p(t), C // 2, _p(tb), tb.numel() * 4, P[3], P[7], P[9], _p(x), _ld(x),
                                                 _p(out), C, s))
    else:
        calls = (lambda: lib().pcgc_irn_child_pass(_p(parent_nbr), n_p, C, 1, _p(x), _ld(x), _p(ta), ta.numel() * 4, P[1], P[5], None, None, 0,
                                                   _p(t), C // 2, s),
                 lambda: lib().pcgc_irn_child_pass(_p(parent_nbr), n_p, C, 2, _p(t), C // 2, _p(tb), tb.numel() * 4, P[3], P[7], P[9], _p(x), _ld(x),
                                                   _p(out), C, s))
    for (ps, name, bf, ff, comp), call, mf in zip(forms, calls, per_tile):
        prof = PROFILE.want((name, n))
        if prof:
            e0, e1 = PROFILE.bracket((name, n), name + ' (fused InceptionResNet pass on a children level, packed-N fp32 MFMA)', n, bf, ff,
                                     compulsory=comp, mfma_issued=tiles * mf * 2048)
            e0.record()
        check(call(), 'irn_child_pass')
        if prof:
            e1.record()
    return out


def conv_child(parent_nbr, x, table, bias, Cout, out=None, residual=None, relu=False):
    _f32(x, 'x')
    n_p = parent_nbr.shape[1]
    if x.shape[0] != 8 * n_p:
        raise PcgcError('conv_child: feature rows must be 8 x the parent level')
    Cin = x.shape[1]
    if out is None:
        out = torch.empty((8 * n_p, Cout), dtype=torch.float32, device=x.device)
    res_p, res_ld = (None, 0) if residual is None else (_p(_f32(residual)), _ld(residual))
    n = 8 * n_p
    key = ('child_conv', Cin, Cout, n)
    prof = PROFILE.want(key)
    if prof:
        tiles = (n_p + 15) // 16
        per_tile = 64 * (Cin // 16) * 4 if Cout == 1 else 216 * (Cin // 16) * (Cout // 16) * 4
        name = f'k_child_cls<{Cin // 16}>' if Cout == 1 else f'k_child_conv<{Cin // 16}, {Cout // 16}>'
        e0, e1 = PROFILE.bracket(key, name + f' (k3 {Cin}->{Cout} on a children level, parent-map halo gather + fp32 MFMA)', n,
                                 lambda P, a=Cin, b=Cout: P * a * 4 + P * 8 + n * b * 4, lambda P, a=Cin, b=Cout: 2 * P * a * b,
                                 compulsory=n * Cin * 4 + 27 * n_p * 4 + n * Cout * 4 + (0 if residual is None else n * Cout * 4),
                                 mfma_issued=tiles * per_tile * 2048)
        e0.record()
    check(lib().pcgc_conv_child(_p(parent_nbr), n_p, _p(x), Cin, _ld(x), _p(table), table.numel() * 4, _p(bias), res_p, res_ld,
                                int(relu), _p(out), Cout, _ld(out), _stream(x)), 'conv_child')
    if prof:
        e1.record()
    elif PROFILE.counting:
# ... 1085 lines not shown
```

Before: 144.1.

## Route persistent-kernel grid sizing and tile walk through a shared plan

Replaces the ad hoc child_grid_units sizing and inline XCD-striped tile walk with a shared PersistPlan that picks workgroup count, active waves per block and slot count. Each persistent kernel gets a slots argument so waves beyond the plan exit immediately. Per-kernel families hook in saturation thresholds, and host entry points let the plan be forced or inspected. All family saturation values are zero, so the default plan may reproduce the old layout, making this mostly groundwork with some risk of shifting occupancy or tile order.

```diff
diff --git a/include/pcgc_hip.h b/include/pcgc_hip.h
--- a/include/pcgc_hip.h
+++ b/include/pcgc_hip.h
@@ -112,6 +112,12 @@
                        const float* bias, int relu, float* out, int out_ld, void* stream);
 int pcgc_set_packed_tuning(int rows, int waves);
 
+int pcgc_set_persist_plan(int waves, int max_workgroups);
+int pcgc_persist_plan(int64_t n_units, int nw_max, int wg_per_xcd, int wg_per_cu, int family, int n_sat, int force_waves, int max_workgroups,
+                      int* plan4);
+int64_t pcgc_persist_tile(int64_t n_units, const int* plan4, int block, int wave, int i);
+int pcgc_persist_walk(int64_t n_units, const int* plan4, int nw_max, int64_t* tiles);
+
 int pcgc_set_convention(int what, int value);
 
 size_t pcgc_topk_workspace_bytes(int64_t n);
diff --git a/pcgcv2_amd/_build.py b/pcgcv2_amd/_build.py
--- a/pcgcv2_amd/_build.py
+++ b/pcgcv2_amd/_build.py
@@ -9,8 +9,8 @@
 OBJ = os.path.join(CSRC, '_obj' + ('_' + VARIANT if VARIANT else ''))
 LIB = os.path.join(HERE, 'libpcgc_hip' + ('_' + VARIANT if VARIANT else '') + '.so')
 SOURCES = ['coords.hip', 'select.hip', 'conv.hip', 'child_conv.hip', 'child_conv32.hip', 'child_cls_w.hip', 'child_irn.hip', 'child_irn_a16.hip', 'child_irn_b16.hip',
-           'child_irn_a32.hip', 'child_irn_b32.hip', 'child_q4.hip', 'rows_irn.hip', 'rows_q4.hip', 'conv_packed.hip', 'entropy.hip', 'loss.hip', 'occupancy.hip', 'grad.hip', 'metric.hip', 'colour.hip', 'normals.hip', 'mesh.hip', 'collate.hip', 'hostcodec.cpp', 'ply.cpp', 'mesh_io.cpp']
-HEADERS = [os.path.join(CSRC, 'pcgc_common.h'), os.path.join(CSRC, 'mfma_util.h'), os.path.join(CSRC, 'child_kernels.h'), os.path.join(CSRC, 'child_q4.h'), os.path.join(CSRC, 'q4x.h'), os.path.join(CSRC, 'q4x_sched.h'), os.path.join(CSRC, 'rows_q4_policy.h'), os.path.join(CSRC, 'eb_logits.h'), os.path.join(CSRC, 'occupancy_tables.h'), os.path.join(HERE, '..', 'include', 'pcgc_hip.h')]
+           'child_irn_a32.hip', 'child_irn_b32.hip', 'child_q4.hip', 'rows_irn.hip', 'rows_q4.hip', 'conv_packed.hip', 'entropy.hip', 'loss.hip', 'occupancy.hip', 'grad.hip', 'metric.hip', 'colour.hip', 'normals.hip', 'mesh.hip', 'collate.hip', 'persist_plan.cpp', 'hostcodec.cpp', 'ply.cpp', 'mesh_io.cpp']
+HEADERS = [os.path.join(CSRC, 'pcgc_common.h'), os.path.join(CSRC, 'mfma_util.h'), os.path.join(CSRC, 'child_kernels.h'), os.path.join(CSRC, 'persist_plan.h'), os.path.join(CSRC, 'child_q4.h'), os.path.join(CSRC, 'q4x.h'), os.path.join(CSRC, 'q4x_sched.h'), os.path.join(CSRC, 'rows_q4_policy.h'), os.path.join(CSRC, 'eb_logits.h'), os.path.join(CSRC, 'occupancy_tables.h'), os.path.join(HERE, '..', 'include', 'pcgc_hip.h')]
 FLAGS = ['--offload-arch=gfx950', '-O3', '-std=c++17', '-ffp-contract=off', '-fPIC', '-Wall', '-Wno-unused-result'] + \
         os.environ.get('PCGC_EXTRA_HIPCC_FLAGS', '').split()
 
diff --git a/pcgcv2_amd/_lib.py b/pcgcv2_amd/_lib.py
--- a/pcgcv2_amd/_lib.py
+++ b/pcgcv2_amd/_lib.py
@@ -56,6 +56,10 @@
     'pcgc_set_rows_q4_variant': (ci, [ci]),
     'pcgc_conv_packed64': (ci, [vp, i64, vp, ci, vp, i64, vp, ci, vp, ci, vp]),
     'pcgc_set_packed_tuning': (ci, [ci, ci]),
+    'pcgc_set_persist_plan': (ci, [ci, ci]),
+    'pcgc_persist_plan': (ci, [i64, ci, ci, ci, ci, ci, ci, ci, vp]),
+    'pcgc_persist_tile': (i64, [i64, vp, ci, ci, ci]),
+    'pcgc_persist_walk': (ci, [i64, vp, ci, vp]),
     'pcgc_conv_up2': (ci, [i64, vp, ci, ci, vp, vp, ci, vp, ci, vp]),
     'pcgc_conv_up2_gather': (ci, [i64, vp, ci, ci, vp, vp, vp, ci, vp, ci, vp]),
     'pcgc_topk_workspace_bytes': (sz, [i64]),
diff --git a/pcgcv2_amd/csrc/child_kernels.h b/pcgcv2_amd/csrc/child_kernels.h
--- a/pcgcv2_amd/csrc/child_kernels.h
+++ b/pcgcv2_amd/csrc/child_kernels.h
@@ -1,6 +1,7 @@
 #pragma once
 #include "pcgc_common.h"
 #include "mfma_util.h"
+#include "persist_plan.h"
 #include <type_traits>
 
 #ifdef PCGC_CHILD_TIMING
@@ -216,15 +217,12 @@
 template <class V> constexpr int frag_floats() { return (V::HALF ? 32 : 64) * V::KS; }
 
 template <int NW, bool PERSIST = true>
-__device__ __forceinline__ int64_t child_tile(int i, int wave, int64_t ntiles) {
+__device__ __forceinline__ int64_t child_tile(int i, int wave, int64_t ntiles, int slots) {
     if constexpr (!PERSIST) {
         const int64_t tile = (int64_t)xcd_tile(blockIdx.x, gridDim.x) * NW + wave;
         return (i == 0 && tile < ntiles) ? tile : -1;
     }
-    const int64_t S = (ntiles + 7) >> 3;
-    const int64_t l = (blockIdx.x >> 3) + (int64_t)(gridDim.x >> 3) * (wave + NW * i);
-    const int64_t tile = (blockIdx.x & 7) * S + l;
-    return (l < S && tile < ntiles) ? tile : -1;
+    return persist_tile(ntiles, (int)gridDim.x, slots, (int)blockIdx.x, wave, i);
 }
 
 template <int NW>
@@ -474,7 +472,7 @@
 template <int NB, int NT, int NW, int D, bool SPLIT = false, int MT = 1, bool RES = false>
 __global__ void __launch_bounds__(NW * 64)
 k_child_conv(const int32_t* __restrict__ pnbr, int64_t n_p, const float* __restrict__ in, int in_ld,
-             const float* __restrict__ table, int table_bytes, ChildEpi ep) {
+             const float* __restrict__ table, int table_bytes, ChildEpi ep, int slots) {
     using V = PlainConv<NB, NT>;
     CHILD_KERNEL_PROLOGUE(V, NW, D, D * NB * 64 * MT)
     float bvs[NT];
@@ -517,7 +515,7 @@
     };
     const int64_t nunits = (SPLIT ? 2 : 1) * ((n_p + 16 * MT - 1) / (16 * MT));
     for (int i = 0;; ++i) {
-        const int64_t u = child_tile<NW>(i, wave, nunits);
+        const int64_t u = child_tile<NW>(i, wave, nunits, slots);
         if (u < 0) break;
         CHILD_T(t_it0);
         if constexpr (SPLIT) {
@@ -536,13 +534,13 @@
 template <int NB, int NW, int D, int MT = 1>
 __global__ void __launch_bounds__(NW * 64)
 k_child_cls(const int32_t* __restrict__ pnbr, int64_t n_p, const float* __restrict__ in, int in_ld,
-            const float* __restrict__ table, int table_bytes, ChildEpi ep) {
+            const float* __restrict__ table, int table_bytes, ChildEpi ep, int slots) {
     using V = ClsHead<NB>;
     CHILD_KERNEL_PROLOGUE(V, NW, D, D * NB * 64 * MT)
     const float bv = ep.bias ? ep.bias[0] : 0.0f;
     const int64_t nunits = (n_p + 16 * MT - 1) / (16 * MT);
     for (int i = 0;; ++i) {
-        const int64_t tile = child_tile<NW>(i, wave, nunits);
+        const int64_t tile = child_tile<NW>(i, wave, nunits, slots);
         if (tile < 0) break;
         const int64_t pu = tile * (16 * MT);
         CHILD_T(t_it0);
@@ -573,7 +571,7 @@
 template <int C, int NW, int D, bool SPLIT = false, int MT = 1>
 __global__ void __launch_bounds__(NW * 64)
 k_child_irn_a(const int32_t* __restrict__ pnbr, int64_t n_p, const float* __restrict__ in, int in_ld,
-              const float* __restrict__ table, int table_bytes, IrnEpi ep) {
+              const float* __restrict__ table, int table_bytes, IrnEpi ep, int slots) {
     using V = PassA<C>;
     constexpr int Q = V::Q, CPT = V::CPT, TH = V::TH;
     static_assert(!SPLIT || CPT <= 2, "half units: tiles of one or two children");
@@ -614,7 +612,7 @@
     };
     const int64_t nunits = (SPLIT ? 2 : 1) * ((n_p + 16 * MT - 1) / (16 * MT));
     for (int i = 0;; ++i) {
-        const int64_t u = child_tile<NW>(i, wave, nunits);
+        const int64_t u = child_tile<NW>(i, wave, nunits, slots);
         if (u < 0) break;
         CHILD_T(t_it0);
         if constexpr (SPLIT) {
@@ -633,7 +631,7 @@
 template <int C, int NW, int D, bool SPLIT = false, int MT = 1, bool T2 = false>
 __global__ void __launch_bounds__(NW * 64)
 k_child_irn_b(const int32_t* __restrict__ pnbr, int64_t n_p, const float* __restrict__ in , int in_ld,
-              const float* __restrict__ table, int table_bytes, IrnEpi ep) {
+              const float* __restrict__ table, int table_bytes, IrnEpi ep, int slots) {
     using V = PassB<C, -1, T2>;
     constexpr int Q = V::Q, H = 2 * Q, KQ = Q / 4, T0 = V::T0, T1 = V::T1, CPT0 = V::CPT0, CPT1 = V::CPT1;
     constexpr int CH = ((128 * Q + 64 * C) * 4 <= D * 1024 * MT) ? 64 : 32, MQC = CH / 32;
@@ -707,7 +705,7 @@
     };
     const int64_t nunits = (SPLIT ? 2 : 1) * ((n_p + 16 * MT - 1) / (16 * MT));
     for (int i = 0;; ++i) {
-        const int64_t u = child_tile<NW>(i, wave, nunits);
+        const int64_t u = child_tile<NW>(i, wave, nunits, slots);
         if (u < 0) break;
         CHILD_T(t_it0);
         if constexpr (SPLIT) {
@@ -737,29 +735,25 @@
     }
     return 0;
 }
-static unsigned child_grid_units(int64_t n_units, int nw, size_t lds, int max_waves_per_cu = 16) {
+static PersistPlan child_persist(int64_t n_units, int nw, size_t lds, int family = PERSIST_PRESENT, int max_waves_per_cu = 16) {
     static int cus = 0;
     if (!cus) { hipDeviceProp_t p; int dev = 0; (void)hipGetDevice(&dev); cus = (hipGetDeviceProperties(&p, dev) == hipSuccess && p.multiProcessorCount > 0) ? p.multiProcessorCount : 256; }
     int per_cu = (int)((160 * 1024) / (lds ? lds : 1));
     if (per_cu > max_waves_per_cu / nw) per_cu = max_waves_per_cu / nw;
     if (per_cu < 1) per_cu = 1;
-    int64_t want = (n_units + nw - 1) / nw;
-    int64_t g = (int64_t)cus * per_cu;
-    if (g > want) g = want;
-    g = (g + 7) / 8 * 8;
-    return (unsigned)g;
-}
-static unsigned child_grid(int64_t n_p, int nw, size_t lds, int units_per_tile = 1) {
-    return child_grid_units(((n_p + 15) / 16) * units_per_tile, nw, lds);
-}
-#define CHILD_LAUNCH_EX(KERN, NW, RINGBYTES, EP, MT_, UPT)                                                                     \
+    return persist_plan(n_units, nw, (cus * per_cu + 7) / 8, per_cu, persist_family_nsat(family), persist_family_floor(family, nw),
+                        g_pcgc_persist_force[0], g_pcgc_persist_force[1]);
+}
+#define CHILD_LAUNCH_EX(KERN, NW, RINGBYTES, EP, MT_, UPT) CHILD_LAUNCH_FAM(KERN, NW, RINGBYTES, EP, MT_, UPT, PERSIST_PRESENT)
+#define CHILD_LAUNCH_FAM(KERN, NW, RINGBYTES, EP, MT_, UPT, FAMILY)                                                            \
     do {                                                                                                                       \
         const size_t lds = (size_t)table_bytes + (size_t)(NW) * (RINGBYTES);                                                   \
         auto kern = KERN;                                                                                                      \
         static ChildLdsGrant granted;                                                                                          \
         if (int rc = child_lds_limit(kern, lds, granted)) return rc;                                                           \
         const int64_t units = ((n_p + 16 * (MT_) - 1) / (16 * (MT_))) * (UPT);                                                 \
-        hipLaunchKernelGGL(kern, dim3(child_grid_units(units, NW, lds)), dim3((NW) * 64), lds, s, pnbr, n_p, in, in_ld, table, table_bytes, EP); \
+        const PersistPlan plan = child_persist(units, NW, lds, FAMILY);                                                        \
+        hipLaunchKernelGGL(kern, dim3(plan.workgroups), dim3((NW) * 64), lds, s, pnbr, n_p, in, in_ld, table, table_bytes, EP, plan.slots); \
         return 0;                                                                                                              \
     } while (0)
 #define CHILD_LAUNCH(KERN, NW, RINGBYTES, EP) CHILD_LAUNCH_EX(KERN, NW, RINGBYTES, EP, 1, 1)
@@ -773,7 +767,7 @@
 template <int NB, int NT, int NW, int D>
 int launch_child_conv_split(const int32_t* pnbr, int64_t n_p, const float* in, int in_ld, const float* table, int table_bytes,
                             const ChildEpi& ep, hipStream_t s) {
-    CHILD_LAUNCH_EX((k_child_conv<NB, NT, NW, D, true, 1, false>), NW, D * NB * 1024, ep, 1, 2);
+    CHILD_LAUNCH_FAM((k_child_conv<NB, NT, NW, D, true, 1, false>), NW, D * NB * 1024, ep, 1, 2, (NB == 2 && NT == 2 ? PERSIST_CHILD_CONV32H : PERSIST_PRESENT));
 }
 template <int NB, int NW, int D, int MT = 1, int WPC = 16>
 int launch_child_cls(const int32_t* pnbr, int64_t n_p, const float* in, int in_ld, const float* table, int table_bytes,
@@ -783,7 +777,8 @@
     static ChildLdsGrant granted;
     if (int rc = child_lds_limit(kern, lds, granted)) return rc;
     const int64_t units = (n_p + 16 * MT - 1) / (16 * MT);
-    hipLaunchKernelGGL(kern, dim3(child_grid_units(units, NW, lds, WPC)), dim3(NW * 64), lds, s, pnbr, n_p, in, in_ld, table, table_bytes, ep);
+    const PersistPlan plan = child_persist(units, NW, lds, PERSIST_PRESENT, WPC);
+    hipLaunchKernelGGL(kern, dim3(plan.workgroups), dim3(NW * 64), lds, s, pnbr, n_p, in, in_ld, table, table_bytes, ep, plan.slots);
     return 0;
 }
 template <int C, int NW, int D, int MT = 1>
diff --git a/pcgcv2_amd/csrc/child_q4.h b/pcgcv2_amd/csrc/child_q4.h
--- a/pcgcv2_amd/csrc/child_q4.h
+++ b/pcgcv2_amd/csrc/child_q4.h
@@ -61,7 +61,7 @@
 template <int KIND, int NW, int MT, int D = 2>
 __global__ void __launch_bounds__(NW * 64)
 k_child_q4(const int32_t* __restrict__ pnbr, int64_t n_p, const float* __restrict__ in, int in_ld,
-           const float* __restrict__ table, int table_bytes, IrnEpi ep) {
+           const float* __restrict__ table, int table_bytes, IrnEpi ep, int slots) {
     constexpr int TP = 64 * MT, SLOT_F4 = MT * 256;
     constexpr Q4Sched S = q4_sched<KIND, MT, D>();
     constexpr int NACC = KIND == Q4_CLS ? 2 : 8, OUT_ROW_BYTES = KIND == Q4_CLS ? 4 : 32;
@@ -93,7 +93,7 @@
             if (!(l < S && tile < ntiles)) tile = -1;
         }
 #else
-        const int64_t tile = child_tile<NW>(it, wave, ntiles);
+        const int64_t tile = child_tile<NW>(it, wave, ntiles, slots);
 #endif
         if (tile < 0) break;
         const int64_t p_base = tile * TP;
@@ -284,7 +284,8 @@
     static ChildLdsGrant granted;
     if (int rc = child_lds_limit(kern, lds, granted)) return rc;
     const int64_t units = (n_p + 64 * MT - 1) / (64 * MT);
-    hipLaunchKernelGGL(kern, dim3(child_grid_units(units, NW, lds)), dim3(NW * 64), lds, s, pnbr, n_p, in, in_ld, table, table_bytes, ep);
+    const PersistPlan plan = child_persist(units, NW, lds);
+    hipLaunchKernelGGL(kern, dim3(plan.workgroups), dim3(NW * 64), lds, s, pnbr, n_p, in, in_ld, table, table_bytes, ep, plan.slots);
     return 0;
 }
 
diff --git a/pcgcv2_amd/csrc/persist_plan.cpp b/pcgcv2_amd/csrc/persist_plan.cpp
--- /dev/null
+++ b/pcgcv2_amd/csrc/persist_plan.cpp
@@ -0,0 +1,47 @@
+#include <stdint.h>
+#include "../../include/pcgc_hip.h"
+#include "persist_plan.h"
+
+int g_pcgc_persist_force[2] = {0, 0};
+
+int persist_family_nsat(int family) {
+    static const int n_sat[PERSIST_FAMILIES] = {
+        0,
+        0,
+        0,
+        0,
+        0,
+    };
+    return family >= 0 && family < PERSIST_FAMILIES ? n_sat[family] : 0;
+}
+int persist_family_floor(int, int nw_max) { return nw_max / 2 > 1 ? nw_max / 2 : 1; }
+
+extern "C" int pcgc_set_persist_plan(int waves, int max_workgroups) {
+    if (waves < 0 || waves > 16 || max_workgroups < 0) return -1;
+    g_pcgc_persist_force[0] = waves;
+    g_pcgc_persist_force[1] = max_workgroups;
+    return 0;
+}
+
+extern "C" int pcgc_persist_plan(int64_t n_units, int nw_max, int wg_per_xcd, int wg_per_cu, int family, int n_sat, int force_waves,
+                                 int max_workgroups, int* plan4) {
+    if (!plan4 || n_units < 0 || nw_max < 1 || nw_max > 16 || wg_per_xcd < 1 || wg_per_cu < 1 || family < 0 || family >= PERSIST_FAMILIES) return -2;
+    const PersistPlan p = persist_plan(n_units, nw_max, wg_per_xcd, wg_per_cu, n_sat < 0 ? persist_family_nsat(family) : n_sat, persist_family_floor(family, nw_max),
+                                       force_waves, max_workgroups);
+    plan4[0] = p.workgroups; plan4[1] = p.waves; plan4[2] = p.rounds; plan4[3] = p.slots;
+    return 0;
+}
+
+extern "C" int64_t pcgc_persist_tile(int64_t n_units, const int* plan4, int block, int wave, int i) {
+    if (!plan4 || block < 0 || block >= plan4[0] || wave < 0 || i < 0) return -1;
+    return persist_tile(n_units, plan4[0], plan4[3], block, wave, i);
+}
+
+extern "C" int pcgc_persist_walk(int64_t n_units, const int* plan4, int nw_max, int64_t* tiles) {
+    if (!plan4 || !tiles || nw_max < 1) return -2;
+    const int cols = plan4[2] + 1;
+    for (int b = 0; b < plan4[0]; ++b)
+        for (int w = 0; w < nw_max; ++w)
+            for (int i = 0; i < cols; ++i) tiles[((int64_t)b * nw_max + w) * cols + i] = persist_tile(n_units, plan4[0], plan4[3], b, w, i);
+    return 0;
+}
diff --git a/pcgcv2_amd/csrc/persist_plan.h b/pcgcv2_amd/csrc/persist_plan.h
--- /dev/null
+++ b/pcgcv2_amd/csrc/persist_plan.h
@@ -0,0 +1,67 @@
+#pragma once
+#include <stdint.h>
+
+#if defined(__HIPCC__) || defined(__CUDACC__)
+#define PERSIST_HD __host__ __device__
+#else
+#define PERSIST_HD
+#endif
+
+struct PersistPlan {
+    int workgroups;
+    int waves;
+    int rounds;
+    int slots;
+};
+
+PERSIST_HD static inline int64_t persist_tile(int64_t n_units, int workgroups, int slots, int block, int wave, int i) {
+    const int64_t S = (n_units + 7) >> 3;
+    const int slot = (block >> 3) + (workgroups >> 3) * wave;
+    if (slot >= slots) return -1;
+    const int64_t l = slot + (int64_t)slots * i;
+    const int64_t tile = (block & 7) * S + l;
+    return (l < S && tile < n_units) ? tile : -1;
+}
+
+static inline PersistPlan persist_plan(int64_t n_units, int nw_max, int wg_per_xcd, int wg_per_cu, int n_sat, int floor_waves,
+                                       int force_waves = 0, int max_workgroups = 0) {
+    if (nw_max < 1) nw_max = 1;
+    if (wg_per_xcd < 1) wg_per_xcd = 1;
+    if (wg_per_cu < 1) wg_per_cu = 1;
+    const int64_t S = (n_units + 7) >> 3;
+    int64_t W = (((n_units + nw_max - 1) / nw_max) + 7) >> 3;
+    if (W > wg_per_xcd) W = wg_per_xcd;
+    if (max_workgroups > 0 && W > (max_workgroups >> 3)) W = max_workgroups >> 3;
+    if (W < 1) W = 1;
+    auto rounds_at = [&](int64_t slots) { return (int)((S + slots - 1) / slots); };
+    PersistPlan p{(int)(8 * W), nw_max, S ? rounds_at(W * nw_max) : 0, (int)(W * nw_max)};
+    if (force_waves > 0) {
+        p.waves = force_waves < nw_max ? force_waves : nw_max;
+        p.slots = (int)(W * p.waves);
+        p.rounds = S ? rounds_at(p.slots) : 0;
+        return p;
+    }
+    if (S == 0 || n_sat <= 0 || n_sat >= nw_max * wg_per_cu) return p;
+    if (floor_waves < 1) floor_waves = 1;
+    int64_t best = (int64_t)p.rounds * (nw_max * wg_per_cu > n_sat ? nw_max * wg_per_cu : n_sat);
+    for (int a = nw_max - 1; a >= floor_waves; --a) {
+        const int r = rounds_at(W * a);
+        const int64_t cost = (int64_t)r * (a * wg_per_cu > n_sat ? a * wg_per_cu : n_sat);
+        if (cost < best) { best = cost; p.waves = a; p.rounds = r; }
+    }
+    p.slots = (int)((S + p.rounds - 1) / p.rounds);
+    p.waves = (int)((p.slots + W - 1) / W);
+    return p;
+}
+
+enum PersistFamily {
+    PERSIST_PRESENT = 0,
+    PERSIST_ROWS_A64,
+    PERSIST_ROWS_B64,
+    PERSIST_ROWS_CONV32,
+    PERSIST_CHILD_CONV32H,
+    PERSIST_FAMILIES
+};
+int persist_family_nsat(int family);
+int persist_family_floor(int family, int nw_max);
+extern int g_pcgc_persist_force[2];
diff --git a/pcgcv2_amd/csrc/rows_irn.hip b/pcgcv2_amd/csrc/rows_irn.hip
--- a/pcgcv2_amd/csrc/rows_irn.hip
+++ b/pcgcv2_amd/csrc/rows_irn.hip
@@ -34,12 +34,12 @@
 template <int NW, int D, class V = RowsPassA64H>
 __global__ void __launch_bounds__(NW * 64)
 k_rows_irn_a64(const int32_t* __restrict__ pnbr, int64_t n_p , const float* __restrict__ in, int in_ld,
-               const float* __restrict__ table, int table_bytes, IrnEpi ep) {
+               const float* __restrict__ table, int table_bytes, IrnEpi ep, int slots) {
     CHILD_KERNEL_PROLOGUE(V, NW, D, D * V::NB * 64)
     const float b00 = ep.b0[mi], b10 = ep.b1[mi];
     float* scratch = (float*)ring;
     for (int i = 0;; ++i) {
-        const int64_t tile = child_tile<NW>(i, wave, ntiles);
+        const int64_t tile = child_tile<NW>(i, wave, ntiles, slots);
         if (tile < 0) break;
         const int64_t row0 = tile * 16;
         CHILD_T(t_it0);
@@ -63,7 +63,7 @@
 template <int NW, int D>
 __global__ void __launch_bounds__(NW * 64)
 k_rows_irn_b64(const int32_t* __restrict__ pnbr, int64_t n_p, const float* __restrict__ in , int in_ld,
-               const float* __restrict__ table, int table_bytes, IrnEpi ep) {
+               const float* __restrict__ table, int table_bytes, IrnEpi ep, int slots) {
     using V = RowsPassB64;
     constexpr int NEEDF4 = (16 * 16 + 16 * 64) / 4;
     constexpr int RINGF4 = (D * V::NB * 64 > NEEDF4) ? D * V::NB * 64 : NEEDF4;
@@ -75,7 +75,7 @@
     for (int n2 = 0; n2 < 2; ++n2) w12[n2] = *((const f32x4*)(lds_raw + (V::FRAG_W12 + n2) * 1024) + lane);
     const float b01a = ep.b0[mi], b01b = ep.b0[16 + mi], b11 = ep.b1[mi], b12a = ep.b2[mi], b12b = ep.b2[16 + mi];
     for (int i = 0;; ++i) {
-        const int64_t tile = child_tile<NW>(i, wave, ntiles);
+        const int64_t tile = child_tile<NW>(i, wave, ntiles, slots);
         if (tile < 0) break;
         const int64_t row0 = tile * 16;
         CHILD_T(t_it0);
@@ -129,13 +129,13 @@
 template <int NW, int D>
 __global__ void __launch_bounds__(NW * 64)
 k_rows_irn_a32(const int32_t* __restrict__ pnbr, int64_t n_p, const float* __restrict__ in, int in_ld,
-               const float* __restrict__ table, int table_bytes, IrnEpi ep) {
+               const float* __restrict__ table, int table_bytes, IrnEpi ep, int slots) {
     using V = RowsPassA32;
     CHILD_KERNEL_PROLOGUE(V, NW, D, D * V::NB * 64)
     const float bcol = mi < 8 ? ep.b0[mi] : ep.b1[mi - 8];
     float* scratch = (float*)ring;
     for (int i = 0;; ++i) {
-        const int64_t tile = child_tile<NW>(i, wave, ntiles);
+        const int64_t tile = child_tile<NW>(i, wave, ntiles, slots);
         if (tile < 0) break;
         const int64_t row0 = tile * 16;
         CHILD_T(t_it0);
@@ -155,7 +155,7 @@
 template <int NW, int D>
 __global__ void __launch_bounds__(NW * 64)
 k_rows_irn_b32(const int32_t* __restrict__ pnbr, int64_t n_p, const float* __restrict__ in , int in_ld,
-               const float* __restrict__ table, int table_bytes, IrnEpi ep) {
+               const float* __restrict__ table, int table_bytes, IrnEpi ep, int slots) {
     using V = RowsPassB32;
     constexpr int NEEDF4 = (16 * 8 + 16 * 32) / 4;
     constexpr int RINGF4 = (D * V::NB * 64 > NEEDF4) ? D * V::NB * 64 : NEEDF4;
@@ -167,7 +167,7 @@
     for (int jj = 0; jj < 2; ++jj) w12[jj] = ((const float*)(lds_raw + V::FRAG_W12 * 512))[lane * 2 + jj];
     const float b01 = ep.b0[mi], b11 = mi < 8 ? ep.b1[mi] : 0.0f, b12 = ep.b2[mi];
     for (int i = 0;; ++i) {
-        const int64_t tile = child_tile<NW>(i, wave, ntiles);
+        const int64_t tile = child_tile<NW>(i, wave, ntiles, slots);
         if (tile < 0) break;
         const int64_t row0 = tile * 16;
         CHILD_T(t_it0);
@@ -209,7 +209,7 @@
 template <int NB, int NT, int NW, int D>
 __global__ void __launch_bounds__(NW * 64)
 k_rows_conv(const int32_t* __restrict__ pnbr, int64_t n_p, const float* __restrict__ in, int in_ld,
-            const float* __restrict__ table, int table_bytes, ChildEpi ep) {
+            const float* __restrict__ table, int table_bytes, ChildEpi ep, int slots) {
     using V = RowsConv<NB, NT>;
     constexpr int W = 16 * NT;
     constexpr int NEEDF4 = 16 * W / 4;
@@ -220,7 +220,7 @@
 #pragma unroll
     for (int t = 0; t < NT; ++t) bv[t] = ep.bias ? ep.bias[16 * t + mi] : 0.0f;
     for (int i = 0;; ++i) {
-        const int64_t tile = child_tile<NW>(i, wave, ntiles);
+        const int64_t tile = child_tile<NW>(i, wave, ntiles, slots);
         if (tile < 0) break;
         const int64_t row0 = tile * 16;
         CHILD_T(t_it0);
@@ -266,7 +266,7 @@
 template <int NB, int NT, int NW, int D>
 __global__ void __launch_bounds__(NW * 64)
 k_rows_down(const int32_t* __restrict__ pnbr , int64_t n_p , const float* __restrict__ in, int in_ld,
-            const float* __restrict__ table, int table_bytes, ChildEpi ep, int64_t n_in ) {
+            const float* __restrict__ table, int table_bytes, ChildEpi ep, int64_t n_in , int slots) {
     using V = RowsDown<NB, NT>;
     constexpr int W = 16 * NT;
     constexpr int NEEDF4 = 16 * W / 4;
@@ -279,7 +279,7 @@
 #pragma unroll
     for (int t = 0; t < NT; ++t) bv[t] = ep.bias ? ep.bias[16 * t + mi] : 0.0f;
     for (int i = 0;; ++i) {
-        const int64_t tile = child_tile<NW>(i, wave, ntiles);
+        const int64_t tile = child_tile<NW>(i, wave, ntiles, slots);
         if (tile < 0) break;
         const int64_t row0 = tile * 16;
         CHILD_T(t_it0);
@@ -308,9 +308,10 @@
 
 template <typename K, typename EPI>
 int launch_rows(K kern, int nw, size_t lds, const int32_t* nbr, int64_t n, const float* in, int in_ld, const float* table, int table_bytes,
-                const EPI& ep, hipStream_t s, ChildLdsGrant& granted) {
+                const EPI& ep, hipStream_t s, ChildLdsGrant& granted, int family = PERSIST_PRESENT) {
     if (int rc = child_lds_limit(kern, lds, granted)) return rc;
-    hipLaunchKernelGGL(kern, dim3(child_grid(n, nw, lds)), dim3(nw * 64), lds, s, nbr, n, in, in_ld, table, table_bytes, ep);
+    const PersistPlan plan = child_persist((n + 15) / 16, nw, lds, family);
+    hipLaunchKernelGGL(kern, dim3(plan.workgroups), dim3(nw * 64), lds, s, nbr, n, in, in_ld, table, table_bytes, ep, plan.slots);
     return 0;
 }
 
@@ -337,15 +338,15 @@
     IrnEpi ep{b0, b1, b2, x, x_ld, out, out_ld};
     int rc;
     static ChildLdsGrant granted[8];
-#define ROWS_GO(SLOT, KERN, NW_, RINGBYTES) launch_rows(KERN, NW_, (size_t)table_bytes + (size_t)(NW_) * (RINGBYTES), nbr, n, in, in_ld, table, (int)table_bytes, ep, s, granted[SLOT])
+#define ROWS_GO(SLOT, KERN, NW_, RINGBYTES, ...) launch_rows(KERN, NW_, (size_t)table_bytes + (size_t)(NW_) * (RINGBYTES), nbr, n, in, in_ld, table, (int)table_bytes, ep, s, granted[SLOT], ##__VA_ARGS__)
     if (C == 32 && n <= ROWS32_DEEP_MAX) {
         rc = pass == 1 ? ROWS_GO(4, (k_rows_irn_a32<8, 4>), 8, 4 * 2048) : ROWS_GO(5, (k_rows_irn_b32<8, 8>), 8, 8 * 1024);
     } else if (C == 32) {
         rc = pass == 1 ? ROWS_GO(0, (k_rows_irn_a32<16, 2>), 16, 2 * 2048) : ROWS_GO(1, (k_rows_irn_b32<16, 4>), 16, 4 * 1024);
     } else if (pass == 1) {
-        rc = ROWS_GO(2, (k_rows_irn_a64<12, 2, RowsPassA64H>), 12, 2 * 2048);
+        rc = ROWS_GO(2, (k_rows_irn_a64<12, 2, RowsPassA64H>), 12, 2 * 2048, PERSIST_ROWS_A64);
     } else {
-        rc = ROWS_GO(3, (k_rows_irn_b64<12, 2>), 12, 5120);
+        rc = ROWS_GO(3, (k_rows_irn_b64<12, 2>), 12, 5120, PERSIST_ROWS_B64);
     }
 #undef ROWS_GO
     if (rc) return rc;
@@ -368,8 +369,8 @@
     ChildEpi ep{bias, residual, res_ld, relu, out, out_ld, Cout / 16};
     static ChildLdsGrant granted[4];
     int rc;
-#define ROWS_GO(SLOT, KERN, NW_, RINGBYTES) launch_rows(KERN, NW_, (size_t)table_bytes + (size_t)(NW_) * (RINGBYTES), nbr, n, in, in_ld, table, (int)table_bytes, ep, s, granted[SLOT])
-    rc = ROWS_GO(3, (k_rows_conv<2, 2, 12, 2>), 12, 2 * 2048);
+#define ROWS_GO(SLOT, KERN, NW_, RINGBYTES, ...) launch_rows(KERN, NW_, (size_t)table_bytes + (size_t)(NW_) * (RINGBYTES), nbr, n, in, in_ld, table, (int)table_bytes, ep, s, granted[SLOT], ##__VA_ARGS__)
+    rc = ROWS_GO(3, (k_rows_conv<2, 2, 12, 2>), 12, 2 * 2048, PERSIST_ROWS_CONV32);
 #undef ROWS_GO
     if (rc) return rc;
     PCGC_CHECK_LAUNCH("conv_rows");
@@ -396,8 +397,9 @@
         const size_t lds = (size_t)table_bytes + (size_t)(NW_) * ringb;                                                                        \
         auto kern = k_rows_down<NB_, NT_, NW_, D_>;                                                                                            \
         rc = child_lds_limit(kern, lds, granted[SLOT]);                                                                                        \
-        if (!rc) hipLaunchKernelGGL(kern, dim3(child_grid(n_coarse, NW_, lds)), dim3((NW_) * 64), lds, s, down, n_coarse, in, in_ld, table,   \
-                                    (int)table_bytes, ep, n_in);                                                                               \
+        const PersistPlan plan = child_persist((n_coarse + 15) / 16, NW_, lds);                                                                \
+        if (!rc) hipLaunchKernelGGL(kern, dim3(plan.workgroups), dim3((NW_) * 64), lds, s, down, n_coarse, in, in_ld, table,                  \
+                                    (int)table_bytes, ep, n_in, plan.slots);                                                                   \
     } while (0)
     if (Cin == 16) DOWN_GO(0, 1, 2, 16, 2);
     else if (Cin == 32) DOWN_GO(1, 2, 4, 12, 2);
diff --git a/pcgcv2_amd/csrc/rows_q4.hip b/pcgcv2_amd/csrc/rows_q4.hip
--- a/pcgcv2_amd/csrc/rows_q4.hip
+++ b/pcgcv2_amd/csrc/rows_q4.hip
@@ -17,7 +17,7 @@
 template <int NW, int MT, int D, bool PAIRED>
 __global__ void __launch_bounds__(NW * 64)
 k_rows_q4_a32(const int32_t* __restrict__ nbr, int64_t n, const float* __restrict__ in, int in_ld, const float* __restrict__ table,
-              int table_bytes, IrnEpi ep) {
+              int table_bytes, IrnEpi ep, int slots) {
     ROWS_Q4_PROLOGUE
     float bias[4][4];
 #pragma unroll
@@ -25,7 +25,7 @@
 #pragma unroll
         for (int r = 0; r < 4; ++r) bias[c][r] = c < 2 ? ep.b0[4 * c + r] : ep.b1[4 * (c - 2) + r];
     for (int it = 0;; ++it) {
-        const int64_t tile = child_tile<NW>(it, wave, ntiles);
+        const int64_t tile = child_tile<NW>(it, wave, ntiles, slots);
         if (tile < 0) break;
         const int64_t row0 = tile * (64 * MT);
         f32x4 acc[MT][4];
@@ -55,7 +55,7 @@
 template <int NW, int MT, int D>
 __global__ void __launch_bounds__(NW * 64)
 k_rows_q4_b32(const int32_t* __restrict__ nbr, int64_t n, const float* __restrict__ in , int in_ld,
-              const float* __restrict__ table, int table_bytes, IrnEpi ep) {
+              const float* __restrict__ table, int table_bytes, IrnEpi ep, int slots) {
     static_assert(D >= 2, "the output staging needs two ring slots");
     ROWS_Q4_PROLOGUE
     float b01[4][4], b11[2][4], b12[4][4];
@@ -69,7 +69,7 @@
         for (int r = 0; r < 4; ++r) b11[g][r] = ep.b1[4 * g + r];
     const unsigned tab_lane = (unsigned)(uintptr_t)(lds_void_ptr)((const float*)lds_raw + (lane & 3) * 16);
     for (int it = 0;; ++it) {
-        const int64_t tile = child_tile<NW>(it, wave, ntiles);
+        const int64_t tile = child_tile<NW>(it, wave, ntiles, slots);
         if (tile < 0) break;
         const int64_t row0 = tile * (64 * MT);
         f32x4 acc[MT][6];
@@ -140,7 +140,8 @@
     const size_t lds = (size_t)table_bytes + (size_t)nw * d * mt * 4096;
     if (int rc = child_lds_limit(kern, lds, granted)) return rc;
     const int64_t units = (n + 64 * mt - 1) / (64 * mt);
-    hipLaunchKernelGGL(kern, dim3(child_grid_units(units, nw, lds)), dim3(nw * 64), lds, s, nbr, n, in, in_ld, table, table_bytes, ep);
+    const PersistPlan plan = child_persist(units, nw, lds);
+    hipLaunchKernelGGL(kern, dim3(plan.workgroups), dim3(nw * 64), lds, s, nbr, n, in, in_ld, table, table_bytes, ep, plan.slots);
     return 0;
 }
 
diff --git a/pcgcv2_amd/ops.py b/pcgcv2_amd/ops.py
--- a/pcgcv2_amd/ops.py
+++ b/pcgcv2_amd/ops.py
@@ -721,6 +721,10 @@
 
 def set_rows_q4_variant(v):
     check(lib().pcgc_set_rows_q4_variant(int(v)), 'set_rows_q4_variant')
+
+
+def set_persist_plan(waves=0, max_workgroups=0):
+    check(lib().pcgc_set_persist_plan(int(waves), int(max_workgroups)), 'set_persist_plan')
 
 
 
```

Result: no change. 144.2 (median of 5 runs) (+0.1%).
